# CostaLab/PILOT

Measured on AMD Instinct MI355X. Metric: W2 patient-pairs/sec (full NxN EMD matrix), higher is better.
Workload: dtype f32 (products as 2-way fp16 splits, 22 significant bits, on the f16 MFMA, f32 accumulate)

## Files before the change

pilot_amd/csrc/grid_plan.hpp:

```cpp
#pragma once
#include <hip/hip_runtime.h>

#include "abi_common.hpp"
#include "sinkhorn_layout.hpp"

constexpr int TIMING_RING = 64;

struct pilot_ot_plan {
    int N, K, device;
    double max_cost;
    void *img;
    void *p_slot;
    int *track_list;
    int *ctrl;
    int *order_list;
    unsigned char *order_bucket;
    int *order_hist;
    int *flags_ws;
    int *emd_counter;
    double *f_slab;
    size_t f_slab_bytes;
    double *emdg_slab;
    int emdg_wgs;
    double *kws;
    int generic_wgs;
    float *wide_rec;
    size_t wide_rec_n;
    int *nan_list;
    int n_cu;
    int timing;
    long n_timed;
    long n_calls;
    hipEvent_t ev[TIMING_RING][4];
    int graph_mode;
    int gkey_seen;
    struct GraphKey {
        const void *P, *M, *emd, *iters, *err, *flags;
        double reg, stop_thr, tau, floor_ulps, max_cost;
        int num_iter_max, check_period, cfg, mixed, sym, row_begin, n_rows, row_step;
        pilot::SinkhornSwitches sw;
        bool operator==(const GraphKey &o) const {
            return P == o.P && M == o.M && emd == o.emd && iters == o.iters && err == o.err && flags == o.flags && reg == o.reg &&
                   stop_thr == o.stop_thr && tau == o.tau && floor_ulps == o.floor_ulps && max_cost == o.max_cost && num_iter_max == o.num_iter_max &&
                   check_period == o.check_period && cfg == o.cfg && mixed == o.mixed && sym == o.sym && row_begin == o.row_begin &&
                   n_rows == o.n_rows && row_step == o.row_step && sw == o.sw;
        }
    } gkey;
    hipStream_t gstream;
    hipGraphExec_t gexec;
};

namespace pilot {

struct HostCtx {
    pilot_ot_plan *plan = nullptr;
    int N = 0, K = 0, device = -1;
    size_t n_out = 0;
    double *dP = nullptr, *dM = nullptr, *dE = nullptr, *dErr = nullptr;
    int *dIt = nullptr, *dFl = nullptr;
    unsigned char *pin = nullptr;
    size_t pin_bytes = 0;
    static constexpr int FETCH_EVENTS = 32;
    hipEvent_t fev[FETCH_EVENTS];
    int n_fev = 0;
    void release() {
        for (int i = 0; i < n_fev; ++i) (void)hipEventDestroy(fev[i]);
        n_fev = 0;
        if (pin) (void)hipHostFree(pin);
        pin = nullptr; pin_bytes = 0;
        if (dP) (void)hipFree(dP);
        if (dM) (void)hipFree(dM);
        if (dE) (void)hipFree(dE);
        if (dErr) (void)hipFree(dErr);
        if (dIt) (void)hipFree(dIt);
        if (dFl) (void)hipFree(dFl);
        dP = dM = dE = dErr = nullptr; dIt = dFl = nullptr;
        if (plan) pilot_ot_plan_destroy(plan);
        plan = nullptr; N = K = 0; n_out = 0; device = -1;
    }
    ~HostCtx() {}
};
HostCtx &thread_host();
int host_ctx_prepare(int N, int K, size_t n_out);
struct Fetch { void *dst; const void *src; size_t bytes; };
int host_fetch(const Fetch *f, int n);

size_t emd_counter_bytes();

}
```

pilot_amd/csrc/pilot_ot_sinkhorn.hip:

```cpp
#include <hip/hip_runtime.h>

#include <chrono>
#include <cmath>
#include <cstdio>
#include <cstdlib>
#include <new>

#include "abi_common.hpp"
#include "grid_plan.hpp"
#include "sinkhorn_launch.hpp"
#include "generic_kernels.hpp"

namespace {
using pilot::LDS_BYTES, pilot::MAX_K, pilot::GENERIC_MAX_K, pilot::WIDE_MAX_K;

bool split_fits_lds(int K, bool sym, int bands = 1) {
    const pilot::CfgShape c = pilot::shape_of(pilot::CFG_S32);
    return pilot::stream_layout(c, (K + 15) / 16, sym, true, 0, bands, 4).bytes + (size_t)pilot::handover_elems(c) * 4 <= LDS_BYTES;
}
}

static double h_max_cost_over_reg() {
    const char *e = pilot::test_switch("PILOT_OT_H_MAX_COST_OVER_REG");
    return e && *e ? atof(e) : pilot::H_MAX_COST_OVER_REG;
}

PILOT_API int pilot_ot_auto_precision(double max_cost_over_reg) {
    if (max_cost_over_reg <= h_max_cost_over_reg()) return PILOT_OT_PREC_F16X2;
    return max_cost_over_reg <= 60.0 ? PILOT_OT_PREC_BF16X3 : PILOT_OT_PREC_F64;
}

PILOT_API int pilot_ot_auto_precision_for(double max_cost_over_reg, int K, int cost_is_symmetric) {
    int prec = pilot_ot_auto_precision(max_cost_over_reg);
    if ((prec == PILOT_OT_PREC_BF16X3 || prec == PILOT_OT_PREC_F16X2) && !split_fits_lds(K, cost_is_symmetric != 0, 1)) prec = PILOT_OT_PREC_F32;
    return prec;
}

PILOT_API int pilot_ot_resolve_precision(int precision, double max_cost_over_reg, int K, int cost_is_symmetric, double tau) {
    if (precision == PILOT_OT_PREC_GENERIC || max_cost_over_reg > PILOT_OT_MAX_COST_OVER_REG) return PILOT_OT_PREC_GENERIC;
    const bool f32_class = precision == PILOT_OT_PREC_F32 || precision == PILOT_OT_PREC_BF16X3 || precision == PILOT_OT_PREC_F16X2;
    const char *raw = pilot::test_switch("PILOT_OT_RAW_PRECISION");
    const bool promote = f32_class && max_cost_over_reg > 60.0 && !(raw && *raw && *raw != '0');
    if (precision == PILOT_OT_PREC_AUTO || promote) {
        precision = pilot_ot_auto_precision_for(max_cost_over_reg, K, cost_is_symmetric);
        if (precision == PILOT_OT_PREC_F64) precision = PILOT_OT_PREC_AUTO_MIXED;
    }
    if (precision == PILOT_OT_PREC_F16X2 &&
        (max_cost_over_reg > h_max_cost_over_reg() || tau > pilot::H_MAX_TAU || !split_fits_lds(K, cost_is_symmetric != 0, 1)))
        precision = split_fits_lds(K, cost_is_symmetric != 0, 1) ? PILOT_OT_PREC_BF16X3 : PILOT_OT_PREC_F32;
    return precision;
}

PILOT_API int pilot_ot_plan_create(int N, int K, pilot_ot_plan **plan) {
    if (!plan) return fail(PILOT_OT_EINVAL, "plan is NULL");
    if (N <= 0 || K <= 0) return fail(PILOT_OT_EINVAL, "N=%d K=%d must be positive", N, K);
    if (K > GENERIC_MAX_K) return fail(PILOT_OT_ENOTSUP, "K=%d > %d cell types", K, GENERIC_MAX_K);
    if ((long long)N * N > 0x7fffffffLL) return fail(PILOT_OT_ENOTSUP, "N=%d: N*N overflows the pair index", N);
    pilot_ot_plan *pl = new (std::nothrow) pilot_ot_plan();
    if (!pl) return fail(PILOT_OT_EINVAL, "out of host memory");
    pl->N = N; pl->K = K; pl->max_cost = 1.0;
    pl->img = nullptr; pl->p_slot = nullptr; pl->track_list = nullptr; pl->ctrl = nullptr;
    pl->emd_counter = nullptr; pl->f_slab = nullptr; pl->f_slab_bytes = 0; pl->emdg_slab = nullptr; pl->emdg_wgs = 0; pl->n_cu = 256; pl->kws = nullptr; pl->generic_wgs = 0; pl->nan_list = nullptr;
    pl->wide_rec = nullptr; pl->wide_rec_n = 0;
    pl->order_list = nullptr; pl->order_bucket = nullptr; pl->order_hist = nullptr;
    pl->flags_ws = nullptr;
    pl->timing = 0; pl->n_timed = 0; pl->n_calls = 0;
    pl->graph_mode = 0; pl->gkey_seen = 0; pl->gstream = nullptr; pl->gexec = nullptr;
    for (int i = 0; i < TIMING_RING; ++i) for (int j = 0; j < 4; ++j) pl->ev[i][j] = nullptr;
    hipError_t e = hipGetDevice(&pl->device);
    if (e == hipSuccess) pl->n_cu = pilot::cu_count();
    const int kp = ((K + 31) / 32) * 32;
    if (K <= MAX_K) {
        const int rt = (K + 15) / 16;
        size_t img_bytes = pilot::img_elems(pilot::CFG_F64, rt) * sizeof(double);
        const size_t b32 = pilot::img_elems(pilot::CFG_F32, rt) * sizeof(float), bs = pilot::img_elems(pilot::CFG_S32, rt) * sizeof(float);
        const size_t bh = pilot::img_elems(pilot::CFG_H32, rt) * sizeof(float);
        if (b32 > img_bytes) img_bytes = b32;
        if (bs > img_bytes) img_bytes = bs;
        if (bh > img_bytes) img_bytes = bh;
        if (e == hipSuccess) e = hipMalloc(&pl->img, img_bytes);
    } else if (K <= WIDE_MAX_K) {
        if (e == hipSuccess) e = hipMalloc(&pl->img, pilot::img_elems(pilot::CFG_H32, 16) * sizeof(float));
    }
    {
        size_t p_bytes = sizeof(double) * ((size_t)N * kp + N);
        if (K > MAX_K && K <= WIDE_MAX_K) { const size_t two = 2 * sizeof(float) * ((size_t)N * 256 + N); p_bytes = two > p_bytes ? two : p_bytes; }
        if (e == hipSuccess) e = hipMalloc(&pl->p_slot, p_bytes);
    }
    if (e == hipSuccess) e = hipMalloc(reinterpret_cast<void **>(&pl->track_list), sizeof(int) * (size_t)N * N);
    if (e == hipSuccess) e = hipMalloc(reinterpret_cast<void **>(&pl->ctrl), pilot::CTRL_BLOCK_INTS * sizeof(int));
    if (e == hipSuccess) e = hipMalloc(reinterpret_cast<void **>(&pl->order_list), sizeof(int) * (size_t)N * N);
    if (e == hipSuccess) e = hipMalloc(reinterpret_cast<void **>(&pl->order_bucket), (size_t)N * N);
    if (e == hipSuccess) e = hipMalloc(reinterpret_cast<void **>(&pl->emd_counter), pilot::emd_counter_bytes());
    if (e == hipSuccess) e = hipMalloc(reinterpret_cast<void **>(&pl->nan_list), 2 * sizeof(int) * (size_t)N * N);
    if (e == hipSuccess) e = hipMalloc(reinterpret_cast<void **>(&pl->flags_ws), sizeof(int) * (size_t)N * N);
    if (e != hipSuccess) {
        pilot_ot_plan_destroy(pl);
        return fail(PILOT_OT_EHIP, "plan allocation failed: %s", hipGetErrorString(e));
    }
    pl->order_hist = pl->ctrl + pilot::CTRL_ORDER_HIST;
    *plan = pl;
    return PILOT_OT_OK;
}

PILOT_API int pilot_ot_plan_set_max_cost(pilot_ot_plan *pl, double max_cost) {
    if (!pl) return fail(PILOT_OT_EINVAL, "plan is NULL");
    if (!(max_cost > 0.0) || !std::isfinite(max_cost)) return fail(PILOT_OT_EINVAL, "max_cost=%g must be positive and finite", max_cost);
    pl->max_cost = max_cost;
    return PILOT_OT_OK;
}

PILOT_API int pilot_ot_plan_destroy(pilot_ot_plan *pl) {
    if (!pl) return PILOT_OT_OK;
    if (pl->img) (void)hipFree(pl->img);
    if (pl->p_slot) (void)hipFree(pl->p_slot);
    if (pl->track_list) (void)hipFree(pl->track_list);
    if (pl->ctrl) (void)hipFree(pl->ctrl);
    if (pl->order_list) (void)hipFree(pl->order_list);
    if (pl->order_bucket) (void)hipFree(pl->order_bucket);
    if (pl->flags_ws) (void)hipFree(pl->flags_ws);
    if (pl->emd_counter) (void)hipFree(pl->emd_counter);
    if (pl->f_slab) (void)hipFree(pl->f_slab);
    if (pl->emdg_slab) (void)hipFree(pl->emdg_slab);
    if (pl->kws) (void)hipFree(pl->kws);
    if (pl->nan_list) (void)hipFree(pl->nan_list);
    if (pl->wide_rec) (void)hipFree(pl->wide_rec);
    if (pl->gexec) (void)hipGraphExecDestroy(pl->gexec);
    if (pl->gstream) (void)hipStreamDestroy(pl->gstream);
    for (int i = 0; i < TIMING_RING; ++i) for (int j = 0; j < 4; ++j) if (pl->ev[i][j]) (void)hipEventDestroy(pl->ev[i][j]);
    delete pl;
    return PILOT_OT_OK;
}

namespace {

int check_grid_args(int N, int K, double reg, int num_iter_max, double stop_thr, double tau, int check_period,
                    int precision, int row_begin, int row_end, int row_step) {
    if (N <= 0 || K <= 0) return fail(PILOT_OT_EINVAL, "N=%d K=%d must be positive", N, K);
    if (!(reg > 0.0) || !std::isfinite(reg)) return fail(PILOT_OT_EINVAL, "reg=%g must be positive and finite", reg);
    if (num_iter_max < 1) return fail(PILOT_OT_EINVAL, "num_iter_max=%d must be >= 1", num_iter_max);
    if (check_period < 1) return fail(PILOT_OT_EINVAL, "check_period=%d must be >= 1", check_period);
    if (!(stop_thr >= 0.0) || !(stop_thr < 1.0)) return fail(PILOT_OT_EINVAL, "stop_thr=%g must be in [0, 1)", stop_thr);
    if (!(tau > 1.0)) return fail(PILOT_OT_EINVAL, "tau=%g must be > 1", tau);
    if (precision < PILOT_OT_PREC_AUTO || precision > PILOT_OT_PREC_F16X2)
        return fail(PILOT_OT_EINVAL, "unknown precision id %d", precision);
    if (row_step < 1 || row_begin < 0 || row_end > N || row_begin > row_end)
        return fail(PILOT_OT_EINVAL, "bad row range [%d, %d) step %d for N=%d", row_begin, row_end, row_step, N);
    if (K > GENERIC_MAX_K) return fail(PILOT_OT_ENOTSUP, "K=%d > %d cell types", K, GENERIC_MAX_K);
    return PILOT_OT_OK;
}

constexpr double MAX_COST_OVER_REG = PILOT_OT_MAX_COST_OVER_REG;

int run_generic(pilot_ot_plan *pl, const pilot::SinkhornSwitches &sw, const double *d_P, const double *d_M, double reg, int num_iter_max, double stop_thr, double tau,
                int check_period, int row_begin, int n_rows, int row_step, double *d_emd, int *d_iters, double *d_err, int *d_flags,
                hipStream_t s, const int *list = nullptr, const int *list_len = nullptr, int *queue = nullptr) {
    const int N = pl->N, K = pl->K;
    const int n_pairs = n_rows * N;
    if (n_pairs == 0) return PILOT_OT_OK;
    int nsplit = pilot::GENERIC_WAVES;
    auto lds_for = [&](int ns) { return sizeof(double) * ((8 + (size_t)ns) * (size_t)K + pilot::GENERIC_WAVES) + 16; };
    while (nsplit > 1 && lds_for(nsplit) > LDS_BYTES) nsplit /= 2;
    const size_t lds = lds_for(nsplit);
    if (lds > LDS_BYTES) return fail(PILOT_OT_ENOTSUP, "K=%d does not fit the generic kernel's LDS vectors", K);
    if (!pl->kws) {
        int wgs = 3 * pl->n_cu;
        const size_t per = sizeof(double) * 2 * (size_t)K * K;
        while (wgs > 1 && per * wgs > ((size_t)8 << 30)) wgs /= 2;
        HIP_TRY(hipMalloc(reinterpret_cast<void **>(&pl->kws), per * wgs));
        pl->generic_wgs = wgs;
    }
    if (!queue) { queue = pl->ctrl + pilot::CTRL_GENERIC_HEAD; HIP_TRY(hipMemsetAsync(queue, 0, sizeof(int), s)); }
    pilot::GenericParams g;
    g.P = d_P; g.M = d_M; g.N = N; g.K = K; g.n_pairs = n_pairs; g.row_begin = row_begin; g.row_step = row_step;
    g.reg = reg; g.tau = tau; g.stop_thr = stop_thr; g.max_iter = num_iter_max; g.period = check_period;
    g.emd = d_emd; g.iters = d_iters; g.err = d_err; g.flags = d_flags; g.kws = pl->kws; g.queue = queue; g.nsplit = nsplit;
    g.list = list; g.list_len = list_len;
    int wgs = pl->generic_wgs < n_pairs ? pl->generic_wgs : n_pairs;
    if (list && wgs > 64) wgs = 64;
    if (sw.generic_wgs > 0 && sw.generic_wgs < wgs) wgs = sw.generic_wgs;
    HIP_TRY(hipFuncSetAttribute(reinterpret_cast<const void *>(pilot::sinkhorn_generic_kernel), hipFuncAttributeMaxDynamicSharedMemorySize, (int)lds));
    hipLaunchKernelGGL(pilot::sinkhorn_generic_kernel, dim3(wgs), dim3(pilot::GENERIC_WG), lds, s, g);
    HIP_TRY(hipGetLastError());
    return PILOT_OT_OK;
}

pilot::GridParams call_params(const pilot_ot_plan *pl, int n_pairs, int row_begin, int row_step, int num_iter_max, int check_period,
                              double stop_thr, double tau, double floor_ulps, double *d_emd, int *d_iters, double *d_err, int *d_flags) {
    pilot::GridParams p;
    p.P = pl->p_slot; p.img = pl->img; p.N = pl->N; p.K = pl->K;
    p.n_pairs = n_pairs;
    p.list = pl->order_list; p.list_len = nullptr;
    p.solo_len = nullptr; p.solo_head = nullptr; p.solo_blocks = 0;
    p.row_begin = row_begin; p.row_step = row_step;
    p.max_iter = num_iter_max; p.period = check_period;
    p.stop_thr = stop_thr; p.tau = tau; p.floor_ulps = floor_ulps;
    p.emd = d_emd; p.iters = d_iters; p.err = d_err; p.flags = d_flags;
    p.track_list = pl->track_list; p.track_count = pl->ctrl + pilot::CTRL_TRACK_LEN;
    p.queue_head = pl->ctrl + pilot::CTRL_HEAD_FAST; p.queue_shards = nullptr;
    p.ring = 0; p.bands = 1;
    p.fb_list = nullptr; p.fb_count = nullptr;
    p.nan_list = pl->nan_list; p.nan_count = pl->ctrl + pilot::CTRL_NAN_LEN;
    p.unequal = pl->ctrl + pilot::CTRL_UNEQUAL;
    p.debug = 0;
    return p;
}

int run_grid(int cfg, pilot_ot_plan *pl, const pilot::SinkhornSwitches &sw, const double *d_P, const double *d_M, double reg, int num_iter_max,
             double stop_thr, double tau, int check_period, double floor_ulps, bool sym, int row_begin, int n_rows, int row_step,
             double *d_emd, int *d_iters, double *d_err, int *d_flags, hipStream_t s, bool mixed = false) {
    const int N = pl->N, K = pl->K, RT = (K + 15) / 16;
    const pilot::GridPasses g = pilot::plan_grid(cfg, N, K, n_rows, sym, mixed, pl->max_cost / reg, pl->n_cu, sw);
    if (g.rc != PILOT_OT_OK) return fail(g.rc, "%s", g.msg);
    HIP_TRY(hipMemsetAsync(pl->ctrl, 0, pilot::CTRL_BLOCK_INTS * sizeof(int), s));
    if (n_rows == 0) return PILOT_OT_OK;
    pilot::GridParams p = call_params(pl, n_rows * N, row_begin, row_step, num_iter_max, check_period, stop_thr, tau, floor_ulps, d_emd, d_iters,
                                      d_err, d_flags);
    p.debug = sw.debug;
    int *const lists[] = {pl->order_list, pl->track_list, pl->nan_list + (size_t)N * N};
    auto slot = [&](int at) { return at == pilot::CTRL_NONE ? nullptr : pl->ctrl + at; };
    if (g.f64.run) { p.fb_list = lists[g.f64.list]; p.fb_count = slot(pilot::CTRL_FB_LEN); }
    if (g.fast.solo_blocks) { p.solo_len = slot(pilot::CTRL_SOLO_LEN); p.solo_head = slot(pilot::CTRL_HEAD_SOLO); }
    auto launch = [&](const pilot::PassPlan &v) -> hipError_t {
        p.list = lists[v.list]; p.list_len = slot(v.len_slot); p.queue_head = slot(v.head_slot); p.queue_shards = slot(v.shards_at);
        p.solo_blocks = v.solo_blocks; p.ring = v.lds.ring; p.bands = v.bands;
        const dim3 wgs(v.wgs);
        if (v.solo_f64) return pilot::launch_solo_track_f64(wgs, s, p);
        if (v.tv) return pilot::launch_stream_tv(v.cfg, v.tv, RT, sym, v.track, wgs, v.lds.bytes, s, p);
        if (v.quad) return pilot::launch_quad(wgs, s, p);
        if (v.cfg == pilot::CFG_H32) return pilot::launch_stream_h32(RT, sym, v.live1, wgs, v.lds.bytes, s, p);
        if (v.cfg == pilot::CFG_S32) return pilot::launch_stream_s32(RT, sym, v.track, v.live1, wgs, v.lds.bytes, s, p);
        return v.cfg == pilot::CFG_F64 ? pilot::launch_stream_f64(RT, sym, v.track, wgs, v.lds.bytes, s, p)
                                       : pilot::launch_stream_f32(RT, sym, v.track, wgs, v.lds.bytes, s, p);
    };
    HIP_TRY(pilot::launch_prep(cfg, d_M, K, RT, reg, pl->img, d_P, pl->p_slot, N, g.write_tail, stop_thr, floor_ulps, n_rows, row_begin, row_step,
                               pl->order_bucket, pl->order_hist, pl->order_list, slot(pilot::CTRL_SPLIT), slot(pilot::CTRL_HEAD_FAST), g.mode, g.ob, s));
    hipEvent_t *ev = (pl->timing > 0 && (pl->n_calls++ % pl->timing) == 0) ? pl->ev[pl->n_timed % TIMING_RING] : nullptr;
    if (ev) HIP_TRY(hipEventRecord(ev[0], s));
    if (g.fast.run) HIP_TRY(launch(g.fast));
    if (ev) { HIP_TRY(hipEventRecord(ev[1], s)); HIP_TRY(hipEventRecord(ev[2], s)); }
    p.img = static_cast<float *>(pl->img) + pilot::track_img_elems(cfg, RT);
    HIP_TRY(launch(g.track));
    if (g.f64.run) {
        HIP_TRY(pilot::launch_prep(pilot::CFG_F64, d_M, K, RT, reg, pl->img, d_P, pl->p_slot, N, 2, stop_thr, floor_ulps, 0, row_begin, row_step,
                                   pl->order_bucket, pl->order_hist, pl->order_list, slot(pilot::CTRL_SPLIT), slot(pilot::CTRL_HEAD_FAST), 0, 1, s));
        p.img = pl->img; p.fb_list = nullptr; p.fb_count = nullptr;
        HIP_TRY(launch(g.f64));
    }
    if (ev) { HIP_TRY(hipEventRecord(ev[3], s)); ++pl->n_timed; }
    if (sw.debug & pilot::DBG_NO_NAN_PASS) return PILOT_OT_OK;
    return run_generic(pl, sw, d_P, d_M, reg, num_iter_max, stop_thr, tau, check_period, row_begin, n_rows, row_step, d_emd, d_iters, d_err, d_flags,
                       s, pl->nan_list, slot(pilot::CTRL_NAN_LEN), slot(pilot::CTRL_NAN_HEAD));
}

int run_wide(pilot_ot_plan *pl, const pilot::SinkhornSwitches &sw, const double *d_P, const double *d_M, double reg, int num_iter_max, double stop_thr, double tau,
             int check_period, double floor_ulps, int row_begin, int n_rows, int row_step, double *d_emd, int *d_iters, double *d_err,
             int *d_flags, hipStream_t s) {
    const int N = pl->N, K = pl->K, RT = 16;
    long WIDE_CHUNK_PAIRS = 512L * 1024;
    if (const char *e = pilot::test_switch("PILOT_OT_WIDE_CHUNK")) { const long v = atol(e); if (v > 0) WIDE_CHUNK_PAIRS = v; }
    if ((long)n_rows * N > WIDE_CHUNK_PAIRS && n_rows > 1) {
        const int rows_per = (int)(WIDE_CHUNK_PAIRS / N) > 0 ? (int)(WIDE_CHUNK_PAIRS / N) : 1;
        for (int r0 = 0; r0 < n_rows; r0 += rows_per) {
            const int nr = n_rows - r0 < rows_per ? n_rows - r0 : rows_per;
            const size_t off = (size_t)r0 * N;
            const int rc = run_wide(pl, sw, d_P, d_M, reg, num_iter_max, stop_thr, tau, check_period, floor_ulps, row_begin + r0 * row_step, nr, row_step,
                                    d_emd + off, d_iters ? d_iters + off : nullptr, d_err ? d_err + off : nullptr, d_flags + off, s);
            if (rc != PILOT_OT_OK) return rc;
        }
        return PILOT_OT_OK;
    }
    HIP_TRY(hipMemsetAsync(pl->ctrl, 0, (pilot::CTRL_ORDER_HIST + 2 * pilot::ORDER_NB) * sizeof(int), s));
    if (n_rows == 0) return PILOT_OT_OK;
    const int n_pairs = n_rows * N;
    if ((size_t)n_pairs > pl->wide_rec_n) {
        if (pl->wide_rec) HIP_TRY(hipFree(pl->wide_rec));
        pl->wide_rec = nullptr; pl->wide_rec_n = 0;
        HIP_TRY(hipMalloc(reinterpret_cast<void **>(&pl->wide_rec), sizeof(float) * pilot::wide_rec_elems() * (size_t)n_pairs));
        pl->wide_rec_n = (size_t)n_pairs;
    }
    int ob = (n_pairs + 1023) / 1024;
    if (ob > pl->n_cu) ob = pl->n_cu;
    HIP_TRY(pilot::launch_prep(pilot::CFG_H32, d_M, K, RT, reg, pl->img, d_P, pl->p_slot, N, 0, stop_thr, floor_ulps, n_rows, row_begin, row_step,
                               pl->order_bucket, pl->order_hist, pl->order_list, pl->ctrl + pilot::CTRL_SPLIT, pl->ctrl + pilot::CTRL_HEAD_FAST, 0, ob, s));
    const pilot::GridParams p = call_params(pl, n_pairs, row_begin, row_step, num_iter_max, check_period, stop_thr, tau, floor_ulps, d_emd,
                                            d_iters, d_err, d_flags);
    hipEvent_t *ev = (pl->timing > 0 && (pl->n_calls++ % pl->timing) == 0) ? pl->ev[pl->n_timed % TIMING_RING] : nullptr;
    if (ev) HIP_TRY(hipEventRecord(ev[0], s));
    const int tiles = (n_pairs + 15) / 16;
    int wgs = pl->n_cu < tiles ? pl->n_cu : tiles;
    HIP_TRY(pilot::launch_wide(dim3(wgs), s, p, pl->wide_rec));
    if (ev) { HIP_TRY(hipEventRecord(ev[1], s)); HIP_TRY(hipEventRecord(ev[2], s)); }
    HIP_TRY(pilot::launch_wide_value(dim3(pilot::clamp_wgs(pl->n_cu, 2, tiles)), s, p, pl->wide_rec));
    if (ev) { HIP_TRY(hipEventRecord(ev[3], s)); ++pl->n_timed; }
    return run_generic(pl, sw, d_P, d_M, reg, num_iter_max, stop_thr, tau, check_period, row_begin, n_rows, row_step, d_emd, d_iters, d_err,
                       d_flags, s, pl->nan_list, pl->ctrl + pilot::CTRL_NAN_LEN, pl->ctrl + pilot::CTRL_NAN_HEAD);
}

pilot::SinkhornSwitches read_switches() {
    const char *dbg = pilot::test_switch("PILOT_OT_DEBUG");
    const int debug = dbg ? atoi(dbg) : 0;
    const int no_quad = pilot::test_switch("PILOT_OT_NO_QUAD") ? 1 : 0;
    const char *gw = pilot::test_switch("PILOT_OT_GENERIC_WGS");
    return {debug, no_quad, gw ? atoi(gw) : 0};
}

}

PILOT_API int pilot_ot_sinkhorn_grid_dev(pilot_ot_plan *pl, const double *d_P, const double *d_M, double reg,
                                         int num_iter_max, double stop_thr, double tau, int check_period,
                                         int precision, double f32_floor_ulps, int cost_is_symmetric,
                                         int row_begin, int row_end, int row_step, double *d_emd, int *d_iters,
                                         double *d_err, int *d_flags, void *stream) {
    if (!pl || !d_P || !d_M || !d_emd) return fail(PILOT_OT_EINVAL, "NULL pointer");
    int rc = check_grid_args(pl->N, pl->K, reg, num_iter_max, stop_thr, tau, check_period, precision, row_begin,
                             row_end, row_step);
    if (rc != PILOT_OT_OK) return rc;
    const pilot::SinkhornSwitches sw = read_switches();
    if (!d_flags) d_flags = pl->flags_ws;
    {
        const int n_rows_g = (row_end - row_begin + row_step - 1) / row_step;
        if (pl->K > MAX_K && pl->K <= WIDE_MAX_K && cost_is_symmetric && precision != PILOT_OT_PREC_GENERIC && precision != PILOT_OT_PREC_F64 &&
            pl->max_cost / reg <= h_max_cost_over_reg() && tau <= pilot::H_MAX_TAU && !pilot::test_switch("PILOT_OT_NO_WIDE")) {
            if (!(f32_floor_ulps > 0.0)) f32_floor_ulps = 8.0;
            return run_wide(pl, sw, d_P, d_M, reg, num_iter_max, stop_thr, tau, check_period, f32_floor_ulps, row_begin, n_rows_g, row_step, d_emd,
                            d_iters, d_err, d_flags, static_cast<hipStream_t>(stream));
        }
        if (precision == PILOT_OT_PREC_GENERIC || pl->K > MAX_K || pl->max_cost / reg > MAX_COST_OVER_REG)
            return run_generic(pl, sw, d_P, d_M, reg, num_iter_max, stop_thr, tau, check_period, row_begin, n_rows_g, row_step, d_emd,
                               d_iters, d_err, d_flags, static_cast<hipStream_t>(stream));
    }
    precision = pilot_ot_resolve_precision(precision, pl->max_cost / reg, pl->K, cost_is_symmetric, tau);
    bool mixed = false;
    if (precision == PILOT_OT_PREC_AUTO_MIXED) {
        precision = PILOT_OT_PREC_F64;
        mixed = true;
    }
    mixed = mixed && split_fits_lds(pl->K, cost_is_symmetric != 0, 2) && pl->max_cost / reg <= 140.0 && !pilot::test_switch("PILOT_OT_NO_MIXED");
    if (!(f32_floor_ulps > 0.0)) f32_floor_ulps = 8.0;
    const int n_rows = (row_end - row_begin + row_step - 1) / row_step;
    hipStream_t s = static_cast<hipStream_t>(stream);
    const int cfg = mixed ? pilot::CFG_S32
                          : (precision == PILOT_OT_PREC_F32 ? pilot::CFG_F32
                             : (precision == PILOT_OT_PREC_BF16X3 ? pilot::CFG_S32 : (precision == PILOT_OT_PREC_F16X2 ? pilot::CFG_H32 : pilot::CFG_F64)));
    auto run = [&](hipStream_t on) {
        int r = run_grid(cfg, pl, sw, d_P, d_M, reg, num_iter_max, stop_thr, tau, check_period, f32_floor_ulps, cost_is_symmetric != 0,
                         row_begin, n_rows, row_step, d_emd, d_iters, d_err, d_flags, on, mixed);
        if (r == PILOT_OT_ENOTSUP)
            r = run_generic(pl, sw, d_P, d_M, reg, num_iter_max, stop_thr, tau, check_period, row_begin, n_rows, row_step, d_emd, d_iters,
                            d_err, d_flags, on);
        return r;
    };
    if (!pl->graph_mode || pl->timing || n_rows == 0) return run(s);
    const pilot_ot_plan::GraphKey key = {d_P, d_M, d_emd, d_iters, d_err, d_flags, reg, stop_thr, tau, f32_floor_ulps, pl->max_cost, num_iter_max,
                                         check_period, cfg, mixed ? 1 : 0, cost_is_symmetric != 0 ? 1 : 0, row_begin, n_rows, row_step, sw};
    if (pl->gexec && key == pl->gkey) {
        HIP_TRY(hipGraphLaunch(pl->gexec, s));
        return PILOT_OT_OK;
    }
    if (pl->gexec) { (void)hipGraphExecDestroy(pl->gexec); pl->gexec = nullptr; }
    if (!(pl->gkey_seen && key == pl->gkey)) {
        pl->gkey = key; pl->gkey_seen = 1;
        return run(s);
    }
    if (!pl->gstream) HIP_TRY(hipStreamCreateWithFlags(&pl->gstream, hipStreamNonBlocking));
    HIP_TRY(hipStreamBeginCapture(pl->gstream, hipStreamCaptureModeThreadLocal));
    rc = run(pl->gstream);
    hipGraph_t graph = nullptr;
    const hipError_t ce = hipStreamEndCapture(pl->gstream, &graph);
    if (rc != PILOT_OT_OK) { if (graph) (void)hipGraphDestroy(graph); return rc; }
    if (ce != hipSuccess) { (void)hipGetLastError(); return fail(PILOT_OT_EHIP, "graph capture failed: %s", hipGetErrorString(ce)); }
    const hipError_t ie = hipGraphInstantiate(&pl->gexec, graph, nullptr, nullptr, 0);
    (void)hipGraphDestroy(graph);
    if (ie != hipSuccess) { (void)hipGetLastError(); pl->gexec = nullptr; return fail(PILOT_OT_EHIP, "graph instantiation failed: %s", hipGetErrorString(ie)); }
    HIP_TRY(hipGraphLaunch(pl->gexec, s));
    return PILOT_OT_OK;
}

PILOT_API int pilot_ot_plan_enable_graph(pilot_ot_plan *pl, int enable) {
    if (!pl) return fail(PILOT_OT_EINVAL, "plan is NULL");
    pl->graph_mode = enable ? 1 : 0;
    if (!enable) {
        if (pl->gexec) { (void)hipGraphExecDestroy(pl->gexec); pl->gexec = nullptr; }
        pl->gkey_seen = 0;
    }
    return PILOT_OT_OK;
}

PILOT_API int pilot_ot_sinkhorn_grid(const double *P, int N, int K, const double *M, double reg, int num_iter_max,
                                     double stop_thr, double tau, int check_period, int precision,
                                     double f32_floor_ulps, int cost_is_symmetric, int row_begin, int row_end,
                                     int row_step, double *emd, int *iters, double *err, int *flags) {
    if (!P || !M || !emd) return fail(PILOT_OT_EINVAL, "NULL pointer");
    int rc = check_grid_args(N, K, reg, num_iter_max, stop_thr, tau, check_period, precision, row_begin, row_end,
                             row_step);
    if (rc != PILOT_OT_OK) return rc;
    double mx = 0.0;
    for (size_t t = 0; t < (size_t)K * K; ++t) mx = M[t] > mx ? M[t] : mx;
    precision = pilot_ot_resolve_precision(precision, mx / reg, K, cost_is_symmetric, tau);
    const int n_rows = (row_end - row_begin + row_step - 1) / row_step;
    const size_t n_out = (size_t)n_rows * N;
    if (n_out == 0) return PILOT_OT_OK;

    const bool trace = pilot::test_switch("PILOT_OT_HOST_TRACE") != nullptr;
    auto now = [] { return std::chrono::steady_clock::now(); };
    auto us = [](std::chrono::steady_clock::time_point a, std::chrono::steady_clock::time_point b) { return std::chrono::duration<double, std::micro>(b - a).count(); };
    const auto t0 = now();
    rc = pilot::host_ctx_prepare(N, K, n_out);
    if (rc != PILOT_OT_OK) return rc;
    pilot::HostCtx &h = pilot::thread_host();
    hipError_t e = hipMemcpy(h.dP, P, sizeof(double) * (size_t)N * K, hipMemcpyHostToDevice);
    if (e == hipSuccess) e = hipMemcpy(h.dM, M, sizeof(double) * (size_t)K * K, hipMemcpyHostToDevice);
    if (e != hipSuccess) return fail(PILOT_OT_EHIP, "H2D copy failed: %s", hipGetErrorString(e));
    const auto t1 = now();
    h.plan->max_cost = mx > 0.0 ? mx : 1.0;
    rc = pilot_ot_sinkhorn_grid_dev(h.plan, h.dP, h.dM, reg, num_iter_max, stop_thr, tau, check_period, precision,
                                    f32_floor_ulps, cost_is_symmetric, row_begin, row_end, row_step, h.dE,
                                    iters ? h.dIt : nullptr, err ? h.dErr : nullptr, h.dFl, nullptr);
    if (rc != PILOT_OT_OK) return rc;
    const auto t2 = now();
    if (trace) (void)hipStreamSynchronize(nullptr);
    const auto t3 = now();
    const pilot::Fetch f[4] = {{emd, h.dE, sizeof(double) * n_out}, {iters, h.dIt, sizeof(int) * n_out},
                        {err, h.dErr, sizeof(double) * n_out}, {flags, h.dFl, sizeof(int) * n_out}};
    rc = pilot::host_fetch(f, 4);
    if (trace) fprintf(stderr, "pilot_ot_sinkhorn_grid: prepare + H2D %.0f us, enqueue %.0f us, device %.0f us, fetch %.0f us\n", us(t0, t1), us(t1, t2), us(t2, t3), us(t3, now()));
    return rc;
}

PILOT_API int pilot_ot_plan_enable_timing(pilot_ot_plan *pl, int enable) {
    if (!pl) return fail(PILOT_OT_EINVAL, "plan is NULL");
    if (enable)
        for (int i = 0; i < TIMING_RING; ++i)
            for (int j = 0; j < 4; ++j)
                if (!pl->ev[i][j]) HIP_TRY(hipEventCreate(&pl->ev[i][j]));
    pl->timing = enable > 0 ? enable : 0;
    pl->n_timed = 0; pl->n_calls = 0;
    return PILOT_OT_OK;
}

PILOT_API int pilot_ot_plan_kernel_times(pilot_ot_plan *pl, int max_n, float *main_ms, float *track_ms, int *n_out) {
    if (!pl || !main_ms || !track_ms || !n_out) return fail(PILOT_OT_EINVAL, "NULL pointer");
    long n = pl->n_timed < TIMING_RING ? pl->n_timed : TIMING_RING;
    if (n > max_n) n = max_n;
    for (long t = 0; t < n; ++t) {
        const long call = pl->n_timed - n + t;
        hipEvent_t *ev = pl->ev[call % TIMING_RING];
        HIP_TRY(hipEventElapsedTime(&main_ms[t], ev[0], ev[1]));
        HIP_TRY(hipEventElapsedTime(&track_ms[t], ev[2], ev[3]));
    }
    *n_out = (int)n;
    return PILOT_OT_OK;
}
```

pilot_amd/csrc/quad_kernels.hpp:

```cpp
#pragma once
#include "sinkhorn_kernels.hpp"

namespace pilot {

constexpr int QUAD_WAVES = 4, QUAD_KB = 4, QUAD_RING = 32;

__device__ inline void lds_barrier() { asm volatile("s_waitcnt lgkmcnt(0)\n\ts_barrier" ::: "memory"); }

template <int RT>
__global__ void __launch_bounds__(WAVE * QUAD_WAVES, 2) sinkhorn_quad_kernel(GridParams p) {
    static_assert(RT == 7 || RT == 8, "four waves own two row-tiles each");
    using C = CfgH32x16;
    using acc_t = C::acc_t;
    constexpr int TILE = C::TILE, NREG = C::NREG, NGRP = C::NGRP, KB = QUAD_KB;
    __shared__ u32x4_t PB[2][KB][2][WAVE];
    __shared__ u32x4_t ring_pu[QUAD_RING][KB][2][NGRP];
    __shared__ u32x4_t ring_pv[QUAD_RING][KB][2][NGRP];
    __shared__ int ring_meta[QUAD_RING][2];
    __shared__ int ovc[2][TILE];
    __shared__ float red_e2[2][QUAD_WAVES][TILE];
    __shared__ float red_val[QUAD_WAVES][TILE];
    __shared__ int sh_base[2];
    const int wave = threadIdx.x / WAVE, lane = threadIdx.x % WAVE, col = lane % TILE, grp = lane / TILE;
    const int K = p.K, N = p.N;
    constexpr int KP = RT * TILE;
    constexpr int KBL = (RT + 1) / 2;
    constexpr bool tail16 = PILOT_TAIL16 && (RT & 1);
    const int n_items = p.list_len ? *p.list_len : p.n_pairs;
    const float *img = static_cast<const float *>(p.img);
    constexpr int FORM = form_elems<C>(RT);
    const float *Pt = static_cast<const float *>(p.P) + (size_t)N * KP + N;
    const float *acc0 = img + 3 * FORM;
    const float tau = float(p.tau) * H_PANEL_SCALE;
    const unsigned long long colmask = (1ull << TILE) - 1ull;
    bool tile_live[2];
#pragma unroll
    for (int tl = 0; tl < 2; ++tl) tile_live[tl] = 2 * wave + tl < RT;

    u32x4_t AR[2][KB][2];
    unsigned int padmask = 0u;
#pragma unroll
    for (int tl = 0; tl < 2; ++tl)
#pragma unroll
        for (int r = 0; r < NREG; ++r) padmask |= (C::lidx(2 * wave + tl, r, grp) >= K ? 1u : 0u) << (tl * NREG + r);

    auto product_of = [&](const u32x4_t (&IMG)[2][KB][2], auto bget, acc_t (&OUT)[2]) {
#pragma unroll
        for (int kb = 0; kb < KBL; ++kb) {
            const u32x4_t b0 = bget(kb, 0), b1 = bget(kb, 1);
            if constexpr (tail16) {
                if (kb == KBL - 1) {
                    tail16_gap();
#pragma unroll
                    for (int tl = 0; tl < 2; ++tl) {
                        OUT[tl] = mfma_pieces<C, true>(IMG[1][kb][tl], b0, OUT[tl]);
                        OUT[tl] = mfma_pieces<C, true>(IMG[0][kb][tl], b1, OUT[tl]);
                        OUT[tl] = mfma_pieces<C, true>(IMG[0][kb][tl], b0, OUT[tl]);
                    }
                    continue;
                }
            }
#pragma unroll
            for (int tl = 0; tl < 2; ++tl) {
                OUT[tl] = mfma_pieces<C>(IMG[1][kb][tl], b0, OUT[tl]);
                OUT[tl] = mfma_pieces<C>(IMG[0][kb][tl], b1, OUT[tl]);
                OUT[tl] = mfma_pieces<C>(IMG[0][kb][tl], b0, OUT[tl]);
            }
        }
    };
    auto product = [&](int panel, acc_t (&OUT)[2]) {
#pragma unroll
        for (int tl = 0; tl < 2; ++tl)
#pragma unroll
            for (int r = 0; r < NREG; ++r) OUT[tl][r] = (padmask >> (tl * NREG + r)) & 1u ? 1.f : 0.f;
        product_of(AR, [&](int kb, int part) { return PB[panel][kb][part][lane]; }, OUT);
    };
    auto pieces_of = [&](const acc_t (&X)[2], u32x4_t &hi, u32x4_t &lo) {
#pragma unroll
        for (int h = 0; h < 4; ++h) {
            unsigned int a, b;
            quot_pieces(X[h / 2][2 * (h & 1)], X[h / 2][2 * (h & 1) + 1], a, b);
            hi[h] = a; lo[h] = b;
        }
    };

    u32x4_t AGM[2][KB][2];
    auto load_image = [&](int form, u32x4_t (&IMG)[2][KB][2]) {
        const u32x4_t *src = reinterpret_cast<const u32x4_t *>(img + form * FORM) + lane;
#pragma unroll
        for (int part = 0; part < 2; ++part)
#pragma unroll
            for (int kb = 0; kb < KBL; ++kb)
#pragma unroll
                for (int tl = 0; tl < 2; ++tl) {
                    const int t = 2 * wave + tl < RT ? 2 * wave + tl : RT - 1;
                    u32x4_t x = src[((part * KBL + kb) * RT + t) * WAVE];
                    if constexpr (RT & 1) {
                        const unsigned int m = tile_live[tl] ? 0xffffffffu : 0u;
#pragma unroll
                        for (int e = 0; e < 4; ++e) x[e] &= m;
                    }
                    IMG[part][kb][tl] = x;
                }
    };
    auto flush = [&](int cnt) {
        lds_barrier();
        for (int base = 0; base < cnt; base += TILE) {
            const int n = cnt - base < TILE ? cnt - base : TILE;
            const int s = base + (col < n ? col : n - 1);
            acc_t W[2];
#pragma unroll
            for (int tl = 0; tl < 2; ++tl)
#pragma unroll
                for (int r = 0; r < NREG; ++r) W[tl][r] = 0.f;
            product_of(AGM, [&](int kb, int part) { return ring_pv[s][kb][part][grp]; }, W);
            const u32x4_t uh = ring_pu[s][wave][0][grp], ul = ring_pu[s][wave][1][grp];
            float val = 0.f;
#pragma unroll
            for (int h = 0; h < 4; ++h) {
                val += pieces_sum_lo(uh[h], ul[h]) * W[h / 2][2 * (h & 1)];
                val += pieces_sum_hi(uh[h], ul[h]) * W[h / 2][2 * (h & 1) + 1];
            }
            val = group_sum<C>(val);
            if (grp == 0) red_val[wave][col] = val;
            lds_barrier();
            if (wave == 0 && grp == 0 && col < n) {
                float tot = 0.f;
#pragma unroll
                for (int w = 0; w < QUAD_WAVES; ++w) tot += red_val[w][col];
                tot *= 1.f / H_IN_SCALE;
                const int qq = ring_meta[s][0];
                int fl = ring_meta[s][1];
                if (p.nan_list && (!(tot - tot == 0.f) || (fl & FLAG_NAN))) {
                    p.nan_list[__hip_atomic_fetch_add(p.nan_count, 1, __ATOMIC_RELAXED, __HIP_MEMORY_SCOPE_AGENT)] = qq;
                } else {
                    if (tot != tot) fl |= FLAG_NAN;
                    p.emd[qq] = double(tot);
                    p.flags[qq] = fl;
                }
            }
            lds_barrier();
        }
    };

    load_image(0, AR);
    load_image(2, AGM);
    bool active = false, want = true, exhausted = false;
    int q = 0, ii = 0, chk = 1, flags = 0, ring_cnt = 0;
    float errv = 1.f, thr = 0.f;
    acc_t A[2], B[2], V[2], ACC[2];
#pragma unroll
    for (int tl = 0; tl < 2; ++tl)
#pragma unroll
        for (int r = 0; r < NREG; ++r) { A[tl][r] = B[tl][r] = V[tl][r] = 0.f; ACC[tl][r] = 1.f; }
    int res_next = 0, res_end = 0, res_base = 0, qbatch = 0, ibatch = 0, jbatch = 0, draws = 0;
    const bool all_over = p.unequal && *p.unequal != 0;
    if (threadIdx.x < 2 * TILE) (&ovc[0][0])[threadIdx.x] = 0;
    lds_barrier();
    if ((int)blockIdx.x * TILE >= n_items) return;

    for (int it = 0;; ++it) {
        const int par = it & 1;
        const unsigned long long wmask = __ballot(want) & colmask;
        if (wmask) {
            if (res_next >= res_end && !exhausted) {
                int base;
                if (draws == 0) {
                    base = (int)blockIdx.x * TILE;
                } else {
                    if (threadIdx.x == 0)
                        sh_base[draws & 1] = (int)gridDim.x * TILE + __hip_atomic_fetch_add(p.queue_head, TILE, __ATOMIC_RELAXED, __HIP_MEMORY_SCOPE_AGENT);
                    lds_barrier();
                    base = __builtin_amdgcn_readfirstlane(sh_base[draws & 1]);
                }
                ++draws;
                exhausted = base >= n_items;
                res_next = exhausted ? n_items : base;
                res_end = (base + TILE < n_items) ? base + TILE : n_items;
                if (exhausted) res_end = n_items;
                res_base = base;
                const int bi = base + col;
                qbatch = (p.list && bi < n_items) ? p.list[bi] : bi;
                const int qv = bi < n_items ? qbatch : 0;
                ibatch = p.row_begin + (qv / N) * p.row_step;
                jbatch = qv % N;
            }
            const int avail = res_end - res_next;
            const int n_want = (int)__popcll(wmask);
            const int rank = (int)__popcll(wmask & ((1ull << col) - 1ull));
            const int item = res_next + rank;
            const bool take = want && rank < avail;
            const int bsel = 4 * ((item - res_base) & (TILE - 1));
            const int qsel = __builtin_amdgcn_ds_bpermute(bsel, qbatch);
            const int isel = __builtin_amdgcn_ds_bpermute(bsel, ibatch), jsel = __builtin_amdgcn_ds_bpermute(bsel, jbatch);
            res_next = __builtin_amdgcn_readfirstlane(res_next + (n_want < avail ? n_want : avail));
            if (want && !take && exhausted) {
                want = false;
#pragma unroll
                for (int tl = 0; tl < 2; ++tl)
#pragma unroll
                    for (int r = 0; r < NREG; ++r) { A[tl][r] = B[tl][r] = 0.f; ACC[tl][r] = 1.f; }
            }
            if (take) {
                want = false; active = true;
                q = qsel;
#pragma unroll
                for (int tl = 0; tl < 2; ++tl) {
                    const int t = 2 * wave + tl;
#pragma unroll
                    for (int r = 0; r < NREG; ++r) { A[tl][r] = B[tl][r] = 0.f; ACC[tl][r] = 1.f; }
                    if (tile_live[tl]) {
                        load_regs<C>(Pt + (size_t)isel * KP + (t * NGRP + grp) * NREG, A[tl]);
                        load_regs<C>(Pt + (size_t)jsel * KP + (t * NGRP + grp) * NREG, B[tl]);
                        load_regs<C>(acc0 + (t * NGRP + grp) * NREG, ACC[tl]);
                    }
                }
                thr = Pt[(size_t)N * KP + jsel];
                chk = 1; ii = 0; flags = 0; errv = 1.f;
                if (all_over) {
                    if (wave == 0 && grp == 0) p.track_list[__hip_atomic_fetch_add(p.track_count, 1, __ATOMIC_RELAXED, __HIP_MEMORY_SCOPE_AGENT)] = q;
                    active = false; want = true;
                }
            }
        }
        if (__ballot(active || want) == 0ull) break;

        float mx = 0.f;
#pragma unroll
        for (int tl = 0; tl < 2; ++tl)
#pragma unroll
            for (int r = 0; r < NREG; ++r) { V[tl][r] = B[tl][r] * C::rcp(ACC[tl][r]); mx = fmaxf(mx, V[tl][r]); }
        {
            u32x4_t hi, lo;
            pieces_of(V, hi, lo);
            PB[0][wave][0][lane] = hi; PB[0][wave][1][lane] = lo;
        }
        if (active && !(mx <= tau)) ovc[par][col] = 1;
        lds_barrier();
        product(0, ACC);
        mx = 0.f;
        {
            acc_t U[2];
#pragma unroll
            for (int tl = 0; tl < 2; ++tl)
#pragma unroll
                for (int r = 0; r < NREG; ++r) { U[tl][r] = A[tl][r] * C::rcp(ACC[tl][r]); mx = fmaxf(mx, U[tl][r]); }
            u32x4_t hi, lo;
            pieces_of(U, hi, lo);
            PB[1][wave][0][lane] = hi; PB[1][wave][1][lane] = lo;
        }
        if (active && !(mx <= tau)) ovc[par][col] = 1;
        if (threadIdx.x < TILE) ovc[par ^ 1][threadIdx.x] = 0;
        lds_barrier();
        const bool over = active && ovc[par][col] != 0;
        if (over) {
            if (wave == 0 && grp == 0) p.track_list[__hip_atomic_fetch_add(p.track_count, 1, __ATOMIC_RELAXED, __HIP_MEMORY_SCOPE_AGENT)] = q;
            active = false; want = true;
        }
        ++ii;
        product(1, ACC);
        const bool pending = active && ii == chk;
        if (pending) chk += p.period;
        const bool capped = active && ii >= p.max_iter;
        if (__ballot(pending || capped)) {
            float e2 = 0.f;
#pragma unroll
            for (int tl = 0; tl < 2; ++tl) {
                float et = 0.f;
#pragma unroll
                for (int r = 0; r < NREG; ++r) { const float d = V[tl][r] * ACC[tl][r] - B[tl][r]; et += d * d; }
                e2 += et;
            }
            e2 = group_sum<C>(e2);
            if (grp == 0) red_e2[par][wave][col] = e2;
            lds_barrier();
            float tot = 0.f;
#pragma unroll
            for (int w = 0; w < QUAD_WAVES; ++w) tot += red_e2[par][w][col];
            const float e = sqrtf(tot);
            bool fin = capped;
            if (pending) {
                errv = e;
                if (e <= thr) { fin = true; flags |= FLAG_CONVERGED; }
                else if (e != e) { fin = true; flags |= FLAG_NAN; }
            }
            unsigned long long fmask = __ballot(fin) & colmask;
            if (fmask) {
                if (fin && wave == 0 && grp == 0) {
                    if (p.iters) p.iters[q] = ii;
                    if (p.err) p.err[q] = double(errv) * double(1.f / H_IN_SCALE);
                }
                while (fmask) {
                    if (ring_cnt >= QUAD_RING) { flush(ring_cnt); ring_cnt = 0; }
                    const int space = QUAD_RING - ring_cnt;
                    const int rank = (int)__popcll(fmask & ((1ull << col) - 1ull));
                    const bool put = fin && ((fmask >> col) & 1ull) && rank < space;
                    if (put) {
                        const int s = ring_cnt + rank;
                        ring_pu[s][wave][0][grp] = PB[1][wave][0][lane]; ring_pu[s][wave][1][grp] = PB[1][wave][1][lane];
                        ring_pv[s][wave][0][grp] = PB[0][wave][0][lane]; ring_pv[s][wave][1][grp] = PB[0][wave][1][lane];
                        if (wave == 0 && grp == 0) { ring_meta[s][0] = q; ring_meta[s][1] = flags; }
                    }
                    const unsigned long long taken = __ballot(put) & colmask;
                    fmask &= ~taken;
                    ring_cnt = __builtin_amdgcn_readfirstlane(ring_cnt + (int)__popcll(taken));
                }
                if (fin) { active = false; want = true; }
            }
        }
    }
    if (ring_cnt > 0) flush(ring_cnt);
}

}
```

pilot_amd/csrc/sinkhorn_kernels.hpp:

```cpp
#pragma once
#include <hip/hip_runtime.h>

#include "sinkhorn_layout.hpp"

namespace pilot {

constexpr int FLAG_CONVERGED = 1, FLAG_NAN = 2, FLAG_ABSORB_LAST = 4, FLAG_ABSORBED = 8, FLAG_F64 = 16;


struct CfgF32x16 {
    using T = float;
    static constexpr bool SPLIT = false, HALF = false;
    static constexpr int NP = 0;
    static constexpr int TILE = 16, NREG = 4, NGRP = 4, VEC = 4;
    using acc_t = float __attribute__((ext_vector_type(4)));
    using vec4_t = float __attribute__((ext_vector_type(4)));
    __host__ __device__ static constexpr int lidx(int t, int r, int g) { return 4 * (4 * t + r) + g; }
    __host__ __device__ static constexpr int lidx_of_row(int t, int p) { return lidx(t, p & 3, p >> 2); }
    __device__ static inline acc_t mfma(float a, float b, acc_t c) {
        return __builtin_amdgcn_mfma_f32_16x16x4f32(a, b, c, 0, 0, 0);
    }
    __device__ static inline float rcp(float x) { return __builtin_amdgcn_rcpf(x); }
    __device__ static inline float eps() { return 1.1920929e-07f; }
};
// ... 241 lines not shown
        V v;
#pragma unroll
        for (int e = 0; e < C::VEC; ++e) v[e] = x[c * C::VEC + e];
        *reinterpret_cast<V *>(dst + c * C::VEC) = v;
    }
}
template <class C> __device__ inline void load_regs(const typename C::T *src, typename C::acc_t &x) {
    using V = typename C::vec4_t;
#pragma unroll
    for (int c = 0; c < C::NREG / C::VEC; ++c) {
        const V v = *reinterpret_cast<const V *>(src + c * C::VEC);
#pragma unroll
        for (int e = 0; e < C::VEC; ++e) x[c * C::VEC + e] = v[e];
    }
}

constexpr float SPLIT_SAFE_MIN = 7.70371978e-34f;
constexpr float BAND1_DOWN = 2.93873588e-39f;
constexpr double BAND1_UP_LN = 88.722839111672999;
using bf16x8_t = __bf16 __attribute__((ext_vector_type(8)));
using bf16x2_t = __bf16 __attribute__((ext_vector_type(2)));
using f16x8_t = _Float16 __attribute__((ext_vector_type(8)));
using f16x2_t = _Float16 __attribute__((ext_vector_type(2)));
using u32x4_t = unsigned int __attribute__((ext_vector_type(4)));
using f32x2_t = float __attribute__((ext_vector_type(2)));

__device__ inline unsigned int cvt_pk_bf16(float lo, float hi) {
    const f32x2_t v = {lo, hi};
    return __builtin_bit_cast(unsigned int, __builtin_convertvector(v, bf16x2_t));
}
__device__ inline unsigned int cvt_pk_f16(float lo, float hi) {
    const f32x2_t v = {lo, hi};
    return __builtin_bit_cast(unsigned int, __builtin_convertvector(v, f16x2_t));
}
__device__ inline float resid_f16_lo(float x, unsigned int h) {
    float r;
    asm("v_fma_mix_f32 %0, %1, -1.0, %2 op_sel:[0,0,0] op_sel_hi:[1,0,0]" : "=v"(r) : "v"(h), "v"(x));
    return r;
}
__device__ inline float resid_f16_hi(float x, unsigned int h) {
    float r;
    asm("v_fma_mix_f32 %0, %1, -1.0, %2 op_sel:[1,0,0] op_sel_hi:[1,0,0]" : "=v"(r) : "v"(h), "v"(x));
    return r;
}
__device__ inline void quot_pieces(float x0, float x1, unsigned int &hi, unsigned int &lo) {
    hi = cvt_pk_f16(x0, x1);
    lo = cvt_pk_f16(resid_f16_lo(x0, hi), resid_f16_hi(x1, hi));
}
__device__ inline float pieces_sum_lo(unsigned int h, unsigned int l) {
    float r;
    asm("v_fma_mix_f32 %0, %1, 1.0, %2 op_sel:[0,0,0] op_sel_hi:[1,0,1]" : "=v"(r) : "v"(h), "v"(l));
    return r;
}
__device__ inline float pieces_sum_hi(unsigned int h, unsigned int l) {
    float r;
    asm("v_fma_mix_f32 %0, %1, 1.0, %2 op_sel:[1,0,1] op_sel_hi:[1,0,1]" : "=v"(r) : "v"(h), "v"(l));
    return r;
}
__device__ inline unsigned int pk_max3_f16(unsigned int a, unsigned int b, unsigned int c) {
    unsigned int r;
    asm("v_pk_maximum3_f16 %0, %1, %2, %3" : "=v"(r) : "v"(a), "v"(b), "v"(c));
    return r;
}
template <int NP> struct Pieces { unsigned int p[NP]; };
template <class C> __device__ inline Pieces<C::NP> split_pair(float x0, float x1) {
    Pieces<C::NP> o;
    if constexpr (C::HALF) {
        o.p[0] = cvt_pk_f16(x0, x1);
        o.p[1] = cvt_pk_f16(resid_f16_lo(x0, o.p[0]), resid_f16_hi(x1, o.p[0]));
    } else {
        o.p[0] = cvt_pk_bf16(x0, x1);
        float r0 = x0 - __uint_as_float(o.p[0] << 16), r1 = x1 - __uint_as_float(o.p[0] & 0xffff0000u);
        o.p[1] = cvt_pk_bf16(r0, r1);
        r0 -= __uint_as_float(o.p[1] << 16);
        r1 -= __uint_as_float(o.p[1] & 0xffff0000u);
        o.p[2] = cvt_pk_bf16(r0, r1);
    }
    return o;
}
__host__ __device__ constexpr int split_kblocks(int RT) { return (RT + 1) / 2; }
template <int NP> __host__ __device__ constexpr int n_terms() { return NP == 3 ? 6 : 3; }
template <int NP> __host__ __device__ constexpr int term_a(int i) {
    if (NP == 3) return i == 0 ? 2 : (i == 2 || i == 3 ? 1 : 0);
    return i == 0 ? 1 : 0;
}
template <int NP> __host__ __device__ constexpr int term_b(int i) {
    if (NP == 3) return i == 1 ? 2 : (i == 2 || i == 4 ? 1 : 0);
    return i == 1 ? 1 : 0;
}
#ifndef PILOT_TAIL16
#define PILOT_TAIL16 7
#endif
template <int RT, int BIT = 7> __host__ __device__ constexpr bool tail16_kb(int kb) { return (PILOT_TAIL16 & BIT) && (RT & 1) && kb == (RT + 1) / 2 - 1; }
using u32x2_t = unsigned int __attribute__((ext_vector_type(2)));
using f16x4_t = _Float16 __attribute__((ext_vector_type(4)));
using s16x4_t = short __attribute__((ext_vector_type(4)));
#ifndef PILOT_TAIL16_GAP
#define PILOT_TAIL16_GAP 12
#endif
#ifndef PILOT_TAIL16_ORDER
#define PILOT_TAIL16_ORDER 1
#endif
__device__ inline void tail16_gap() {
    __builtin_amdgcn_sched_barrier(0);
    asm volatile("s_nop %0" ::"n"(PILOT_TAIL16_GAP - 1) : "memory");
    __builtin_amdgcn_sched_barrier(0);
}
template <class C, bool TAIL16 = false> __device__ inline typename C::acc_t mfma_pieces(u32x4_t a, u32x4_t b, typename C::acc_t c) {
    if constexpr (TAIL16) {
        const u32x2_t a2 = {a[0], a[1]}, b2 = {b[0], b[1]};
        if constexpr (C::HALF) return __builtin_amdgcn_mfma_f32_16x16x16f16(__builtin_bit_cast(f16x4_t, a2), __builtin_bit_cast(f16x4_t, b2), c, 0, 0, 0);
        else return __builtin_amdgcn_mfma_f32_16x16x16bf16_1k(__builtin_bit_cast(s16x4_t, a2), __builtin_bit_cast(s16x4_t, b2), c, 0, 0, 0);
    } else {
    if constexpr (C::HALF) return __builtin_amdgcn_mfma_f32_16x16x32_f16(__builtin_bit_cast(f16x8_t, a), __builtin_bit_cast(f16x8_t, b), c, 0, 0, 0);
    else return __builtin_amdgcn_mfma_f32_16x16x32_bf16(__builtin_bit_cast(bf16x8_t, a), __builtin_bit_cast(bf16x8_t, b), c, 0, 0, 0);
    }
}

template <int RT, int NP> struct SplitPanel { u32x4_t p[NP][split_kblocks(RT)]; };
template <class C, int RT, bool LIVE1 = false>
__device__ inline void split_panel(const typename C::acc_t (&IN)[RT], SplitPanel<RT, C::NP> &B) {
    constexpr int KB = split_kblocks(RT);
#pragma unroll
    for (int kb = 0; kb < KB; ++kb)
#pragma unroll
        for (int h = 0; h < 4; ++h) {
            const int t = 2 * kb + h / 2;
            Pieces<C::NP> sp;
#pragma unroll
            for (int part = 0; part < C::NP; ++part) sp.p[part] = 0u;
            if (t < RT && !(LIVE1 && t == RT - 1 && (h & 1)))
                sp = split_pair<C>(IN[t < RT ? t : 0][2 * (h & 1)], (LIVE1 && t == RT - 1) ? 0.f : IN[t < RT ? t : 0][2 * (h & 1) + 1]);
#pragma unroll
            for (int part = 0; part < C::NP; ++part) B.p[part][kb][h] = sp.p[part];
        }
}
template <class C, int RT, int TP = C::NP>
__device__ inline typename C::acc_t split_tile_product(const typename C::T *form, int lane, int t, const SplitPanel<RT, C::NP> &B,
                                                       typename C::acc_t acc) {
    constexpr int KB = split_kblocks(RT);
    const u32x4_t *img = reinterpret_cast<const u32x4_t *>(form);
#pragma unroll
    for (int kb = 0; kb < KB; ++kb) {
        u32x4_t a[TP];
#pragma unroll
        for (int part = 0; part < TP; ++part) a[part] = img[((part * KB + kb) * RT + t) * WAVE + lane];
        if (tail16_kb<RT, 4>(kb)) {
            if (kb > 0) tail16_gap();
#pragma unroll
            for (int i = 0; i < n_terms<TP>(); ++i) acc = mfma_pieces<C, true>(a[term_a<TP>(i)], B.p[term_b<TP>(i)][kb], acc);
        } else {
#pragma unroll
        for (int i = 0; i < n_terms<TP>(); ++i) acc = mfma_pieces<C>(a[term_a<TP>(i)], B.p[term_b<TP>(i)][kb], acc);
        }
    }
    return acc;
}
template <class C, int RT> __host__ __device__ constexpr int lds_ahead() {
#ifdef PILOT_LDS_AHEAD
    return PILOT_LDS_AHEAD;
#else
    return !C::HALF ? 1 : (RT <= 5 ? 2 : 3);
#endif
}
template <class C, int RT>
__device__ inline void panel_product_pieces(const typename C::T *form, const typename C::T *form1, int lane,
                                            const SplitPanel<RT, C::NP> &B, typename C::acc_t (&OUT)[RT],
                                            const typename C::acc_t &last_init) {
    constexpr int KB = split_kblocks(RT), NP = C::NP;
    const u32x4_t *img = reinterpret_cast<const u32x4_t *>(form) + lane;
    constexpr bool TAILS_LAST = PILOT_TAIL16_ORDER == 1 && tail16_kb<RT, 2>(KB - 1) && KB > 1;
    constexpr int STEPS = RT * KB, FULL = RT * (KB - 1);
    auto step_t = [](int s) { return TAILS_LAST ? (s < FULL ? s / (KB - 1) : s - FULL) : s / KB; };
    auto step_kb = [](int s) { return TAILS_LAST ? (s < FULL ? s % (KB - 1) : KB - 1) : s % KB; };
    constexpr int AHEAD = lds_ahead<C, RT>();
    u32x4_t a[AHEAD + 1][NP];
#pragma unroll
    for (int d = 0; d < AHEAD; ++d)
        if (d < STEPS) {
#pragma unroll
            for (int part = 0; part < NP; ++part) a[d][part] = img[((part * KB + step_kb(d)) * RT + step_t(d)) * WAVE];
        }
#pragma unroll
    for (int t = 0; t < RT; ++t)
#pragma unroll
        for (int r = 0; r < 4; ++r) OUT[t][r] = (t == RT - 1) ? last_init[r] : 0.f;
#pragma unroll
    for (int s = 0; s < STEPS; ++s) {
        const int t = step_t(s), kb = step_kb(s);
        if (s + AHEAD < STEPS) {
            const int nt = step_t(s + AHEAD), nkb = step_kb(s + AHEAD);
#pragma unroll
            for (int part = 0; part < NP; ++part) a[(s + AHEAD) % (AHEAD + 1)][part] = img[((part * KB + nkb) * RT + nt) * WAVE];
        }
        __builtin_amdgcn_sched_barrier(0x6);
        const u32x4_t (&ac)[NP] = a[s % (AHEAD + 1)];
        if (tail16_kb<RT, 2>(kb)) {
            if (kb > 0 && !TAILS_LAST) tail16_gap();
#pragma unroll
            for (int i = 0; i < n_terms<NP>(); ++i) OUT[t] = mfma_pieces<C, true>(ac[term_a<NP>(i)], B.p[term_b<NP>(i)][kb], OUT[t]);
        } else {
#pragma unroll
            for (int i = 0; i < n_terms<NP>(); ++i) OUT[t] = mfma_pieces<C>(ac[term_a<NP>(i)], B.p[term_b<NP>(i)][kb], OUT[t]);
        }
        __builtin_amdgcn_sched_barrier(0x6);
    }
    if (form1) {
#pragma unroll
        for (int t = 0; t < RT; ++t) {
            typename C::acc_t zero;
#pragma unroll
            for (int r = 0; r < 4; ++r) zero[r] = 0.f;
            const typename C::acc_t lo = split_tile_product<C, RT, 2>(form1, lane, t, B, zero);
#pragma unroll
            for (int r = 0; r < 4; ++r) OUT[t][r] = fmaf(lo[r], BAND1_DOWN, OUT[t][r]);
        }
    }
}
template <int RT, int NP> struct SplitImage { u32x4_t a[NP][split_kblocks(RT)][RT]; };
#ifndef PILOT_AREG_ORDER
#define PILOT_AREG_ORDER 2
#endif
#ifndef PILOT_E2_EARLY
#define PILOT_E2_EARLY 0
#endif
#ifndef PILOT_DEFER_HANDOVER
#define PILOT_DEFER_HANDOVER 1
#endif
#ifndef PILOT_E2_PACKED
#define PILOT_E2_PACKED 1
#endif
template <class C, int RT>
__device__ inline void panel_product_pieces_regs(const SplitImage<RT, C::NP> &A, const SplitPanel<RT, C::NP> &B,
                                                 typename C::acc_t (&OUT)[RT], const typename C::acc_t &last_init) {
    constexpr int KB = split_kblocks(RT), NP = C::NP;
#pragma unroll
    for (int t = 0; t < RT; ++t)
#pragma unroll
        for (int r = 0; r < 4; ++r) OUT[t][r] = (t == RT - 1) ? last_init[r] : 0.f;
#if PILOT_AREG_ORDER == 0
#pragma unroll
    for (int t = 0; t < RT; ++t)
#pragma unroll
        for (int kb = 0; kb < KB; ++kb)
#pragma unroll
            for (int i = 0; i < n_terms<NP>(); ++i) OUT[t] = mfma_pieces<C>(A.a[term_a<NP>(i)][kb][t], B.p[term_b<NP>(i)][kb], OUT[t]);
#elif PILOT_AREG_ORDER == 2
#pragma unroll
    for (int kb = 0; kb < KB - 1; ++kb)
#pragma unroll
        for (int i = 0; i < n_terms<NP>(); ++i)
#pragma unroll
            for (int t = 0; t < RT; ++t) OUT[t] = mfma_pieces<C>(A.a[term_a<NP>(i)][kb][t], B.p[term_b<NP>(i)][kb], OUT[t]);
#pragma unroll
    for (int t = 0; t < RT; ++t)
#pragma unroll
        for (int i = 0; i < n_terms<NP>(); ++i) OUT[t] = mfma_pieces<C, tail16_kb<RT, 1>(KB - 1)>(A.a[term_a<NP>(i)][KB - 1][t], B.p[term_b<NP>(i)][KB - 1], OUT[t]);
#elif PILOT_AREG_ORDER == 3
#pragma unroll
    for (int kb = 0; kb < KB; ++kb)
#pragma unroll
        for (int t = 0; t < RT; ++t)
#pragma unroll
            for (int i = 0; i < n_terms<NP>(); ++i) OUT[t] = mfma_pieces<C>(A.a[term_a<NP>(i)][kb][t], B.p[term_b<NP>(i)][kb], OUT[t]);
#elif PILOT_AREG_ORDER == 4
#pragma unroll
    for (int kb = 0; kb < KB - 1; ++kb)
#pragma unroll
        for (int i = 0; i < n_terms<NP>(); ++i)
#pragma unroll
            for (int t = 0; t < RT; ++t) OUT[t] = mfma_pieces<C>(A.a[term_a<NP>(i)][kb][t], B.p[term_b<NP>(i)][kb], OUT[t]);
#pragma unroll
    for (int t0 = 0; t0 < RT; t0 += 2)
#pragma unroll
        for (int i = 0; i < n_terms<NP>(); ++i)
#pragma unroll
            for (int t = t0; t < (t0 + 2 < RT ? t0 + 2 : RT); ++t) OUT[t] = mfma_pieces<C>(A.a[term_a<NP>(i)][KB - 1][t], B.p[term_b<NP>(i)][KB - 1], OUT[t]);
#else
#pragma unroll
    for (int kb = 0; kb < KB; ++kb)
#pragma unroll
        for (int i = 0; i < n_terms<NP>(); ++i)
#pragma unroll
            for (int t = 0; t < RT; ++t) OUT[t] = mfma_pieces<C>(A.a[term_a<NP>(i)][kb][t], B.p[term_b<NP>(i)][kb], OUT[t]);
#endif
}
template <class C, int RT, bool LIVE1 = false>
__device__ inline void panel_product_split(const typename C::T *form, const typename C::T *form1, int lane,
                                           const typename C::acc_t (&IN)[RT], typename C::acc_t (&OUT)[RT],
                                           const typename C::acc_t &last_init) {
    SplitPanel<RT, C::NP> B;
    split_panel<C, RT, LIVE1>(IN, B);
    panel_product_pieces<C, RT>(form, form1, lane, B, OUT, last_init);
}

constexpr int QUEUE_SHARD_MAX_RT = 2;
struct GridParams {
    const void *P;
    const void *img;
    int N, K;
    int n_pairs;
    const int *list;
    const int *list_len;
    int row_begin, row_step;
    int max_iter, period;
    double stop_thr, tau, floor_ulps;
    double *emd;
    int *iters;
    double *err;
    int *flags;
    int *track_list;
    int *track_count;
    int *queue_head;
    int *queue_shards;
    const int *solo_len;
    int *solo_head;
    int solo_blocks;
    int ring;
    int bands;
    int *fb_list;
    int *fb_count;
    int *nan_list;
    int *nan_count;
    int debug;
    const int *unequal;
};

template <class C> constexpr int form_elems(int RT) { return form_elems(shape_of<C>(), RT); }
template <class C> __host__ __device__ constexpr int acc0_offset(int RT) { return 3 * form_elems<C>(RT); }
template <class C> __host__ __device__ constexpr int tail_offset(int RT) { return acc0_offset<C>(RT) + RT * C::TILE; }
template <class C> __host__ __device__ constexpr int plain_offset(int RT) { return tail_offset<C>(RT) + 2 * 2 * ((RT - 1) * 4 + 1) * WAVE * 2; }
template <class C> __host__ __device__ constexpr int band1_offset(int RT) { return plain_offset<C>(RT) + 3 * 64 * WAVE; }
template <class C> __host__ __device__ constexpr int img_total_plain(int RT) { return band1_offset<C>(RT) + ((C::SPLIT && !C::HALF) ? 3 * form_elems<C>(RT) : 0); }
template <class C> __host__ __device__ constexpr int track_img_offset(int RT) { return C::HALF ? band1_offset<C>(RT) : 0; }
template <class C> __host__ __device__ constexpr int img_total(int RT) { return img_total_plain<C>(RT) + (C::HALF ? img_total_plain<CfgS32x16>(RT) : 0); }


template <typename T> __device__ inline T readlane_t(T x, int k);
template <> __device__ inline float readlane_t<float>(float x, int k) {
    return __int_as_float(__builtin_amdgcn_readlane(__float_as_int(x), k));
}
template <> __device__ inline double readlane_t<double>(double x, int k) {
    union { double d; int u[2]; } v;
    v.d = x;
    v.u[0] = __builtin_amdgcn_readlane(v.u[0], k);
    v.u[1] = __builtin_amdgcn_readlane(v.u[1], k);
    return v.d;
}
template <typename T> __device__ inline T wave_sum(T x) {
#pragma unroll
    for (int off = 1; off < 16; off <<= 1) x += __shfl_xor(x, off);
    return sum_xor32(sum_xor16(x));
}

template <class C, bool SYM, int NCH, bool TRACK = false>
__device__ inline void solo_pairs(const GridParams &p, unsigned char *solo_smem, const int *n_items_ptr, int *head_ptr) {
    constexpr int RT = NCH, KP = NCH * C::TILE;
    using T = typename C::T;
    const int lane = threadIdx.x % WAVE;
    const int K = p.K, N = p.N;
    const T *img = static_cast<const T *>(p.img);
    const T *plain = img + plain_offset<C>(RT);
    const T *Pt = static_cast<const T *>(p.P);
    constexpr int KC = NCH * 16;
    using P2 = pair_of<T>;
    P2 g1[KC / 2], g2[SYM ? 1 : KC / 2];
#pragma unroll
    for (int k = 0; k < KC / 2; ++k) {
        g1[k] = P2{plain[(2 * k) * WAVE + lane], plain[(2 * k + 1) * WAVE + lane]};
        if constexpr (!SYM) g2[k] = P2{plain[64 * WAVE + (2 * k) * WAVE + lane], plain[64 * WAVE + (2 * k + 1) * WAVE + lane]};
    }
    T *xline = reinterpret_cast<T *>(solo_smem) + (threadIdx.x / WAVE) * WAVE;
    using V4 = T __attribute__((ext_vector_type(16 / sizeof(T))));
    constexpr int VE = 16 / sizeof(T);
    auto matvec = [&](const P2 (&g)[KC / 2], T x) {
        xline[lane] = x;
        constexpr int NV = NCH * 16 / VE;
        V4 xv[NV];
#pragma unroll
        for (int c = 0; c < NV; ++c) xv[c] = *reinterpret_cast<const V4 *>(xline + c * VE);
        P2 acc[4];
#pragma unroll
        for (int j = 0; j < 4; ++j) acc[j] = P2{T(0), T(0)};
#pragma unroll
        for (int c = 0; c < NV; ++c)
#pragma unroll
            for (int h = 0; h < VE / 2; ++h) {
                const int k2 = c * (VE / 2) + h;
                const P2 xx = {xv[c][2 * h], xv[c][2 * h + 1]};
                acc[k2 & 3] = __builtin_elementwise_fma(g[k2], xx, acc[k2 & 3]);
            }
        const P2 s2 = (acc[0] + acc[1]) + (acc[2] + acc[3]);
        return s2[0] + s2[1];
    };
    const bool live = lane < K;
    const int pos = ((lane / 16) * 4 + (lane % 4)) * 4 + (lane % 16) / 4;
    const bool inrec = lane < KP;
    const T acc0 = inrec ? img[acc0_offset<C>(RT) + pos] * (C::HALF ? T(1) / (T(H_GIBBS_SCALE) * T(H_PANEL_SCALE)) : T(1)) : T(1);
    const T tau = T(p.tau);
    const int n_items = *n_items_ptr;
    const T kk = T(K) * T(K);
    for (;;) {
        int item = 0;
        if (lane == 0) item = __hip_atomic_fetch_add(head_ptr, 1, __ATOMIC_RELAXED, __HIP_MEMORY_SCOPE_AGENT);
        item = __builtin_amdgcn_readfirstlane(item);
        if (item >= n_items) break;
        const int q = p.list[item];
        const int i = p.row_begin + (q / N) * p.row_step, j = q % N;
        const T a = inrec ? Pt[(size_t)i * KP + pos] : T(0), b = inrec ? Pt[(size_t)j * KP + pos] : T(0);
        const T thr = Pt[(size_t)N * KP + j];
        T u = live ? T(1) / T(K) : T(0), v = u, ACC = acc0, errv = T(1);
        T ru = live ? T(1) : T(0), rv = ru;
        int ii = 0, chk = 1, flags = sizeof(T) == 8 ? FLAG_F64 : 0, abs_at = -1;
        for (;;) {
            v = b * C::rcp(ACC);
            T r1 = SYM ? matvec(g1, v) : matvec(g1, v);
            r1 = live ? r1 : T(1);
            u = a * C::rcp(r1);
            if constexpr (TRACK) {
                if (ballot_b(live && (u * ru > tau || v * rv > tau))) {
                    ru = live ? C::rcp(u * T(K)) : T(0);
                    rv = live ? T(K) * C::rcp(v) : T(0);
                    abs_at = ii;
                    flags |= FLAG_ABSORBED;
                    {
                        constexpr T BIG = sizeof(T) == 4 ? T(1.2676506e30) : T(8.452712498170644e270);
                        constexpr T SMALL = T(1) / BIG;
                        if (ballot_b(live && !(u >= SMALL && u < BIG && v >= SMALL && v < BIG))) u = T(__builtin_nanf(""));
                    }
                }
            } else {
                if (ballot_b(live && (u > tau || v > tau))) {
                    if (lane == 0) p.track_list[__hip_atomic_fetch_add(p.track_count, 1, __ATOMIC_RELAXED, __HIP_MEMORY_SCOPE_AGENT)] = q;
                    break;
                }
            }
            ++ii;
            if constexpr (SYM) ACC = matvec(g1, u); else ACC = matvec(g2, u);
            ACC = live ? ACC : T(1);
            const bool pending = ii == chk, capped = ii >= p.max_iter;
            if (pending) chk += p.period;
            if (pending || capped) {
                const T sc = (TRACK && abs_at == ii - 1) ? T(1) / kk : T(1);
                const T d = v * ACC * sc - b;
                const T e = sqrt(wave_sum(d * d));
                bool fin = capped;
                if (pending) {
                    errv = e;
                    if (e <= thr) { fin = true; flags |= FLAG_CONVERGED; }
                    else if (e != e) { fin = true; flags |= FLAG_NAN; }
                }
                if (fin) {
                    xline[lane] = v;
                    T val = T(0);
                    {
                        const T *gm = plain + 2 * 64 * WAVE + lane;
                        for (int k0 = 0; k0 < K; k0 += 8) {
                            T gk[8];
#pragma unroll
                            for (int e = 0; e < 8; ++e) gk[e] = gm[(k0 + e) * WAVE];
#pragma unroll
                            for (int e = 0; e < 8; ++e) val = fma(gk[e], xline[k0 + e], val);
                        }
                    }
                    val = wave_sum(live ? u * val : T(0));
                    if (TRACK && abs_at >= 0 && abs_at == ii - 1) { val *= T(1) / kk; flags |= FLAG_ABSORB_LAST; }
                    if (lane == 0) {
                        if (!(val - val == T(0))) flags |= FLAG_NAN;
                        if (p.fb_list && (flags & FLAG_NAN) && sizeof(T) == 4) {
                            p.fb_list[__hip_atomic_fetch_add(p.fb_count, 1, __ATOMIC_RELAXED, __HIP_MEMORY_SCOPE_AGENT)] = q;
                        } else if (p.nan_list && (flags & FLAG_NAN)) {
                            p.nan_list[__hip_atomic_fetch_add(p.nan_count, 1, __ATOMIC_RELAXED, __HIP_MEMORY_SCOPE_AGENT)] = q;
                        } else {
                            p.emd[q] = double(val);
                            if (p.iters) p.iters[q] = ii;
                            if (p.err) p.err[q] = double(errv);
                            p.flags[q] = flags;
                        }
                    }
                    break;
                }
            }
        }
    }
}

template <class C>
__global__ void __launch_bounds__(WAVE * WAVES_PER_WG) sinkhorn_solo_track_kernel(GridParams p) {
    extern __shared__ __attribute__((aligned(16))) unsigned char solo_track_smem[];
    switch ((p.K + C::TILE - 1) / C::TILE) {
    case 1: solo_pairs<C, true, 1, true>(p, solo_track_smem, p.list_len, p.queue_head); break;
    case 2: solo_pairs<C, true, 2, true>(p, solo_track_smem, p.list_len, p.queue_head); break;
    case 3: solo_pairs<C, true, 3, true>(p, solo_track_smem, p.list_len, p.queue_head); break;
    default: solo_pairs<C, true, 4, true>(p, solo_track_smem, p.list_len, p.queue_head); break;
    }
}

template <class C, int RT, bool V_PIECES = false>
__device__ inline __attribute__((always_inline)) void ring_flush_body(const typename C::T *ring, const GridParams &p, int cnt) {
    using M = C;
    using T = typename C::T;
    using acc_t = typename C::acc_t;
    constexpr int TILE = C::TILE, NREG = C::NREG, NGRP = C::NGRP;
    constexpr StreamLayout L = stream_layout(shape_of<C>(), RT, true, false, 0, 1, 0);
    constexpr int RSTRIDE = L.slot, PE = L.panel;
    const int lane = threadIdx.x % WAVE;
    const int col = lane % TILE, grp = lane / TILE;
    const T *img_gm = static_cast<const T *>(p.img) + 2 * form_elems<C>(RT);
    __builtin_amdgcn_fence(__ATOMIC_RELEASE, "workgroup");
    __builtin_amdgcn_wave_barrier();
    __builtin_amdgcn_fence(__ATOMIC_ACQUIRE, "workgroup");
    const int s = col < cnt ? col : cnt - 1;
    const T *rec = ring + s * RSTRIDE;
    const T scale = rec[2 * PE];
    T val = T(0), val1 = T(0);
    if constexpr (C::HALF) {
        constexpr int KB = split_kblocks(RT);
        SplitPanel<RT, 2> Bv;
        if constexpr (V_PIECES) {
#pragma unroll
            for (int part = 0; part < 2; ++part)
#pragma unroll
                for (int kb = 0; kb < KB; ++kb)
                    Bv.p[part][kb] = *reinterpret_cast<const u32x4_t *>(rec + PE + ((part * KB + kb) * NGRP + grp) * 4);
        } else {
            acc_t Vr[RT];
#pragma unroll
            for (int t = 0; t < RT; ++t) load_regs<C>(rec + PE + (t * NGRP + grp) * NREG, Vr[t]);
#pragma unroll
            for (int kb = 0; kb < KB; ++kb)
#pragma unroll
                for (int h = 0; h < 4; ++h) {
                    const int t = 2 * kb + h / 2, e = 2 * (h & 1);
                    unsigned int hi = 0u, lo = 0u;
                    if (t < RT) quot_pieces(float(Vr[t][e]), float(Vr[t][e + 1]), hi, lo);
                    Bv.p[0][kb][h] = hi; Bv.p[1][kb][h] = lo;
                }
        }
#pragma unroll
        for (int t = 0; t < RT; ++t) {
            acc_t zero;
#pragma unroll
            for (int r = 0; r < NREG; ++r) zero[r] = T(0);
            const acc_t w = split_tile_product<C, RT>(img_gm, lane, t, Bv, zero);
            using u32x2_t = unsigned int __attribute__((ext_vector_type(2)));
            const u32x2_t uh = *reinterpret_cast<const u32x2_t *>(rec + ((0 * KB + t / 2) * NGRP + grp) * 4 + 2 * (t & 1));
            const u32x2_t ul = *reinterpret_cast<const u32x2_t *>(rec + ((1 * KB + t / 2) * NGRP + grp) * 4 + 2 * (t & 1));
            val += pieces_sum_lo(uh[0], ul[0]) * w[0];
            val += pieces_sum_hi(uh[0], ul[0]) * w[1];
            val += pieces_sum_lo(uh[1], ul[1]) * w[2];
            val += pieces_sum_hi(uh[1], ul[1]) * w[3];
        }
    } else if constexpr (C::SPLIT) {
        SplitPanel<RT, C::NP> Bv;
        {
            acc_t Vr[RT];
#pragma unroll
            for (int t = 0; t < RT; ++t) load_regs<C>(rec + PE + (t * NGRP + grp) * NREG, Vr[t]);
            split_panel<C, RT>(Vr, Bv);
        }
        const T *img_gm1 = static_cast<const T *>(p.img) + band1_offset<C>(RT) + 2 * form_elems<C>(RT);
#pragma unroll
        for (int t = 0; t < RT; ++t) {
            acc_t zero;
#pragma unroll
            for (int r = 0; r < NREG; ++r) zero[r] = T(0);
            acc_t w = split_tile_product<C, RT>(img_gm, lane, t, Bv, zero);
            acc_t ur;
            load_regs<C>(rec + (t * NGRP + grp) * NREG, ur);
            if (p.bands == 2) {
                const acc_t w1 = split_tile_product<C, RT>(img_gm1, lane, t, Bv, zero);
#pragma unroll
                for (int r = 0; r < NREG; ++r) {
                    w[r] = fmaf(w1[r], BAND1_DOWN, w[r]);
                    val1 += ur[r] * (w1[r] * BAND1_DOWN);
                }
            }
#pragma unroll
            for (int r = 0; r < NREG; ++r) val += ur[r] * w[r];
        }
    } else {
        acc_t Vr[RT];
#pragma unroll
        for (int t = 0; t < RT; ++t) load_regs<C>(rec + PE + (t * NGRP + grp) * NREG, Vr[t]);
        const int n_last = (p.K - M::lidx(RT - 1, 0, 0) + NGRP - 1) / NGRP;
#pragma unroll
        for (int t = 0; t < RT; ++t) {
            acc_t w;
#pragma unroll
            for (int r = 0; r < NREG; ++r) w[r] = T(0);
#pragma unroll
            for (int tp = 0; tp < RT; ++tp)
#pragma unroll
                for (int r = 0; r < NREG; ++r)
                    if (tp < RT - 1 || r < n_last)
                        w = M::mfma(img_gm[((tp * NREG + r) * RT + t) * WAVE + lane], Vr[tp][r], w);
            acc_t ur;
            load_regs<C>(rec + (t * NGRP + grp) * NREG, ur);
#pragma unroll
            for (int r = 0; r < NREG; ++r) val += ur[r] * w[r];
        }
    }
    val = group_sum<C>(val) * scale;
    if constexpr (C::HALF) val *= T(1) / T(H_IN_SCALE);
    bool redo = p.fb_list && !(val - val == T(0));
    if constexpr (C::SPLIT && !C::HALF) {
        if (p.bands == 2 && p.fb_list) redo = redo || group_sum<C>(val1) * scale > T(0.25) * val;
    }
    if (grp == 0 && col < cnt) {
        const int *meta = reinterpret_cast<const int *>(rec + 2 * PE + 1);
        const int qq = meta[0];
        int fl = meta[1];
        if (redo || (p.fb_list && (fl & FLAG_NAN))) {
            p.fb_list[__hip_atomic_fetch_add(p.fb_count, 1, __ATOMIC_RELAXED, __HIP_MEMORY_SCOPE_AGENT)] = qq;
        } else if (p.nan_list && (!(val - val == T(0)) || (fl & FLAG_NAN))) {
            p.nan_list[__hip_atomic_fetch_add(p.nan_count, 1, __ATOMIC_RELAXED, __HIP_MEMORY_SCOPE_AGENT)] = qq;
        } else {
            if (val != val) fl |= FLAG_NAN;
            p.emd[qq] = double(val);
            p.flags[qq] = fl;
        }
    }
    __builtin_amdgcn_fence(__ATOMIC_RELEASE, "workgroup");
    __builtin_amdgcn_wave_barrier();
}
template <class C, int RT>
__device__ __attribute__((noinline)) void ring_flush(const typename C::T *ring, const GridParams &p, int cnt) {
    ring_flush_body<C, RT>(ring, p, cnt);
}
template <class C, int RT, bool TRACK> constexpr bool parked_flush() { return parked_flush(shape_of<C>(), RT, TRACK); }

#ifndef PILOT_AREG_MAX_RT
#define PILOT_AREG_MAX_RT 4
#endif
template <class C, int RT, bool SYM> constexpr bool operands_in_regs() { return operands_in_regs(shape_of<C>(), RT, SYM); }
template <class C, int RT, bool SYM, bool TRACK, int TV = 0> constexpr int min_waves_per_simd() { return min_waves_per_simd(shape_of<C>(), RT, SYM, TRACK, TV); }
template <class C, int RT, bool SYM, bool TRACK, int TV> constexpr bool solo_in_stream() { return solo_in_stream(shape_of<C>(), RT, SYM, TRACK, TV); }

template <class C, int RT, bool SYM, bool TRACK, int TV = 0>
__global__ void __launch_bounds__(WAVE * WAVES_PER_WG, (min_waves_per_simd<C, RT, SYM, TRACK, TV>()))
sinkhorn_stream_kernel(GridParams p) {
    using M = C;
    using T = typename C::T;
    using acc_t = typename M::acc_t;
    static_assert(!(C::HALF && TRACK), "the fp16-split configuration has no tracking variant (scalings beyond tau leave its scaled domain)");
    constexpr int TILE = M::TILE, NREG = M::NREG, NGRP = M::NGRP;
    constexpr int KP = RT * TILE, FORM = form_elems<C>(RT);
    constexpr StreamLayout L0 = stream_layout(shape_of<C>(), RT, SYM, TRACK, TV, 1, 0);
    constexpr int RSTRIDE = L0.slot;
    constexpr T PANEL_SCALE = C::HALF ? T(H_PANEL_SCALE) : T(1), IN_SCALE = C::HALF ? T(H_IN_SCALE) : T(1);
    extern __shared__ __attribute__((aligned(16))) unsigned char smem_raw[];
    T *lds = reinterpret_cast<T *>(smem_raw);

    int block = blockIdx.x;
    if constexpr (solo_in_stream<C, RT, SYM, TRACK, TV>()) {
        if (block < p.solo_blocks) { solo_pairs<C, SYM, RT>(p, smem_raw, p.solo_len, p.solo_head); return; }
        block -= p.solo_blocks;
    }
    const int n_items = p.list_len ? *p.list_len : p.n_pairs;
    const int lane = threadIdx.x % WAVE;
    if (block * WAVES_PER_WG * TILE >= n_items) return;

    const bool two_bands = C::SPLIT && TRACK && p.bands == 2;
    const int n_img = two_bands ? stream_layout(shape_of<C>(), RT, SYM, TRACK, TV, 2, 0).table : L0.table;
    {
        const T *g = static_cast<const T *>(p.img);
        constexpr int n_b0 = L0.table;
        for (int i = threadIdx.x; i < n_b0; i += WAVE * WAVES_PER_WG) lds[i] = g[i];
        if (two_bands)
            for (int i = threadIdx.x; i < n_b0; i += WAVE * WAVES_PER_WG) lds[n_b0 + i] = g[band1_offset<C>(RT) + i];
        for (int i = threadIdx.x; i < KP; i += WAVE * WAVES_PER_WG) lds[n_img + i] = g[acc0_offset<C>(RT) + i];
        if constexpr (TV > 0 && !C::SPLIT) {
            constexpr int n_form = TV * tail_steps<RT>() * WAVE * 2;
            const T *tg = g + tail_offset<C>(RT);
            for (int i = threadIdx.x; i < n_form; i += WAVE * WAVES_PER_WG) {
                lds[n_img + (L0.tail - L0.table) + i] = tg[i];
                if constexpr (!SYM) lds[n_img + (L0.tail - L0.table) + n_form + i] = tg[2 * tail_form_stride<RT>() + i];
            }
        }
    }
    __syncthreads();
    const T *img_gt = lds;
    const T *img_g = SYM ? lds : lds + FORM;
    T *ring = lds + n_img + (L0.rings - L0.table) + (threadIdx.x / WAVE) * p.ring * RSTRIDE;
    constexpr bool PARK = parked_flush<C, RT, TRACK>();
    constexpr int PARK_LANE = park_lane_elems<C>(RT);
    T *park = lds + n_img + (L0.park - L0.table) + WAVES_PER_WG * p.ring * RSTRIDE + (threadIdx.x / WAVE) * (PARK_LANE * WAVE) + (threadIdx.x % WAVE) * 4;
    static_assert(HANDOVER_FLUSH - 1 + C::TILE <= HANDOVER_BUF, "a wave's hand-over buffer must hold one flush level plus one tile of pairs");
    int *hb = reinterpret_cast<int *>(lds + n_img + (L0.hb - L0.table) + WAVES_PER_WG * p.ring * RSTRIDE) + (threadIdx.x / WAVE) * HANDOVER_BUF;
    int hb_cnt = 0;
    auto hb_flush = [&]() {
        int base = 0;
        if (lane == 0) base = __hip_atomic_fetch_add(p.track_count, hb_cnt, __ATOMIC_RELAXED, __HIP_MEMORY_SCOPE_AGENT);
        base = __builtin_amdgcn_readfirstlane(base);
        if (lane < hb_cnt) p.track_list[base + lane] = hb[lane];
        hb_cnt = 0;
    };
    constexpr int NA = RT * NREG * RT;
    constexpr bool GREG = operands_in_regs<C, RT, SYM>();
    AFromRegs<C, GREG ? NA : 1> areg;
    if constexpr (GREG) {
#pragma unroll
        for (int i = 0; i < NA; ++i) areg.a[i] = lds[i * WAVE + lane];
    }
    const AFromImage<C> a_gt{img_gt, lane}, a_g{img_g, lane};
    const T *acc0 = lds + n_img;
    const int col = lane % TILE, grp = lane / TILE;
    constexpr int NTF = (TV > 0 ? TV : 1) * tail_steps<RT>() * WAVE;
    const pair_of<T> *tl_base = reinterpret_cast<const pair_of<T> *>(acc0 + (L0.tail - L0.table));
    const TailFromImage<T, RT> w_gt{tl_base, lane}, w_g{SYM ? tl_base : tl_base + NTF, lane};
    TailFromRegs<T, RT, (GREG && TV > 0) ? TV : 0> wreg;
    if constexpr (GREG && TV > 0 && !C::SPLIT) {
#pragma unroll
        for (int i = 0; i < TV * tail_steps<RT>(); ++i) wreg.a[i] = tl_base[i * WAVE + lane];
    }
    auto dead = [](int t, int r) { return TV > 0 && t == RT - 1 && r > 0; };
    auto product = [&](const AFromImage<C> &a_img, const TailFromImage<T, RT> &w_img, const acc_t (&IN)[RT], acc_t (&OUT)[RT],
                       const acc_t &init) {
        if constexpr (C::SPLIT) {
            if constexpr (TRACK) panel_product_split<C, RT, (TV > 0)>(a_img.img, two_bands ? a_img.img + L0.table : nullptr, lane, IN, OUT, init);
            else panel_product_split<C, RT, (TV > 0)>(a_img.img, nullptr, lane, IN, OUT, init);
        } else if constexpr (TV > 0) {
            if constexpr (GREG) panel_product_tail<C, RT, TV>(areg, wreg, IN, OUT, init, grp);
            else panel_product_tail<C, RT, TV>(a_img, w_img, IN, OUT, init, grp);
        } else {
            if constexpr (GREG) panel_product<C, RT>(areg, IN, OUT, p.K, init);
            else panel_product<C, RT>(a_img, IN, OUT, p.K, init);
        }
    };

    const int K = p.K, N = p.N;
    const T *Pt = static_cast<const T *>(p.P) + (C::HALF ? (size_t)p.N * (RT * M::TILE) + p.N : 0);
    const T uinit = PANEL_SCALE / T(K);
    const T tau = T(p.tau) * PANEL_SCALE * (C::HALF ? T(1) - T(0.0009765625) : T(1));
    const T kk = T(K) * T(K);
    const unsigned long long colmask = (1ull << TILE) - 1ull;

    acc_t A[RT], B[RT], U[RT], V[RT], ACC[RT];
    acc_t RU[TRACK ? RT : 1], RV[TRACK ? RT : 1];
    constexpr int KB = split_kblocks(RT);
    constexpr bool LIVE1 = TV > 0;
    SplitPanel<RT, 2> PU, PV;
    constexpr bool AREG = C::HALF && SYM && RT <= PILOT_AREG_MAX_RT;
    SplitImage<AREG ? RT : 1, 2> AR;
    if constexpr (AREG) {
#pragma unroll
        for (int part = 0; part < 2; ++part)
#pragma unroll
            for (int kb = 0; kb < KB; ++kb)
#pragma unroll
                for (int t = 0; t < RT; ++t) AR.a[part][kb][t] = reinterpret_cast<const u32x4_t *>(lds)[((part * KB + kb) * RT + t) * WAVE + lane];
    }
    unsigned int pu0_hi = 0u, pu0_lo = 0u;
    if constexpr (C::HALF) { const Pieces<2> s0 = split_pair<C>(PANEL_SCALE / T(p.K), PANEL_SCALE / T(p.K)); pu0_hi = s0.p[0]; pu0_lo = s0.p[1]; }
    auto pieces_live = [](int kb, int h) { const int t = 2 * kb + h / 2; return t < RT && !(LIVE1 && t == RT - 1 && (h & 1)); };
    auto pad_mask = [&](int kb, int h, const acc_t &padc) -> unsigned int {
        const int t = 2 * kb + h / 2;
        if (t != RT - 1) return 0xffffffffu;
        const int e = 2 * (h & 1);
        return (padc[e] != T(0) ? 0u : 0x0000ffffu) | ((padc[e + 1] != T(0) || LIVE1) ? 0u : 0xffff0000u);
    };
    auto quot_panel = [&](const acc_t (&X)[RT], SplitPanel<RT, 2> &P) {
#pragma unroll
        for (int kb = 0; kb < KB; ++kb)
#pragma unroll
            for (int h = 0; h < 4; ++h) {
                const int t = 2 * kb + h / 2, e = 2 * (h & 1);
                unsigned int hi = 0u, lo = 0u;
                if (pieces_live(kb, h)) {
                    const int tt = t < RT ? t : 0;
                    quot_pieces(float(X[tt][e]), (LIVE1 && t == RT - 1) ? 0.f : float(X[tt][e + 1]), hi, lo);
                }
                P.p[0][kb][h] = hi; P.p[1][kb][h] = lo;
            }
    };
    acc_t PADC;
#pragma unroll
    for (int r = 0; r < NREG; ++r) PADC[r] = M::lidx(RT - 1, r, grp) >= K ? T(1) : T(0);
    auto product_h = [&](const T *form, const SplitPanel<RT, 2> &P, acc_t (&OUT)[RT]) {
        if constexpr (AREG) panel_product_pieces_regs<C, RT>(AR, P, OUT, PADC);
        else if constexpr (C::HALF) panel_product_pieces<C, RT>(form, nullptr, lane, P, OUT, PADC);
    };
    bool active = false;
    int q = 0, ii = 0, chk = 1, flags = 0, abs_at = -1;
    T errv = T(1), thr = T(0);
#pragma unroll
    for (int t = 0; t < RT; ++t)
#pragma unroll
        for (int r = 0; r < NREG; ++r) {
            A[t][r] = B[t][r] = U[t][r] = V[t][r] = T(0);
            ACC[t][r] = T(1);
            if constexpr (TRACK) { RU[t][r] = RV[t][r] = T(0); }
        }
#pragma unroll
    for (int part = 0; part < 2; ++part)
#pragma unroll
        for (int kb = 0; kb < KB; ++kb)
#pragma unroll
            for (int h = 0; h < 4; ++h) { PU.p[part][kb][h] = 0u; PV.p[part][kb][h] = 0u; }

    int ring_cnt = 0;
    auto flush = [&](int cnt) { ring_flush<C, RT>(ring, p, cnt); };

    int res_next = 0, res_end = 0, res_base = 0, qbatch = 0, ibatch = 0, jbatch = 0;
    bool exhausted = false, first_draw = true;
    const int wave_id = block * WAVES_PER_WG + (int)(threadIdx.x / WAVE);
    const int n_tile_waves = ((int)gridDim.x - (solo_in_stream<C, RT, SYM, TRACK, TV>() ? p.solo_blocks : 0)) * WAVES_PER_WG;
    const int queue_start = (solo_in_stream<C, RT, SYM, TRACK, TV>() && p.solo_len && p.solo_blocks > 0) ? *p.solo_len : 0;
    bool want = true;
    constexpr bool SHARDED_QUEUE = RT <= QUEUE_SHARD_MAX_RT;
    int qc = wave_id % QUEUE_SHARDS, q_tries = 0;
    const int q_max_tries = n_tile_waves >= QUEUE_SHARDS ? 4 : QUEUE_SHARDS;
    const bool hand_all_over = C::HALF && p.unequal && *p.unequal != 0;
    for (;;) {
        const unsigned long long wmask = ballot_b(want) & colmask;
        if (wmask) {
            if (res_next >= res_end && !exhausted) {
                int base = 0;
                if (first_draw) {
                    base = queue_start + wave_id * TILE;
                    first_draw = false;
                } else if (SHARDED_QUEUE && p.queue_shards) {
                    base = n_items;
                    while (q_tries < q_max_tries) {
                        int t = 0;
                        if (lane == 0) t = __hip_atomic_fetch_add(p.queue_shards + qc * QUEUE_SHARD_STRIDE, 1, __ATOMIC_RELAXED, __HIP_MEMORY_SCOPE_AGENT);
                        t = __builtin_amdgcn_readfirstlane(t);
                        const long b = (long)queue_start + ((long)n_tile_waves + qc + (long)QUEUE_SHARDS * t) * TILE;
                        if (b < n_items) { base = (int)b; q_tries = 0; break; }
                        ++q_tries;
                        qc = qc + 1 == QUEUE_SHARDS ? 0 : qc + 1;
                    }
                } else {
                    if (lane == 0) base = __hip_atomic_fetch_add(p.queue_head, TILE, __ATOMIC_RELAXED, __HIP_MEMORY_SCOPE_AGENT);
                    base = __builtin_amdgcn_readfirstlane(base) + n_tile_waves * TILE;
                }
                exhausted = base >= n_items;
                res_next = exhausted ? n_items : base;
                res_end = (base + TILE < n_items) ? base + TILE : n_items;
                if (exhausted) res_end = n_items;
                res_base = base;
                const int bi = base + col;
                qbatch = (p.list && bi < n_items) ? p.list[bi] : bi;
                const int qv = bi < n_items ? qbatch : 0;
                ibatch = p.row_begin + (qv / N) * p.row_step;
                jbatch = qv % N;
            }
            const int avail = res_end - res_next;
            const int n_want = (int)__popcll(wmask);
            const int rank = (int)__popcll(wmask & ((1ull << col) - 1ull));
            const int item = res_next + rank;
            const bool take = want && rank < avail;
            const int bsel = 4 * ((item - res_base) & (TILE - 1));
            const int qsel = __builtin_amdgcn_ds_bpermute(bsel, qbatch);
            const int isel = __builtin_amdgcn_ds_bpermute(bsel, ibatch), jsel = __builtin_amdgcn_ds_bpermute(bsel, jbatch);
            res_next = __builtin_amdgcn_readfirstlane(res_next + (n_want < avail ? n_want : avail));
            if (want && !take && exhausted) {
                want = false;
#pragma unroll
                for (int t = 0; t < RT; ++t)
#pragma unroll
                    for (int r = 0; r < NREG; ++r) { A[t][r] = B[t][r] = U[t][r] = V[t][r] = T(0); ACC[t][r] = T(1); }
                if constexpr (C::HALF) {
#pragma unroll
                    for (int part = 0; part < 2; ++part)
#pragma unroll
                        for (int kb = 0; kb < KB; ++kb)
#pragma unroll
                            for (int h = 0; h < 4; ++h) { PU.p[part][kb][h] = 0u; PV.p[part][kb][h] = 0u; }
                }
            }
            if (take) {
                want = false;
                active = true;
                q = qsel;
                const int i = isel, j = jsel;
                const T *pa = Pt + (size_t)i * KP + grp * NREG, *pb = Pt + (size_t)j * KP + grp * NREG;
#pragma unroll
                for (int t = 0; t < RT; ++t) {
                    load_regs<C>(pa + t * NGRP * NREG, A[t]);
                    load_regs<C>(pb + t * NGRP * NREG, B[t]);
                }
                thr = Pt[(size_t)N * KP + j];
#pragma unroll
                for (int t = 0; t < RT; ++t) {
                    load_regs<C>(acc0 + (t * NGRP + grp) * NREG, ACC[t]);
#pragma unroll
                    for (int r = 0; r < NREG; ++r) {
                        U[t][r] = (t == RT - 1) ? uinit - uinit * PADC[r] : uinit;
                        if constexpr (TRACK) { RU[t][r] = T(1); RV[t][r] = T(1); }
                    }
                }
                if constexpr (C::HALF) {
#pragma unroll
                    for (int kb = 0; kb < KB; ++kb)
#pragma unroll
                        for (int h = 0; h < 4; ++h)
                            if (pieces_live(kb, h)) {
                                const unsigned int m = pad_mask(kb, h, PADC);
                                PU.p[0][kb][h] = pu0_hi & m; PU.p[1][kb][h] = pu0_lo & m;
                            }
                }
                chk = 1;
                ii = 0; flags = 0; abs_at = -1; errv = T(1);
            }
            if constexpr (C::HALF) {
                if (hand_all_over) {
                    const unsigned long long tm = ballot_b(take) & colmask;
                    if (tm) {
                        int base = 0;
                        if (lane == 0) base = __hip_atomic_fetch_add(p.track_count, (int)__popcll(tm), __ATOMIC_RELAXED, __HIP_MEMORY_SCOPE_AGENT);
                        base = __builtin_amdgcn_readfirstlane(base);
                        if (take && grp == 0) p.track_list[base + __popcll(tm & ((1ull << col) - 1ull))] = q;
                    }
                    if (take) { active = false; want = true; }
                }
            }
        }
        if (ballot_b(active || want) == 0ull) break;

        T mx = T(0);
        if constexpr (C::HALF) {
#pragma unroll
            for (int t = 0; t < RT; ++t)
#pragma unroll
                for (int r = 0; r < NREG; ++r) V[t][r] = dead(t, r) ? T(0) : B[t][r] * M::rcp(ACC[t][r]);
            quot_panel(V, PV);
            unsigned int m2 = 0u;
            {
                unsigned int pend = 0u;
                bool have = false;
#pragma unroll
                for (int kb = 0; kb < KB; ++kb)
#pragma unroll
                    for (int h = 0; h < 4; ++h)
                        if (pieces_live(kb, h)) {
                            if (have) { m2 = pk_max3_f16(m2, pend, PV.p[0][kb][h]); have = false; }
                            else { pend = PV.p[0][kb][h]; have = true; }
                        }
                if (have) m2 = pk_max3_f16(m2, pend, pend);
            }
            product_h(a_g.img, PV, ACC);
            {
                acc_t X[RT];
#pragma unroll
                for (int t = 0; t < RT; ++t)
#pragma unroll
                    for (int r = 0; r < NREG; ++r) X[t][r] = dead(t, r) ? T(0) : A[t][r] * M::rcp(ACC[t][r]);
                quot_panel(X, PU);
            }
            {
                unsigned int pend = 0u;
                bool have = false;
#pragma unroll
                for (int kb = 0; kb < KB; ++kb)
#pragma unroll
                    for (int h = 0; h < 4; ++h)
                        if (pieces_live(kb, h)) {
                            if (have) { m2 = pk_max3_f16(m2, pend, PU.p[0][kb][h]); have = false; }
                            else { pend = PU.p[0][kb][h]; have = true; }
                        }
                if (have) m2 = pk_max3_f16(m2, pend, pend);
            }
            const f16x2_t mh = __builtin_bit_cast(f16x2_t, m2);
            const float m0 = float(mh[0]), m1 = float(mh[1]);
            mx = (m0 <= tau && m1 <= tau) ? fmax(m0, m1) : __builtin_inff();
        } else {
#pragma unroll
        for (int t = 0; t < RT; ++t)
#pragma unroll
            for (int r = 0; r < NREG; ++r) {
                if (dead(t, r)) continue;
                V[t][r] = B[t][r] * M::rcp(ACC[t][r]);
            }
        product(a_g, w_g, V, ACC, PADC);
#pragma unroll
        for (int t = 0; t < RT; ++t)
#pragma unroll
            for (int r = 0; r < NREG; ++r) {
                if (dead(t, r)) continue;
                const T un = A[t][r] * M::rcp(ACC[t][r]);
                U[t][r] = un;
                if constexpr (TRACK) mx = fmax(fmax(mx, un * RU[t][r]), V[t][r] * RV[t][r]);
                else mx = fmax(fmax(mx, un), V[t][r]);
            }
        }
        const unsigned long long omask = column_any_mask<C>(active && mx > tau);
        const bool over = (omask >> col) & 1ull;
        if constexpr (TRACK) {
            if (over) {
#pragma unroll
                for (int t = 0; t < RT; ++t)
#pragma unroll
                    for (int r = 0; r < NREG; ++r) {
                        const bool pad = M::lidx(t, r, grp) >= K;
                        RU[t][r] = pad ? T(0) : M::rcp(U[t][r] * T(K));
                        RV[t][r] = pad ? T(0) : T(K) * M::rcp(V[t][r]);
                    }
                abs_at = ii;
                flags |= FLAG_ABSORBED;
            }
            if (omask) {
                constexpr T BIG = sizeof(T) == 4 ? T(1.2676506e30) : T(8.452712498170644e270);
                constexpr T SMALL = T(1) / BIG;
                bool z = false;
#pragma unroll
                for (int t = 0; t < RT; ++t)
#pragma unroll
                    for (int r = 0; r < NREG; ++r)
                        z = z || (M::lidx(t, r, grp) < K && !(U[t][r] >= SMALL && U[t][r] < BIG && V[t][r] >= SMALL && V[t][r] < BIG));
                const unsigned long long zmask = column_any_mask<C>(over && z);
                if ((zmask >> col) & 1ull) U[0][0] = __builtin_nanf("");
            }
        }
        auto hand_over = [&]() {
            if (omask) {
                if (over) {
                    if (grp == 0) hb[hb_cnt + (int)__popcll(omask & ((1ull << col) - 1ull))] = q;
                    active = false;
                    want = true;
                }
                hb_cnt += (int)__popcll(omask);
                if (hb_cnt >= HANDOVER_FLUSH) hb_flush();
            }
        };
        if constexpr (!TRACK && !(C::HALF && PILOT_DEFER_HANDOVER)) hand_over();
        ++ii;

        if constexpr (C::HALF) product_h(a_gt.img, PU, ACC);
        else product(a_gt, w_gt, U, ACC, PADC);
        if constexpr (!TRACK && C::HALF && PILOT_DEFER_HANDOVER) hand_over();

        const bool pending = active && ii == chk;
        if (pending) chk += p.period;
        const bool capped = active && ii >= p.max_iter;
        auto lane_e2 = [&](T sc) {
            T e2 = T(0);
            if constexpr (PILOT_E2_PACKED && sizeof(T) == 4 && !TRACK && NREG == 4) {
                using P2 = pair_of<float>;
                P2 acc2 = {0.f, 0.f};
#pragma unroll
                for (int t = 0; t < RT; ++t)
#pragma unroll
                    for (int h = 0; h < 2; ++h) {
                        const int r0 = 2 * h, r1 = 2 * h + 1;
                        if (dead(t, r0) && dead(t, r1)) continue;
                        if (dead(t, r0) || dead(t, r1)) {
                            const int r = dead(t, r0) ? r1 : r0;
                            const float d = V[t][r] * ACC[t][r] - B[t][r];
                            acc2[0] = __builtin_fmaf(d, d, acc2[0]);
                            continue;
                        }
                        const P2 v2 = {V[t][r0], V[t][r1]}, a2 = {ACC[t][r0], ACC[t][r1]}, b2 = {B[t][r0], B[t][r1]};
                        const P2 d2 = __builtin_elementwise_fma(v2, a2, -b2);
                        acc2 = __builtin_elementwise_fma(d2, d2, acc2);
                    }
                return acc2[0] + acc2[1];
            }
#pragma unroll
            for (int t = 0; t < RT; ++t) {
                T et = T(0);
#pragma unroll
                for (int r = 0; r < NREG; ++r) {
                    if (dead(t, r)) continue;
                    T d;
                    if constexpr (TRACK) d = V[t][r] * ACC[t][r] * sc - B[t][r];
                    else d = V[t][r] * ACC[t][r] - B[t][r];
                    et += d * d;
                }
                e2 += et;
            }
            return e2;
        };
        constexpr bool E2_EARLY = C::SPLIT && !TRACK && PILOT_E2_EARLY;
        T e2_early = T(0);
        if constexpr (E2_EARLY) e2_early = lane_e2(T(1));
        if (ballot_b(pending || capped)) {
            T sc = T(1);
            if constexpr (TRACK) sc = (abs_at == ii - 1) ? T(1) / kk : T(1);
            T e2 = E2_EARLY ? e2_early : lane_e2(sc);
            e2 = group_sum<C>(e2);
            const T e = sqrt(e2);
            bool fin = capped;
            if (pending) {
                errv = e;
                if (e <= thr) { fin = true; flags |= FLAG_CONVERGED; }
                else if (e != e) { fin = true; flags |= FLAG_NAN; }
            }
            unsigned long long fmask = ballot_b(fin) & colmask;
            if (fmask) {
                T scale = T(1);
                if constexpr (TRACK) {
                    if (fin && abs_at >= 0 && abs_at == ii - 1) { scale = T(1) / kk; flags |= FLAG_ABSORB_LAST; }
                }
                if constexpr (sizeof(T) == 8) flags |= FLAG_F64;
                if (fin && grp == 0) {
                    if (p.iters) p.iters[q] = ii;
                    if (p.err) p.err[q] = double(errv) * double(T(1) / IN_SCALE);
                }
                while (fmask) {
                    if constexpr (PARK) {
                        if (ring_cnt > 0 && ring_cnt + (int)__popcll(fmask) > p.ring) {
                            if constexpr (C::HALF) {
#pragma unroll
                                for (int part = 0; part < 2; ++part)
#pragma unroll
                                    for (int kb = 0; kb < KB; ++kb) *reinterpret_cast<u32x4_t *>(park + (part * KB + kb) * 4 * WAVE) = PU.p[part][kb];
                            } else {
#pragma unroll
                            for (int t = 0; t < RT; ++t) store_regs<C>(park + t * NREG * WAVE, U[t]);
                            }
                            ring_flush_body<C, RT>(ring, p, ring_cnt);
                            ring_cnt = 0;
                            __builtin_amdgcn_fence(__ATOMIC_ACQUIRE, "workgroup");
                            const int i = p.row_begin + (q / N) * p.row_step, j = q % N;
                            const T *pa = Pt + (size_t)i * KP + grp * NREG, *pb = Pt + (size_t)j * KP + grp * NREG;
                            if constexpr (C::HALF) {
#pragma unroll
                                for (int part = 0; part < 2; ++part)
#pragma unroll
                                    for (int kb = 0; kb < KB; ++kb) PU.p[part][kb] = *reinterpret_cast<const u32x4_t *>(park + (part * KB + kb) * 4 * WAVE);
                            }
#pragma unroll
                            for (int t = 0; t < RT; ++t) {
                                if constexpr (!C::HALF) load_regs<C>(park + t * NREG * WAVE, U[t]);
#pragma unroll
                                for (int r = 0; r < NREG; ++r) { A[t][r] = T(0); B[t][r] = T(0); }
                                if (active) {
                                    load_regs<C>(pa + t * NGRP * NREG, A[t]);
                                    load_regs<C>(pb + t * NGRP * NREG, B[t]);
                                }
                            }
                            if constexpr (C::HALF) product_h(a_gt.img, PU, ACC);
                            else product(a_gt, w_gt, U, ACC, PADC);
                        }
                    }
                    const int space = p.ring - ring_cnt;
                    const int rank = (int)__popcll(fmask & ((1ull << col) - 1ull));
                    const bool put = fin && ((fmask >> col) & 1ull) && rank < space;
                    if (put) {
                        T *rec = ring + (ring_cnt + rank) * RSTRIDE;
                        constexpr int PE = L0.panel;
                        if constexpr (C::HALF) {
#pragma unroll
                            for (int part = 0; part < 2; ++part)
#pragma unroll
                                for (int kb = 0; kb < KB; ++kb)
                                    *reinterpret_cast<u32x4_t *>(rec + ((part * KB + kb) * NGRP + grp) * 4) = PU.p[part][kb];
                            static_assert(!C::HALF || PE >= RT * C::TILE, "the v half of a ring slot holds f32 values");
#pragma unroll
                            for (int t = 0; t < RT; ++t) store_regs<C>(rec + PE + (t * NGRP + grp) * NREG, V[t]);
                        } else {
#pragma unroll
                        for (int t = 0; t < RT; ++t) {
                            store_regs<C>(rec + (t * NGRP + grp) * NREG, U[t]);
                            store_regs<C>(rec + PE + (t * NGRP + grp) * NREG, V[t]);
                        }
                        }
                        if (grp == 0) {
                            rec[2 * PE] = scale;
                            int *meta = reinterpret_cast<int *>(rec + 2 * PE + 1);
                            meta[0] = q;
                            meta[1] = flags;
                        }
                    }
                    const unsigned long long taken = ballot_b(put) & colmask;
                    fmask &= ~taken;
                    ring_cnt = __builtin_amdgcn_readfirstlane(ring_cnt + (int)__popcll(taken));
                    if constexpr (!PARK) {
                        if (ring_cnt >= p.ring) { flush(ring_cnt); ring_cnt = 0; }
                    }
                }
                if (fin) { active = false; want = true; }
            }
        }
    }
    if (ring_cnt > 0) {
        if constexpr (PARK) ring_flush_body<C, RT>(ring, p, ring_cnt);
        else flush(ring_cnt);
    }
    if constexpr (!TRACK) {
        if (hb_cnt > 0) hb_flush();
    }
}

__device__ inline unsigned short bf16_bits(float x) {
    return __builtin_bit_cast(unsigned short, static_cast<__bf16>(x));
}
__device__ inline unsigned short f16_bits(float x) {
    return __builtin_bit_cast(unsigned short, static_cast<_Float16>(x));
}
template <class C>
__device__ inline void write_split_forms(const double *__restrict__ Msrc, int K, int RT, double reg, float *__restrict__ img,
                                         bool two_bands, int tid, int nthr) {
    using M = C;
    const int nimg = form_elems<C>(RT);
    const int KB = split_kblocks(RT);
    unsigned short *im16 = reinterpret_cast<unsigned short *>(img);
    for (int idx = tid; idx < KB * RT * WAVE * 8; idx += nthr) {
        const int e = idx % 8;
        int rest = idx / 8;
        const int lane = rest % WAVE; rest /= WAVE;
        const int t = rest % RT;
        const int kb = rest / RT;
        const int orow = M::lidx_of_row(t, lane % M::TILE);
        const int kt = 2 * kb + e / 4;
        const int k = kt < RT ? M::lidx(kt, e % 4, lane / M::TILE) : K;
        float f[3] = {0.f, 0.f, 0.f}, f1[3] = {0.f, 0.f, 0.f};
        if (orow < K && k < K) {
            const double m_ko = Msrc[(size_t)k * K + orow], m_ok = Msrc[(size_t)orow * K + k];
            const double sc = C::HALF ? double(H_GIBBS_SCALE) : 1.0;
            f[0] = float(exp(-m_ko / reg) * sc);
            f[1] = float(exp(-m_ok / reg) * sc);
            f[2] = float(exp(-m_ok / reg) * m_ok * sc);
            if (two_bands) {
                if (f[0] < SPLIT_SAFE_MIN) { f1[0] = float(exp(-m_ko / reg + BAND1_UP_LN)); f[0] = 0.f; }
                if (f[1] < SPLIT_SAFE_MIN) {
                    f1[1] = float(exp(-m_ok / reg + BAND1_UP_LN));
                    f1[2] = float(exp(-m_ok / reg + BAND1_UP_LN) * m_ok);
                    f[1] = 0.f; f[2] = 0.f;
                }
            }
        }
        if (two_bands) {
            unsigned short *im1 = reinterpret_cast<unsigned short *>(img + band1_offset<C>(RT));
#pragma unroll
            for (int form = 0; form < 3; ++form) {
                float x = f1[form];
#pragma unroll
                for (int part = 0; part < C::NP; ++part) {
                    const unsigned short hb = bf16_bits(x);
                    im1[(size_t)form * nimg * 2 + ((((size_t)part * KB + kb) * RT + t) * WAVE + lane) * 8 + e] = hb;
                    x -= __uint_as_float((unsigned int)hb << 16);
                }
            }
        }
#pragma unroll
        for (int form = 0; form < 3; ++form) {
            float x = f[form];
#pragma unroll
            for (int part = 0; part < C::NP; ++part) {
                unsigned short hb;
                if constexpr (C::HALF) { hb = f16_bits(x); x -= float(__builtin_bit_cast(_Float16, hb)); }
                else { hb = bf16_bits(x); x -= __uint_as_float((unsigned int)hb << 16); }
                im16[(size_t)form * nimg * 2 + ((((size_t)part * KB + kb) * RT + t) * WAVE + lane) * 8 + e] = hb;
            }
        }
    }
}
template <class C>
__device__ inline void write_first_product(const double *__restrict__ Msrc, int K, int RT, double reg, typename C::T *__restrict__ tab,
                                           double scale, int tid, int nthr) {
    using M = C;
    using T = typename C::T;
    const int KP = RT * M::TILE;
    for (int idx = tid; idx < 4 * KP; idx += nthr) {
        const int part = idx & 3, slot = idx >> 2;
        const int r = slot % M::NREG;
        const int g = (slot / M::NREG) % M::NGRP;
        const int t = slot / (M::NGRP * M::NREG);
        const int j = M::lidx(t, r, g);
        double s = 0.0;
        if (j < K)
            for (int k = part; k < K; k += 4) s += exp(-Msrc[(size_t)k * K + j] / reg);
        s += __shfl_xor(s, 1);
        s += __shfl_xor(s, 2);
        if (part == 0) tab[slot] = T(j < K ? s / K * scale : 1.0);
    }
}

template <class C>
__device__ inline void setup_body(const double *__restrict__ Msrc, int K, int RT, double reg,
                                  typename C::T *__restrict__ img, const double *__restrict__ Psrc,
                                  typename C::T *__restrict__ Pdst, long n_p, int write_tail, double stop_thr,
                                  double floor_ulps, int tid, int nthr, int *unequal = nullptr) {
    using M = C;
    using T = typename C::T;
    const int KP = RT * M::TILE;
    const int nimg = form_elems<C>(RT);
    if constexpr (C::SPLIT) {
        write_split_forms<C>(Msrc, K, RT, reg, img, (write_tail & 4) != 0, tid, nthr);
        if constexpr (C::HALF) {
            write_split_forms<CfgS32x16>(Msrc, K, RT, reg, img + track_img_offset<C>(RT), false, tid, nthr);
            write_first_product<CfgS32x16>(Msrc, K, RT, reg, img + track_img_offset<C>(RT) + acc0_offset<CfgS32x16>(RT), 1.0, tid, nthr);
        }
    } else {
    for (int idx = tid; idx < nimg; idx += nthr) {
        const int lane = idx % WAVE;
        int rest = idx / WAVE;
        const int t = rest % RT; rest /= RT;
        const int r = rest % M::NREG;
        const int tp = rest / M::NREG;
        const int orow = M::lidx_of_row(t, lane % M::TILE);
        const int k = M::lidx(tp, r, lane / M::TILE);
        double gt = 0.0, g = 0.0, gm = 0.0;
        if (orow < K && k < K) {
            const double m_ko = Msrc[(size_t)k * K + orow], m_ok = Msrc[(size_t)orow * K + k];
            gt = exp(-m_ko / reg);
            g = exp(-m_ok / reg);
            gm = g * m_ok;
        }
        img[idx] = T(gt);
        img[nimg + idx] = T(g);
        img[2 * nimg + idx] = T(gm);
    }
    }
    write_first_product<C>(Msrc, K, RT, reg, img + acc0_offset<C>(RT), C::HALF ? double(H_GIBBS_SCALE) * double(H_PANEL_SCALE) : 1.0, tid, nthr);
    if (write_tail & 2) {
        T *plain = img + plain_offset<C>(RT);
        for (int idx = tid; idx < 3 * 64 * WAVE; idx += nthr) {
            const int lane = idx % WAVE, k = (idx / WAVE) % 64, tbl = idx / (64 * WAVE);
            double v = 0.0;
            if (k < K && lane < K) {
                if (tbl == 1) v = exp(-Msrc[(size_t)k * K + lane] / reg);
                else v = exp(-Msrc[(size_t)lane * K + k] / reg);
                if (tbl == 2) v *= Msrc[(size_t)lane * K + k];
            }
            plain[idx] = T(v);
        }
    }
    if (write_tail & 1) {
        const int nst = (RT - 1) * 4 + 1;
        T *tail = img + tail_offset<C>(RT);
        for (int idx = tid; idx < 2 * 2 * nst * WAVE * 2; idx += nthr) {
            const int h = idx & 1;
            int rest = idx >> 1;
            const int lane = rest % WAVE; rest /= WAVE;
            const int st = rest % nst; rest /= nst;
            const int c = rest & 1, form = rest >> 1;
            const int row = M::lidx(RT - 1, 0, 2 * c + h);
            const int k = M::lidx(st / M::NREG, st % M::NREG, lane / M::TILE);
            double v = 0.0;
            if (row < K && k < K) v = form == 0 ? exp(-Msrc[(size_t)k * K + row] / reg) : exp(-Msrc[(size_t)row * K + k] / reg);
            tail[idx] = T(v);
        }
    }
    double mass0 = 0.0;
    for (int k = 0; k < K; ++k) mass0 += Psrc[k];
    for (long row = tid; row < n_p / KP; row += nthr) {
        double n2 = 0.0, mass = 0.0;
        for (int k = 0; k < K; ++k) { n2 += Psrc[row * K + k] * Psrc[row * K + k]; mass += Psrc[row * K + k]; }
        if (unequal && !(fabs(mass - mass0) <= 1e-6 * fabs(mass0))) atomicOr(unequal, 1);
        double thr = stop_thr;
        if (sizeof(T) == 4) { const double fl = floor_ulps * 1.1920928955078125e-07 * sqrt(n2); thr = thr > fl ? thr : fl; }
        Pdst[n_p + row] = T(thr);
        if constexpr (C::HALF) Pdst[(n_p + n_p / KP) + n_p + row] = T(thr) * T(H_IN_SCALE);
    }
    for (long idx = tid; idx < n_p; idx += nthr) {
        const long row = idx / KP;
        const int sidx = (int)(idx % KP);
        const int r = sidx % M::NREG, g = (sidx / M::NREG) % M::NGRP, t = sidx / (M::NGRP * M::NREG);
        const int l = M::lidx(t, r, g);
        Pdst[idx] = l < K ? T(Psrc[row * K + l]) : T(0);
        if constexpr (C::HALF) Pdst[(n_p + n_p / KP) + idx] = l < K ? T(Psrc[row * K + l]) * T(H_IN_SCALE) : T(0);
    }
}


__device__ inline int lds_count_aggregated(int *counters, int b, bool valid) {
    int slot = 0;
    unsigned long long todo = ballot_b(valid);
    while (todo) {
        const int leader = __builtin_ctzll(todo);
        const int b0 = __builtin_amdgcn_readlane(b, leader);
        const unsigned long long same = ballot_b(valid && b == b0);
        const int lane = threadIdx.x % WAVE;
        int base = 0;
        if (lane == leader) base = atomicAdd(&counters[b0], (int)__popcll(same));
        base = __builtin_amdgcn_readlane(base, leader);
        if (valid && b == b0) slot = base + (int)__popcll(same & ((1ull << lane) - 1ull));
        todo &= ~same;
    }
    return slot;
}

constexpr int ORDER_JW = 128, ORDER_RI = 8;

__device__ inline void bucket_body(int tile, const double *__restrict__ Psrc, int N, int K, int n_rows, int row_begin,
                                   int row_step, unsigned char *__restrict__ bucket, int *__restrict__ hist, int collapse,
                                   unsigned char *order_smem) {
    const int K4 = (K + 3) & ~3;
    float *Bt = reinterpret_cast<float *>(order_smem);
    float *Ar = Bt + (size_t)K4 * (ORDER_JW + 1);
    int *lh = reinterpret_cast<int *>(Ar + ORDER_RI * K4);
    const int n_jb = (N + ORDER_JW - 1) / ORDER_JW;
    const int jb = (tile % n_jb) * ORDER_JW, rb = (tile / n_jb) * ORDER_RI;
    const int nj = N - jb < ORDER_JW ? N - jb : ORDER_JW;
    const int nr = n_rows - rb < ORDER_RI ? n_rows - rb : ORDER_RI;
    for (int e = threadIdx.x; e < ORDER_NB; e += blockDim.x) lh[e] = 0;
    for (int e = threadIdx.x; e < nj * K; e += blockDim.x) {
        const int row = e / K, k = e % K;
        Bt[k * (ORDER_JW + 1) + row] = float(Psrc[(size_t)jb * K + e]);
    }
    for (int e = threadIdx.x; e < (K4 - K) * ORDER_JW; e += blockDim.x) Bt[(K + e / ORDER_JW) * (ORDER_JW + 1) + e % ORDER_JW] = 0.f;
    for (int e = threadIdx.x; e < ORDER_RI * K4; e += blockDim.x) {
        const int r = e / K4, k = e % K4;
        Ar[e] = (r < nr && k < K) ? float(Psrc[(size_t)(row_begin + (rb + r) * row_step) * K + k]) : 0.f;
    }
    __syncthreads();
    constexpr int R = ORDER_RI / 2;
    const int jl = threadIdx.x % ORDER_JW, half = threadIdx.x / ORDER_JW;
    float l1[R];
#pragma unroll
    for (int r = 0; r < R; ++r) l1[r] = 0.f;
    using f4 = float __attribute__((ext_vector_type(4)));
    for (int k = 0; k < K4; k += 4) {
        float bv[4];
#pragma unroll
        for (int e = 0; e < 4; ++e) bv[e] = Bt[(k + e) * (ORDER_JW + 1) + jl];
#pragma unroll
        for (int r = 0; r < R; ++r) {
            const f4 av = *reinterpret_cast<const f4 *>(Ar + (half * R + r) * K4 + k);
#pragma unroll
            for (int e = 0; e < 4; ++e) l1[r] += fabsf(av[e] - bv[e]);
        }
    }
#pragma unroll
    for (int r = 0; r < R; ++r) {
        const int rr = rb + half * R + r;
        const bool valid = jl < nj && half * R + r < nr;
        int b = ORDER_NB - 1;
        if (l1[r] > 0.f) {
            const float v = 4.f * (1.f - log2f(l1[r]));
            b = v < 0.f ? 0 : (v > float(ORDER_NB - 2) ? ORDER_NB - 2 : int(v));
            if (collapse) b = 0;
        } else if (row_begin + rr * row_step != jb + jl) {
            b = ORDER_NB - 2;
        }
        if (valid) bucket[(size_t)rr * N + jb + jl] = (unsigned char)b;
        (void)lds_count_aggregated(lh, b, valid);
    }
    __syncthreads();
    for (int i = threadIdx.x; i < ORDER_NB; i += blockDim.x) if (lh[i]) atomicAdd(&hist[i], lh[i]);
}

constexpr int PREP_SETUP_BLOCKS = 64;
template <class C>
__global__ void __launch_bounds__(256) sinkhorn_prep_kernel(const double *__restrict__ Msrc, int K, int RT, double reg,
                                                            typename C::T *__restrict__ img, const double *__restrict__ Psrc,
                                                            typename C::T *__restrict__ Pdst, int N, int write_tail, double stop_thr,
                                                            double floor_ulps, int n_tiles,
                                                            int n_rows, int row_begin, int row_step,
                                                            unsigned char *__restrict__ bucket, int *__restrict__ hist, int collapse) {
    extern __shared__ __attribute__((aligned(16))) unsigned char order_smem[];
    if ((int)blockIdx.x < n_tiles) {
        bucket_body(blockIdx.x, Psrc, N, K, n_rows, row_begin, row_step, bucket, hist, collapse, order_smem);
    } else {
        setup_body<C>(Msrc, K, RT, reg, img, Psrc, Pdst, (long)N * RT * C::TILE, write_tail, stop_thr, floor_ulps,
                      ((int)blockIdx.x - n_tiles) * (int)blockDim.x + (int)threadIdx.x, PREP_SETUP_BLOCKS * (int)blockDim.x,
                      hist - (CTRL_ORDER_HIST - CTRL_UNEQUAL));
    }
}

static __global__ void order_scatter_kernel(const unsigned char *__restrict__ bucket, int n_items, const int *__restrict__ hist,
                                     int *__restrict__ cursor, int *__restrict__ list, int *__restrict__ split,
                                     int *__restrict__ main_queue_head, int solo_mode) {
    __shared__ int offs[ORDER_NB], lh[ORDER_NB], lbase[ORDER_NB], gh[ORDER_NB];
    if (threadIdx.x < ORDER_NB) { lh[threadIdx.x] = 0; gh[threadIdx.x] = hist[threadIdx.x]; }
    __syncthreads();
    if (threadIdx.x < ORDER_NB) {
        int run = 0;
        for (int b = ORDER_NB - 1; b > (int)threadIdx.x; --b) run += gh[b];
        offs[threadIdx.x] = run;
    }
    if (blockIdx.x == 0 && threadIdx.x == 64) {
        const int n_dup = (solo_mode & 2) ? gh[ORDER_NB - 1] : 0;
        for (int i = 0; i < CTRL_SPLIT_INTS; ++i) split[i] = n_dup;
        *main_queue_head = n_dup;
    }
    __syncthreads();
    const int chunk = (n_items + gridDim.x - 1) / gridDim.x;
    const int q0 = blockIdx.x * chunk, q1 = (q0 + chunk < n_items) ? q0 + chunk : n_items;
    const int n_it = (q1 - q0 + (int)blockDim.x - 1) / (int)blockDim.x;
    for (int it = 0; it < n_it; ++it) {
        const int q = q0 + it * blockDim.x + threadIdx.x;
        const bool valid = q < q1;
        (void)lds_count_aggregated(lh, valid ? bucket[q] : 0, valid);
    }
    __syncthreads();
    if (threadIdx.x < ORDER_NB) {
        const int c = lh[threadIdx.x];
        lbase[threadIdx.x] = offs[threadIdx.x] + (c ? atomicAdd(&cursor[threadIdx.x], c) : 0);
        lh[threadIdx.x] = 0;
    }
    __syncthreads();
    for (int it = 0; it < n_it; ++it) {
        const int q = q0 + it * blockDim.x + threadIdx.x;
        const bool valid = q < q1;
        const int b = valid ? bucket[q] : 0;
        const int slot = lds_count_aggregated(lh, b, valid);
        if (valid) list[lbase[b] + slot] = q;
    }
}

}
```

pilot_amd/csrc/sinkhorn_launch.hpp:

```cpp
#pragma once
#include <hip/hip_runtime.h>
#include "sinkhorn_kernels.hpp"

namespace pilot {

constexpr bool same_shape(CfgShape a, CfgShape b) {
    return a.w == b.w && a.nreg == b.nreg && a.split == b.split && a.half == b.half && a.np == b.np && a.tile == b.tile && a.ngrp == b.ngrp;
}
static_assert(same_shape(shape_of(CFG_F32), shape_of<CfgF32x16>()) && same_shape(shape_of(CFG_F64), shape_of<CfgF64x16>()) &&
              same_shape(shape_of(CFG_S32), shape_of<CfgS32x16>()) && same_shape(shape_of(CFG_H32), shape_of<CfgH32x16>()),
              "shape_of(cfg) in sinkhorn_layout.hpp must state the traits of the kernels' configuration structs");

hipError_t launch_stream_f32(int RT, bool sym, bool track, dim3 grid, size_t lds, hipStream_t s, const GridParams &p);
hipError_t launch_stream_f64(int RT, bool sym, bool track, dim3 grid, size_t lds, hipStream_t s, const GridParams &p);
hipError_t launch_solo_track_f64(dim3 grid, hipStream_t s, const GridParams &p);
hipError_t launch_stream_s32(int RT, bool sym, bool track, int live1, dim3 grid, size_t lds, hipStream_t s, const GridParams &p);
hipError_t launch_stream_h32(int RT, bool sym, int live1, dim3 grid, size_t lds, hipStream_t s, const GridParams &p);
hipError_t launch_stream_tv(int cfg, int tv, int RT, bool sym, bool track, dim3 grid, size_t lds, hipStream_t s, const GridParams &p);
hipError_t launch_prep(int cfg, const double *M, int K, int RT, double reg, void *img, const double *P, void *Pslot, int N, int write_tail,
                       double stop_thr, double floor_ulps, int n_rows, int row_begin, int row_step, unsigned char *bucket, int *hist, int *list, int *split,
                       int *main_queue_head, int mode, int n_blocks, hipStream_t s);
hipError_t launch_wide(dim3 grid, hipStream_t s, const GridParams &p, float *rec);
hipError_t launch_wide_value(dim3 grid, hipStream_t s, const GridParams &p, const float *rec);
size_t wide_rec_elems();
hipError_t launch_quad(dim3 grid, hipStream_t s, const GridParams &p);
size_t img_elems(int cfg, int RT);
size_t track_img_elems(int cfg, int RT);

}
```

pilot_amd/csrc/sinkhorn_layout.hpp:

```cpp
#pragma once
#include <cstddef>
#include <cstdio>

#include "../../include/pilot_ot.h"

namespace pilot {

constexpr int WAVE = 64, WAVES_PER_WG = 4;
constexpr size_t LDS_BYTES = 160 * 1024;
constexpr int HANDOVER_BUF = 32, HANDOVER_FLUSH = 16;
constexpr int RING_MAX = 16, GREG_MAX = 64;
constexpr int min_of(int a, int b) { return a < b ? a : b; }
#ifndef PILOT_SPLIT_OCC2_MAX_RT
#define PILOT_SPLIT_OCC2_MAX_RT 4
#endif
#ifndef PILOT_SPLIT_OCC2_MAX_RT_TRACK
#define PILOT_SPLIT_OCC2_MAX_RT_TRACK 4
#endif
#ifndef PILOT_HALF_OCC2_MAX_RT
#define PILOT_HALF_OCC2_MAX_RT 7
#endif
#ifndef PILOT_HALF_SOLO_MIN_RT
#define PILOT_HALF_SOLO_MIN_RT 1
#endif
constexpr int HALF_SOLO_MIN_RT = PILOT_HALF_SOLO_MIN_RT, HALF_OCC4_MAX_RT = 2;
constexpr int SPLIT_OCC2_MAX_RT = PILOT_SPLIT_OCC2_MAX_RT, SPLIT_OCC2_MAX_RT_TRACK = PILOT_SPLIT_OCC2_MAX_RT_TRACK, HALF_OCC2_MAX_RT = PILOT_HALF_OCC2_MAX_RT;

enum { CFG_F32 = 0, CFG_F64 = 1, CFG_S32 = 2, CFG_H32 = 3 };
struct CfgShape { int w, nreg; bool split, half; int np, tile, ngrp; };
constexpr CfgShape shape_of(int cfg) {
    return cfg == CFG_H32 ? CfgShape{1, 4, true, true, 2, 16, 4}
                          : (cfg == CFG_S32 ? CfgShape{1, 4, true, false, 3, 16, 4} : CfgShape{cfg == CFG_F64 ? 2 : 1, 4, false, false, 0, 16, 4});
}

constexpr int tail_steps(int RT) { return (RT - 1) * 4 + 1; }
constexpr bool operands_in_regs(CfgShape c, int RT, bool sym) { return !c.split && sym && RT * c.nreg * RT * c.w <= GREG_MAX; }
constexpr int panel_regs(CfgShape c, int RT, bool sym, bool track, int tv) {
    return (track ? 7 : 5) * RT * c.nreg * c.w + c.nreg * c.w + 56 +
           (tv > 0 ? 24 * c.w : 0) +
           (c.split ? 3 * ((RT + 1) / 2) * 4 + 24 : 0) +
           (operands_in_regs(c, RT, sym) ? (RT * c.nreg * RT + 2 * tv * tail_steps(RT)) * c.w : 0);
}
constexpr int min_waves_per_simd(CfgShape c, int RT, bool sym, bool track, int tv) {
    if (c.half && !track && RT <= HALF_OCC4_MAX_RT) return 4;
    if (c.split) return RT <= (track ? SPLIT_OCC2_MAX_RT_TRACK : (c.half ? HALF_OCC2_MAX_RT : SPLIT_OCC2_MAX_RT)) ? 2 : 1;
    const int regs = panel_regs(c, RT, sym, track, tv);
    return regs <= 128 ? 4 : (regs <= 168 ? 3 : (regs <= 256 ? 2 : 1));
}
constexpr bool solo_in_stream(CfgShape c, int RT, bool sym, bool track, int tv) {
    const int mw = min_waves_per_simd(c, RT, sym, track, tv);
    const int budget = mw >= 4 ? 128 : (mw == 3 ? 168 : 256);
    return !track && sym && RT <= 4 && !(c.half && RT < HALF_SOLO_MIN_RT) && (64 + 45) * c.w <= budget;
}
constexpr int form_elems(CfgShape c, int RT) { return c.split ? c.np * ((RT + 1) / 2) * RT * WAVE * 4 : RT * c.tile * RT * c.tile; }
constexpr int ring_panel_elems(CfgShape c, int RT) { return c.half ? 2 * ((RT + 1) / 2) * c.ngrp * 4 : RT * c.tile; }
constexpr int ring_slot_stride(CfgShape c, int RT) { return 2 * ring_panel_elems(c, RT) + 4; }
constexpr bool parked_flush(CfgShape c, int RT, bool track) { return c.split && !track && RT <= 4; }
constexpr int park_lane_elems(CfgShape c, int RT) { return c.half ? 2 * ((RT + 1) / 2) * 4 : RT * c.nreg; }
constexpr int tail_weight_elems(CfgShape c, int RT, bool sym, int tv) { return (tv > 0 && !c.split) ? (sym ? 1 : 2) * tv * tail_steps(RT) * WAVE * 2 : 0; }
constexpr int handover_elems(CfgShape c) { return WAVES_PER_WG * HANDOVER_BUF / c.w; }
struct StreamLayout {
    int table, tail, rings, park, hb, end;
    int slot, panel;
    size_t bytes;
};
constexpr StreamLayout stream_layout(CfgShape c, int RT, bool sym, bool track, int tv, int bands, int ring) {
    StreamLayout l{};
    l.table = (sym ? 1 : 2) * form_elems(c, RT) * ((c.split && track && bands == 2) ? 2 : 1);
    l.tail = l.table + RT * c.tile;
    l.rings = l.tail + tail_weight_elems(c, RT, sym, tv);
    l.panel = ring_panel_elems(c, RT); l.slot = ring_slot_stride(c, RT);
    l.park = l.rings + WAVES_PER_WG * ring * l.slot;
    l.hb = l.park + (parked_flush(c, RT, track) ? WAVES_PER_WG * park_lane_elems(c, RT) * WAVE : 0);
    l.end = l.hb + (track ? 0 : handover_elems(c));
    l.bytes = (size_t)l.end * 4 * c.w;
    return l;
}
struct StreamLds { size_t bytes; int ring, wgs_per_cu; };
constexpr StreamLds stream_lds(CfgShape c, int RT, bool sym, bool track, int tv, int bands, size_t inherited, int want, int min_ring = 4) {
    const size_t fixed = stream_layout(c, RT, sym, track, tv, bands, 0).bytes + inherited;
    const size_t slots = stream_layout(c, RT, sym, track, tv, bands, 1).bytes + inherited - fixed;
    for (;; --want) {
        const size_t budget = LDS_BYTES / (size_t)want;
        const int ring = budget > fixed ? min_of((int)((budget - fixed) / slots), RING_MAX) : 0;
        if (ring >= min_ring || want == 1) return {fixed + slots * (size_t)(ring < 1 ? 1 : ring), ring, want};
    }
}
constexpr int ORDER_NB = 48;
constexpr int QUEUE_SHARDS = 32, QUEUE_SHARD_STRIDE = 32;
enum : int {
    CTRL_TRACK_LEN = 0,
    CTRL_GENERIC_HEAD = 0,
    CTRL_HEAD_FAST = 1,
    CTRL_HEAD_TRACK = 2,
    CTRL_HEAD_SOLO = 3,
    CTRL_SPLIT = 4,
    CTRL_SPLIT_INTS = 4,
    CTRL_SOLO_LEN = CTRL_SPLIT + 3,
    CTRL_FB_LEN = 8,
    CTRL_FB_HEAD = 9,
    CTRL_NAN_LEN = 10,
    CTRL_NAN_HEAD = 11,
    CTRL_UNEQUAL = 12,
    CTRL_INTS = 16,
    CTRL_ORDER_HIST = CTRL_INTS,
    CTRL_SHARDS_AT = (CTRL_ORDER_HIST + 2 * ORDER_NB + 31) / 32 * 32,
    CTRL_SHARDS_TRACK_AT = CTRL_SHARDS_AT + QUEUE_SHARDS * QUEUE_SHARD_STRIDE,
    CTRL_BLOCK_INTS = CTRL_SHARDS_TRACK_AT + QUEUE_SHARDS * QUEUE_SHARD_STRIDE,
    CTRL_NONE = -1,
};
enum : int {
    DBG_NATURAL_ORDER = 2,
    DBG_WGS_SHIFT = 4,
    DBG_NO_TAIL_ROWS = 256,
    DBG_NO_SOLO = 512,
    DBG_NO_NAN_PASS = 1024,
    DBG_NO_SOLO_F64 = 2048,
    DBG_NO_REDO64 = 4096,
    DBG_NO_TRACK_ALL = 8192,
};
struct SinkhornSwitches {
    int debug;
    int no_quad;
    int generic_wgs;
    bool operator==(const SinkhornSwitches &o) const { return debug == o.debug && no_quad == o.no_quad && generic_wgs == o.generic_wgs; }
};

constexpr int QUAD_MIN_K = 113, QUAD_MAX_K = 128;
constexpr bool quad_covers(int K, bool sym) { return sym && K >= QUAD_MIN_K && K <= QUAD_MAX_K; }
constexpr int clamp_wgs(int n_cu, int per_cu, int tiles) { return min_of(n_cu * per_cu, (tiles + WAVES_PER_WG - 1) / WAVES_PER_WG); }
enum PairList { LIST_ORDER, LIST_TRACK, LIST_FB };
struct PassPlan {
    bool run = false, track = false, quad = false, solo_f64 = false;
    int cfg = 0, tv = 0, live1 = 0;
    int bands = 1;
    size_t inherited = 0;
    StreamLds lds = {};
    int wgs = 0, solo_blocks = 0;
    PairList list = LIST_ORDER;
    int len_slot = CTRL_NONE, head_slot = CTRL_NONE, shards_at = CTRL_NONE;
};
struct GridPasses {
    int rc = PILOT_OT_OK;
    char msg[160] = "";
    int mode = 0, write_tail = 0, ob = 0;
    PassPlan fast, track, f64;
};
inline GridPasses plan_grid(int cfg, int N, int K, int n_rows, bool sym, bool mixed, double max_cost_over_reg, int n_cu, const SinkhornSwitches &sw) {
    GridPasses g;
    const CfgShape fast = shape_of(cfg);
    const bool half = fast.half, split = fast.split;
    const int TILE = 16, RT = (K + TILE - 1) / TILE, n_tail = K - (RT - 1) * TILE, debug = sw.debug;
    const int live1 = (split && RT >= 2 && RT <= 4 && n_tail <= 4) ? 1 : 0;
    int tv = (!split && RT >= 2 && RT <= 7 && n_tail <= 4 && !(debug & DBG_NO_TAIL_ROWS)) ? (n_tail <= 2 ? 1 : 2) : 0;
    if (tv && stream_layout(fast, RT, sym, false, tv, 1, 4).bytes > LDS_BYTES) tv = 0;
    const bool redo64 = !mixed && split && max_cost_over_reg > 12.0 && !(debug & DBG_NO_REDO64);
    const bool track_all = mixed || (split && !half && max_cost_over_reg > 24.0 && !(debug & DBG_NO_TRACK_ALL));
    const int tv_fast = split ? live1 : tv;
    const long full_tiles = ((long)N * N + TILE - 1) / TILE, wave_slots = (long)n_cu * min_waves_per_simd(fast, RT, sym, false, tv_fast) * WAVES_PER_WG;
    const bool solo = solo_in_stream(fast, RT, sym, false, tv_fast) && !(debug & DBG_NO_SOLO) && !track_all && full_tiles < 3 * wave_slots;
    const int n_pairs = n_rows * N, tiles = (n_pairs + TILE - 1) / TILE;
    PassPlan &f = g.fast, &t = g.track, &d = g.f64;
    f.run = !track_all; f.cfg = cfg; f.tv = tv; f.live1 = live1; f.quad = half && quad_covers(K, sym) && !sw.no_quad;  f.head_slot = CTRL_HEAD_FAST; f.shards_at = CTRL_SHARDS_AT;
    t.run = t.track = true; t.cfg = split ? (int)CFG_S32 : cfg; t.tv = RT <= 4 ? tv : 0; t.live1 = live1; t.bands = mixed ? 2 : 1;
    t.head_slot = CTRL_HEAD_TRACK; t.shards_at = CTRL_SHARDS_TRACK_AT; if (!track_all) { t.list = LIST_TRACK; t.len_slot = CTRL_TRACK_LEN; }
    const CfgShape tracking = shape_of(t.cfg);
    t.inherited = ((size_t)handover_elems(tracking) + tail_weight_elems(tracking, RT, sym, tv) - tail_weight_elems(tracking, RT, sym, t.tv)) * 4 * tracking.w;
    d.run = mixed || redo64; d.track = true; d.cfg = CFG_F64; d.solo_f64 = sym && K <= 64 && !(debug & DBG_NO_SOLO_F64);
    d.list = mixed ? LIST_TRACK : LIST_FB; d.len_slot = CTRL_FB_LEN; d.head_slot = CTRL_FB_HEAD;
    g.rc = PILOT_OT_ENOTSUP;
    t.lds = stream_lds(tracking, RT, sym, true, t.tv, t.bands, t.inherited, min_waves_per_simd(tracking, RT, sym, true, split ? live1 : t.tv));
    if (!t.lds.ring) { snprintf(g.msg, sizeof g.msg, "K=%d with a %ssymmetric cost needs %zu B of LDS (> %zu) in this precision", K, sym ? "" : "non-", t.lds.bytes, LDS_BYTES); return g; }
    if (f.run && !f.quad) {
        int want = min_waves_per_simd(fast, RT, sym, false, tv_fast);
        if (half && K <= 4 && want > 2) want = 2;
        if ((debug >> DBG_WGS_SHIFT) & 7) want = (debug >> DBG_WGS_SHIFT) & 7;
        f.lds = stream_lds(fast, RT, sym, false, tv, 1, 0, want);
        if (!f.lds.ring) { snprintf(g.msg, sizeof g.msg, "K=%d: operand images + ring + park area exceed LDS", K); return g; }
    }
    if (d.run && !d.solo_f64) {
        d.lds = stream_lds(shape_of(CFG_F64), RT, sym, true, 0, 1, 0, min_waves_per_simd(shape_of(CFG_F64), RT, sym, true, 0));
        if (!d.lds.ring) { snprintf(g.msg, sizeof g.msg, "K=%d: the f64 fallback needs %zu B of LDS", K, d.lds.bytes); return g; }
    }
    g.rc = PILOT_OT_OK;
    if (n_rows == 0) { f.run = t.run = d.run = false; return g; }
    g.ob = min_of((n_pairs + 1023) / 1024, n_cu);
    g.mode = (solo ? 2 : 0) | ((debug & DBG_NATURAL_ORDER) ? 4 : 0);
    g.write_tail = (tv ? 1 : 0) | 2 | (mixed ? 4 : 0);
    if (solo) f.solo_blocks = min_of((n_rows + WAVES_PER_WG - 1) / WAVES_PER_WG, n_cu);
    f.wgs = f.quad ? min_of(2 * n_cu, tiles) : clamp_wgs(n_cu, f.lds.wgs_per_cu, tiles) + f.solo_blocks;
    t.wgs = clamp_wgs(n_cu, t.lds.wgs_per_cu, tiles);
    d.wgs = d.solo_f64 ? 64 : clamp_wgs(n_cu, d.lds.wgs_per_cu, tiles);
    return g;
}

}
```

pilot_amd/csrc/sk_inst.hip:

```cpp
#include "sinkhorn_launch.hpp"

namespace pilot {
namespace {

template <class C, int RT, bool SYM, bool TRACK, int TV = 0>
hipError_t stream_one(dim3 grid, size_t lds, hipStream_t s, const GridParams &p) {
    auto kern = sinkhorn_stream_kernel<C, RT, SYM, TRACK, TV>;
    if (lds > 32 * 1024) {
        hipError_t e = hipFuncSetAttribute(reinterpret_cast<const void *>(kern), hipFuncAttributeMaxDynamicSharedMemorySize, (int)lds);
        if (e != hipSuccess) return e;
    }
    hipLaunchKernelGGL(kern, grid, dim3(WAVE * WAVES_PER_WG), lds, s, p);
    return hipGetLastError();
}
template <class C, int RT, int TV, int MAX_RT>
hipError_t stream_rt(bool sym, bool track, dim3 grid, size_t lds, hipStream_t s, const GridParams &p) {
    if constexpr (RT > MAX_RT || (TV > 0 && RT == 1)) return hipErrorInvalidValue;
    else {
        if constexpr (C::HALF) { if (track) return hipErrorInvalidValue; }
        else if (track) return sym ? stream_one<C, RT, true, true, TV>(grid, lds, s, p) : stream_one<C, RT, false, true, TV>(grid, lds, s, p);
        return sym ? stream_one<C, RT, true, false, TV>(grid, lds, s, p) : stream_one<C, RT, false, false, TV>(grid, lds, s, p);
    }
}
template <class C, int TV = 0, int MAX_RT = 8>
hipError_t stream_any(int RT, bool sym, bool track, dim3 grid, size_t lds, hipStream_t s, const GridParams &p) {
    switch (RT) {
    case 1: return stream_rt<C, 1, TV, MAX_RT>(sym, track, grid, lds, s, p);
    case 2: return stream_rt<C, 2, TV, MAX_RT>(sym, track, grid, lds, s, p);
    case 3: return stream_rt<C, 3, TV, MAX_RT>(sym, track, grid, lds, s, p);
    case 4: return stream_rt<C, 4, TV, MAX_RT>(sym, track, grid, lds, s, p);
    case 5: return stream_rt<C, 5, TV, MAX_RT>(sym, track, grid, lds, s, p);
    case 6: return stream_rt<C, 6, TV, MAX_RT>(sym, track, grid, lds, s, p);
    case 7: return stream_rt<C, 7, TV, MAX_RT>(sym, track, grid, lds, s, p);
    case 8: return stream_rt<C, 8, TV, MAX_RT>(sym, track, grid, lds, s, p);
    default: return hipErrorInvalidValue;
    }
}

template <class C>
hipError_t prep_any(const double *M, int K, int RT, double reg, void *img, const double *P, void *Pslot, int N, int write_tail,
                    double stop_thr, double floor_ulps, int n_rows, int row_begin, int row_step, unsigned char *bucket, int *hist, int *list, int *split,
                    int *main_queue_head, int mode, int n_blocks, hipStream_t s) {
    using T = typename C::T;
    const int collapse = (mode >> 2) & 1;
    const int tiles = n_rows > 0 ? ((N + ORDER_JW - 1) / ORDER_JW) * ((n_rows + ORDER_RI - 1) / ORDER_RI) : 0;
    const int K4 = (K + 3) & ~3;
    const size_t lds = sizeof(float) * ((size_t)K4 * (ORDER_JW + 1) + (size_t)ORDER_RI * K4) + sizeof(int) * ORDER_NB;
    static bool attr_set[64] = {};
    int dev = 0;
    if (hipGetDevice(&dev) != hipSuccess || dev < 0 || dev >= 64) dev = 0;
    if (!attr_set[dev]) {
        hipError_t e = hipFuncSetAttribute(reinterpret_cast<const void *>(sinkhorn_prep_kernel<C>),
                                           hipFuncAttributeMaxDynamicSharedMemorySize, 150 * 1024);
        if (e != hipSuccess) return e;
        attr_set[dev] = true;
    }
    hipLaunchKernelGGL(sinkhorn_prep_kernel<C>, dim3(tiles + PREP_SETUP_BLOCKS), dim3(256), lds, s, M, K, RT, reg, static_cast<T *>(img), P,
                       static_cast<T *>(Pslot), N, write_tail, stop_thr, floor_ulps, tiles, n_rows, row_begin, row_step, bucket, hist, collapse);
    if (n_rows > 0)
        hipLaunchKernelGGL(order_scatter_kernel, dim3(n_blocks), dim3(256), 0, s, bucket, n_rows * N, hist, hist + ORDER_NB, list, split,
                           main_queue_head, mode & 3);
    return hipGetLastError();
}
}

#if SK_PART == 0
hipError_t launch_stream_f32(int RT, bool sym, bool track, dim3 grid, size_t lds, hipStream_t s, const GridParams &p) {
    return stream_any<CfgF32x16>(RT, sym, track, grid, lds, s, p);
}
hipError_t launch_prep_f64(const double *M, int K, int RT, double reg, void *img, const double *P, void *Pslot, int N, int write_tail,
                           double stop_thr, double floor_ulps, int n_rows, int row_begin, int row_step, unsigned char *bucket, int *hist, int *list, int *split,
                           int *main_queue_head, int mode, int n_blocks, hipStream_t s);
hipError_t launch_prep_s32(const double *M, int K, int RT, double reg, void *img, const double *P, void *Pslot, int N, int write_tail,
                           double stop_thr, double floor_ulps, int n_rows, int row_begin, int row_step, unsigned char *bucket, int *hist, int *list, int *split,
                           int *main_queue_head, int mode, int n_blocks, hipStream_t s);
hipError_t launch_prep_h32(const double *M, int K, int RT, double reg, void *img, const double *P, void *Pslot, int N, int write_tail,
                           double stop_thr, double floor_ulps, int n_rows, int row_begin, int row_step, unsigned char *bucket, int *hist, int *list, int *split,
                           int *main_queue_head, int mode, int n_blocks, hipStream_t s);
hipError_t launch_prep(int cfg, const double *M, int K, int RT, double reg, void *img, const double *P, void *Pslot, int N, int write_tail,
                       double stop_thr, double floor_ulps, int n_rows, int row_begin, int row_step, unsigned char *bucket, int *hist, int *list, int *split,
                       int *main_queue_head, int mode, int n_blocks, hipStream_t s) {
    if (cfg == CFG_F64)
        return launch_prep_f64(M, K, RT, reg, img, P, Pslot, N, write_tail, stop_thr, floor_ulps, n_rows, row_begin, row_step, bucket, hist, list, split,
                               main_queue_head, mode, n_blocks, s);
    if (cfg == CFG_H32)
        return launch_prep_h32(M, K, RT, reg, img, P, Pslot, N, write_tail, stop_thr, floor_ulps, n_rows, row_begin, row_step, bucket, hist, list, split,
                               main_queue_head, mode, n_blocks, s);
    if (cfg == CFG_S32)
        return launch_prep_s32(M, K, RT, reg, img, P, Pslot, N, write_tail, stop_thr, floor_ulps, n_rows, row_begin, row_step, bucket, hist, list, split,
                               main_queue_head, mode, n_blocks, s);
    return prep_any<CfgF32x16>(M, K, RT, reg, img, P, Pslot, N, write_tail, stop_thr, floor_ulps, n_rows, row_begin, row_step, bucket, hist, list, split,
                               main_queue_head, mode, n_blocks, s);
}
size_t track_img_elems(int cfg, int RT) { return cfg == CFG_H32 ? (size_t)track_img_offset<CfgH32x16>(RT) : 0; }
size_t img_elems(int cfg, int RT) {
    if (cfg == CFG_H32) return (size_t)img_total<CfgH32x16>(RT);
    return cfg == CFG_S32 ? (size_t)img_total<CfgS32x16>(RT) : (cfg == CFG_F64 ? (size_t)img_total<CfgF64x16>(RT) : (size_t)img_total<CfgF32x16>(RT));
}
#define PILOT_TV_DECL(NAME) \
    hipError_t launch_stream_##NAME(int RT, bool sym, bool track, dim3 grid, size_t lds, hipStream_t s, const GridParams &p);
PILOT_TV_DECL(f32_tv1) PILOT_TV_DECL(f32_tv2) PILOT_TV_DECL(f64_tv1) PILOT_TV_DECL(f64_tv2)
#undef PILOT_TV_DECL
hipError_t launch_stream_tv(int cfg, int tv, int RT, bool sym, bool track, dim3 grid, size_t lds, hipStream_t s, const GridParams &p) {
    if (cfg == CFG_F32) return tv == 1 ? launch_stream_f32_tv1(RT, sym, track, grid, lds, s, p) : launch_stream_f32_tv2(RT, sym, track, grid, lds, s, p);
    return tv == 1 ? launch_stream_f64_tv1(RT, sym, track, grid, lds, s, p) : launch_stream_f64_tv2(RT, sym, track, grid, lds, s, p);
}
#elif SK_PART == 1
hipError_t launch_stream_f64(int RT, bool sym, bool track, dim3 grid, size_t lds, hipStream_t s, const GridParams &p) {
    return stream_any<CfgF64x16>(RT, sym, track, grid, lds, s, p);
}
hipError_t launch_solo_track_f64(dim3 grid, hipStream_t s, const GridParams &p) {
    hipLaunchKernelGGL(sinkhorn_solo_track_kernel<CfgF64x16>, grid, dim3(WAVE * WAVES_PER_WG), sizeof(double) * WAVE * WAVES_PER_WG, s, p);
    return hipGetLastError();
}
hipError_t launch_prep_f64(const double *M, int K, int RT, double reg, void *img, const double *P, void *Pslot, int N, int write_tail,
                           double stop_thr, double floor_ulps, int n_rows, int row_begin, int row_step, unsigned char *bucket, int *hist, int *list, int *split,
                           int *main_queue_head, int mode, int n_blocks, hipStream_t s) {
    return prep_any<CfgF64x16>(M, K, RT, reg, img, P, Pslot, N, write_tail, stop_thr, floor_ulps, n_rows, row_begin, row_step, bucket, hist, list, split,
                               main_queue_head, mode, n_blocks, s);
}
#elif SK_PART == 7
hipError_t launch_stream_s32_l1(int RT, bool sym, bool track, dim3 grid, size_t lds, hipStream_t s, const GridParams &p) {
    return stream_any<CfgS32x16, 1>(RT, sym, track, grid, lds, s, p);
}
#elif SK_PART == 9
hipError_t launch_stream_h32_l1(int RT, bool sym, dim3 grid, size_t lds, hipStream_t s, const GridParams &p) {
    return stream_any<CfgH32x16, 1, 4>(RT, sym, false, grid, lds, s, p);
}
#elif SK_PART == 8
hipError_t launch_stream_h32_l1(int RT, bool sym, dim3 grid, size_t lds, hipStream_t s, const GridParams &p);
hipError_t launch_stream_h32(int RT, bool sym, int live1, dim3 grid, size_t lds, hipStream_t s, const GridParams &p) {
    if (live1) return launch_stream_h32_l1(RT, sym, grid, lds, s, p);
    return stream_any<CfgH32x16>(RT, sym, false, grid, lds, s, p);
}
hipError_t launch_prep_h32(const double *M, int K, int RT, double reg, void *img, const double *P, void *Pslot, int N, int write_tail,
                           double stop_thr, double floor_ulps, int n_rows, int row_begin, int row_step, unsigned char *bucket, int *hist, int *list, int *split,
                           int *main_queue_head, int mode, int n_blocks, hipStream_t s) {
    return prep_any<CfgH32x16>(M, K, RT, reg, img, P, Pslot, N, write_tail, stop_thr, floor_ulps, n_rows, row_begin, row_step, bucket, hist, list, split,
                               main_queue_head, mode, n_blocks, s);
}
#elif SK_PART == 6
hipError_t launch_stream_s32_l1(int RT, bool sym, bool track, dim3 grid, size_t lds, hipStream_t s, const GridParams &p);
hipError_t launch_stream_s32(int RT, bool sym, bool track, int live1, dim3 grid, size_t lds, hipStream_t s, const GridParams &p) {
    if (live1) return launch_stream_s32_l1(RT, sym, track, grid, lds, s, p);
    return stream_any<CfgS32x16>(RT, sym, track, grid, lds, s, p);
}
hipError_t launch_prep_s32(const double *M, int K, int RT, double reg, void *img, const double *P, void *Pslot, int N, int write_tail,
                           double stop_thr, double floor_ulps, int n_rows, int row_begin, int row_step, unsigned char *bucket, int *hist, int *list, int *split,
                           int *main_queue_head, int mode, int n_blocks, hipStream_t s) {
    return prep_any<CfgS32x16>(M, K, RT, reg, img, P, Pslot, N, write_tail, stop_thr, floor_ulps, n_rows, row_begin, row_step, bucket, hist, list, split,
                               main_queue_head, mode, n_blocks, s);
}
#else
#if SK_PART == 2
#define PILOT_TV_CFG CfgF32x16
#define PILOT_TV_N 1
#define PILOT_TV_NAME(x) x##f32_tv1
#elif SK_PART == 3
#define PILOT_TV_CFG CfgF32x16
#define PILOT_TV_N 2
#define PILOT_TV_NAME(x) x##f32_tv2
#elif SK_PART == 4
#define PILOT_TV_CFG CfgF64x16
#define PILOT_TV_N 1
#define PILOT_TV_NAME(x) x##f64_tv1
#else
#define PILOT_TV_CFG CfgF64x16
#define PILOT_TV_N 2
#define PILOT_TV_NAME(x) x##f64_tv2
#endif
hipError_t PILOT_TV_NAME(launch_stream_)(int RT, bool sym, bool track, dim3 grid, size_t lds, hipStream_t s, const GridParams &p) {
    return stream_any<PILOT_TV_CFG, PILOT_TV_N>(RT, sym, track, grid, lds, s, p);
}
#endif

}
```

pilot_amd/csrc/wide_kernels.hpp:

```cpp
#pragma once
#include "sinkhorn_kernels.hpp"

namespace pilot {

constexpr int WIDE_WAVES = 8, WIDE_RT = 16, WIDE_KB = 8, WIDE_KP = 256, WIDE_MAX_K = 256;
constexpr int WIDE_PE = ring_panel_elems<CfgH32x16>(WIDE_RT);
constexpr int WIDE_REC = ring_slot_stride<CfgH32x16>(WIDE_RT);

__global__ void __launch_bounds__(WAVE * WIDE_WAVES, 2) sinkhorn_wide_kernel(GridParams p, float *__restrict__ rec_base) {
    using C = CfgH32x16;
    using acc_t = C::acc_t;
    constexpr int TILE = C::TILE, NREG = C::NREG, NGRP = C::NGRP, KB = WIDE_KB, RT = WIDE_RT, KP = WIDE_KP;
    __shared__ u32x4_t PB[2][KB][2][WAVE];
    __shared__ int ovc[2][TILE];
    __shared__ float red_e2[2][WIDE_WAVES][TILE];
    __shared__ int sh_base[2];
    const int wave = threadIdx.x / WAVE, lane = threadIdx.x % WAVE, col = lane % TILE, grp = lane / TILE;
    const int K = p.K, N = p.N, n_items = p.n_pairs;
    const int KBL = (K + 31) / 32;
    const bool live_wave = 2 * wave * TILE < K;
    const float *img = static_cast<const float *>(p.img);
    const float *Pt = static_cast<const float *>(p.P);
    const float *acc0 = img + acc0_offset<C>(RT);
    const float uinit = H_PANEL_SCALE / float(K), tau = float(p.tau) * H_PANEL_SCALE;
    const unsigned long long colmask = (1ull << TILE) - 1ull;

    u32x4_t AR[2][KB][2];
#pragma unroll
    for (int part = 0; part < 2; ++part)
#pragma unroll
        for (int kb = 0; kb < KB; ++kb)
#pragma unroll
            for (int tl = 0; tl < 2; ++tl)
                AR[part][kb][tl] = reinterpret_cast<const u32x4_t *>(img)[((part * KB + kb) * RT + (2 * wave + tl)) * WAVE + lane];
    acc_t PADC[2];
#pragma unroll
    for (int tl = 0; tl < 2; ++tl)
#pragma unroll
        for (int r = 0; r < NREG; ++r) PADC[tl][r] = C::lidx(2 * wave + tl, r, grp) >= K ? 1.f : 0.f;

    auto product = [&](int panel, acc_t (&OUT)[2]) {
#pragma unroll
        for (int tl = 0; tl < 2; ++tl) OUT[tl] = PADC[tl];
        if (live_wave) {
#pragma unroll
            for (int kb = 0; kb < KB; ++kb)
                if (kb < KBL) {
                    const u32x4_t b0 = PB[panel][kb][0][lane], b1 = PB[panel][kb][1][lane];
#pragma unroll
                    for (int tl = 0; tl < 2; ++tl) {
                        OUT[tl] = mfma_pieces<C>(AR[1][kb][tl], b0, OUT[tl]);
                        OUT[tl] = mfma_pieces<C>(AR[0][kb][tl], b1, OUT[tl]);
                        OUT[tl] = mfma_pieces<C>(AR[0][kb][tl], b0, OUT[tl]);
                    }
                }
        }
    };
    auto pieces_of = [&](const acc_t (&X)[2], u32x4_t &hi, u32x4_t &lo) {
#pragma unroll
        for (int h = 0; h < 4; ++h) {
            unsigned int a, b;
            quot_pieces(X[h / 2][2 * (h & 1)], X[h / 2][2 * (h & 1) + 1], a, b);
            hi[h] = a; lo[h] = b;
        }
    };

    bool active = false, want = true, exhausted = false;
    int q = 0, ii = 0, chk = 1, flags = 0;
    float errv = 1.f, thr = 0.f;
    acc_t A[2], B[2], V[2], U[2], ACC[2];
#pragma unroll
    for (int tl = 0; tl < 2; ++tl)
#pragma unroll
        for (int r = 0; r < NREG; ++r) { A[tl][r] = B[tl][r] = V[tl][r] = U[tl][r] = 0.f; ACC[tl][r] = 1.f; }
    u32x4_t pu_hi = {0u, 0u, 0u, 0u}, pu_lo = pu_hi, pv_hi = pu_hi, pv_lo = pu_hi;
    int res_next = 0, res_end = 0, res_base = 0, qbatch = 0, ibatch = 0, jbatch = 0, draws = 0;
    const bool all_over = p.unequal && *p.unequal != 0;
    if (threadIdx.x < 2 * TILE) (&ovc[0][0])[threadIdx.x] = 0;
    __syncthreads();

    for (int it = 0;; ++it) {
        const int par = it & 1;
        const unsigned long long wmask = __ballot(want) & colmask;
        if (wmask) {
            if (res_next >= res_end && !exhausted) {
                int base;
                if (draws == 0) {
                    base = (int)blockIdx.x * TILE;
                } else {
                    if (threadIdx.x == 0)
                        sh_base[draws & 1] = (int)gridDim.x * TILE + __hip_atomic_fetch_add(p.queue_head, TILE, __ATOMIC_RELAXED, __HIP_MEMORY_SCOPE_AGENT);
                    __syncthreads();
                    base = __builtin_amdgcn_readfirstlane(sh_base[draws & 1]);
                }
                ++draws;
                exhausted = base >= n_items;
                res_next = exhausted ? n_items : base;
                res_end = (base + TILE < n_items) ? base + TILE : n_items;
                if (exhausted) res_end = n_items;
                res_base = base;
                const int bi = base + col;
                qbatch = (p.list && bi < n_items) ? p.list[bi] : bi;
                const int qv = bi < n_items ? qbatch : 0;
                ibatch = p.row_begin + (qv / N) * p.row_step;
                jbatch = qv % N;
            }
            const int avail = res_end - res_next;
            const int n_want = (int)__popcll(wmask);
            const int rank = (int)__popcll(wmask & ((1ull << col) - 1ull));
            const int item = res_next + rank;
            const bool take = want && rank < avail;
            const int bsel = 4 * ((item - res_base) & (TILE - 1));
            const int qsel = __builtin_amdgcn_ds_bpermute(bsel, qbatch);
            const int isel = __builtin_amdgcn_ds_bpermute(bsel, ibatch), jsel = __builtin_amdgcn_ds_bpermute(bsel, jbatch);
            res_next = __builtin_amdgcn_readfirstlane(res_next + (n_want < avail ? n_want : avail));
            if (want && !take && exhausted) {
                want = false;
#pragma unroll
                for (int tl = 0; tl < 2; ++tl)
#pragma unroll
                    for (int r = 0; r < NREG; ++r) { A[tl][r] = B[tl][r] = 0.f; ACC[tl][r] = 1.f; }
                pu_hi = pu_lo = u32x4_t{0u, 0u, 0u, 0u};
            }
            if (take) {
                want = false; active = true;
                q = qsel;
#pragma unroll
                for (int tl = 0; tl < 2; ++tl) {
                    const int t = 2 * wave + tl;
                    load_regs<C>(Pt + (size_t)isel * KP + (t * NGRP + grp) * NREG, A[tl]);
                    load_regs<C>(Pt + (size_t)jsel * KP + (t * NGRP + grp) * NREG, B[tl]);
                    load_regs<C>(acc0 + (t * NGRP + grp) * NREG, ACC[tl]);
#pragma unroll
                    for (int r = 0; r < NREG; ++r) {
                        A[tl][r] *= H_IN_SCALE; B[tl][r] *= H_IN_SCALE;
                        U[tl][r] = uinit - uinit * PADC[tl][r];
                    }
                }
                pieces_of(U, pu_hi, pu_lo);
                thr = Pt[(size_t)N * KP + jsel] * H_IN_SCALE;
                chk = 1; ii = 0; flags = 0; errv = 1.f;
                if (all_over) {
                    if (wave == 0 && grp == 0) {
                        int *meta = reinterpret_cast<int *>(rec_base + (size_t)q * WIDE_REC + 2 * WIDE_PE + 1);
                        meta[0] = q; meta[1] = FLAG_NAN;
                    }
                    active = false; want = true;
                }
            }
        }
        if (__ballot(active || want) == 0ull) break;

        float mx = 0.f;
#pragma unroll
        for (int tl = 0; tl < 2; ++tl)
#pragma unroll
            for (int r = 0; r < NREG; ++r) { V[tl][r] = B[tl][r] * C::rcp(ACC[tl][r]); mx = fmaxf(mx, V[tl][r]); }
        pieces_of(V, pv_hi, pv_lo);
        PB[0][wave][0][lane] = pv_hi; PB[0][wave][1][lane] = pv_lo;
        if (active && !(mx <= tau)) ovc[par][col] = 1;
        __syncthreads();
        product(0, ACC);
        mx = 0.f;
#pragma unroll
        for (int tl = 0; tl < 2; ++tl)
#pragma unroll
            for (int r = 0; r < NREG; ++r) { U[tl][r] = A[tl][r] * C::rcp(ACC[tl][r]); mx = fmaxf(mx, U[tl][r]); }
        pieces_of(U, pu_hi, pu_lo);
        PB[1][wave][0][lane] = pu_hi; PB[1][wave][1][lane] = pu_lo;
        if (active && !(mx <= tau)) ovc[par][col] = 1;
        if (threadIdx.x < TILE) ovc[par ^ 1][threadIdx.x] = 0;
        __syncthreads();
        const bool over = active && ovc[par][col] != 0;
        if (over) {
            if (wave == 0 && grp == 0) {
                int *meta = reinterpret_cast<int *>(rec_base + (size_t)q * WIDE_REC + 2 * WIDE_PE + 1);
                meta[0] = q; meta[1] = FLAG_NAN;
            }
            active = false; want = true;
        }
        ++ii;
        product(1, ACC);
        const bool pending = active && ii == chk;
        if (pending) chk += p.period;
        const bool capped = active && ii >= p.max_iter;
        if (__ballot(pending || capped)) {
            float e2 = 0.f;
#pragma unroll
            for (int tl = 0; tl < 2; ++tl) {
                float et = 0.f;
#pragma unroll
                for (int r = 0; r < NREG; ++r) { const float d = V[tl][r] * ACC[tl][r] - B[tl][r]; et += d * d; }
                e2 += et;
            }
            e2 = group_sum<C>(e2);
            if (grp == 0) red_e2[par][wave][col] = e2;
            __syncthreads();
            float tot = 0.f;
#pragma unroll
            for (int w = 0; w < WIDE_WAVES; ++w) tot += red_e2[par][w][col];
            const float e = sqrtf(tot);
            bool fin = capped;
            if (pending) {
                errv = e;
                if (e <= thr) { fin = true; flags |= FLAG_CONVERGED; }
                else if (e != e) { fin = true; flags |= FLAG_NAN; }
            }
            if (fin) {
                float *rec = rec_base + (size_t)q * WIDE_REC;
                *reinterpret_cast<u32x4_t *>(rec + ((0 * KB + wave) * NGRP + grp) * 4) = pu_hi;
                *reinterpret_cast<u32x4_t *>(rec + ((1 * KB + wave) * NGRP + grp) * 4) = pu_lo;
                *reinterpret_cast<u32x4_t *>(rec + WIDE_PE + ((0 * KB + wave) * NGRP + grp) * 4) = pv_hi;
                *reinterpret_cast<u32x4_t *>(rec + WIDE_PE + ((1 * KB + wave) * NGRP + grp) * 4) = pv_lo;
                if (wave == 0 && grp == 0) {
                    rec[2 * WIDE_PE] = 1.f;
                    int *meta = reinterpret_cast<int *>(rec + 2 * WIDE_PE + 1);
                    meta[0] = q; meta[1] = flags;
                    if (p.iters) p.iters[q] = ii;
                    if (p.err) p.err[q] = double(errv) * double(1.f / H_IN_SCALE);
                }
                active = false; want = true;
            }
        }
    }
}

__global__ void __launch_bounds__(WAVE * WAVES_PER_WG) sinkhorn_wide_value_kernel(GridParams p, const float *__restrict__ rec_base) {
    const int n_tiles = (p.n_pairs + 15) / 16;
    const int n_waves = (int)gridDim.x * WAVES_PER_WG;
    for (int tile = (int)blockIdx.x * WAVES_PER_WG + (int)threadIdx.x / WAVE; tile < n_tiles; tile += n_waves) {
        const int cnt = p.n_pairs - tile * 16 < 16 ? p.n_pairs - tile * 16 : 16;
        ring_flush_body<CfgH32x16, WIDE_RT, true>(rec_base + (size_t)tile * 16 * WIDE_REC, p, cnt);
    }
}

}
```

Measured before the change: 568.3 million.

## Double-buffer control blocks and fuse pair ordering into a one-pass prep

Adds two ping-pong control blocks so each call zeroes the next call's block during prep instead of issuing a separate memset up front. It also adds a one-pass ordering mode that skips the order_scatter kernel, with consumers resolving pair indices through a class-end map (pair_at). The intent is fewer launches and memsets per call. The cost is more complex state, including graph-capture bookkeeping and cleanup on error paths.

```diff
diff --git a/pilot_amd/csrc/grid_plan.hpp b/pilot_amd/csrc/grid_plan.hpp
--- a/pilot_amd/csrc/grid_plan.hpp
+++ b/pilot_amd/csrc/grid_plan.hpp
@@ -12,10 +12,10 @@
     void *img;
     void *p_slot;
     int *track_list;
+    int *ctrl_blocks;
     int *ctrl;
     int *order_list;
     unsigned char *order_bucket;
-    int *order_hist;
     int *flags_ws;
     int *emd_counter;
     double *f_slab;
@@ -48,6 +48,8 @@
     } gkey;
     hipStream_t gstream;
     hipGraphExec_t gexec;
+    int capturing;
+    int *gctrl_next;
 };
 
 namespace pilot {
diff --git a/pilot_amd/csrc/pilot_ot_sinkhorn.hip b/pilot_amd/csrc/pilot_ot_sinkhorn.hip
--- a/pilot_amd/csrc/pilot_ot_sinkhorn.hip
+++ b/pilot_amd/csrc/pilot_ot_sinkhorn.hip
@@ -59,13 +59,13 @@
     pilot_ot_plan *pl = new (std::nothrow) pilot_ot_plan();
     if (!pl) return fail(PILOT_OT_EINVAL, "out of host memory");
     pl->N = N; pl->K = K; pl->max_cost = 1.0;
-    pl->img = nullptr; pl->p_slot = nullptr; pl->track_list = nullptr; pl->ctrl = nullptr;
+    pl->img = nullptr; pl->p_slot = nullptr; pl->track_list = nullptr; pl->ctrl_blocks = nullptr; pl->ctrl = nullptr;
     pl->emd_counter = nullptr; pl->f_slab = nullptr; pl->f_slab_bytes = 0; pl->emdg_slab = nullptr; pl->emdg_wgs = 0; pl->n_cu = 256; pl->kws = nullptr; pl->generic_wgs = 0; pl->nan_list = nullptr;
     pl->wide_rec = nullptr; pl->wide_rec_n = 0;
-    pl->order_list = nullptr; pl->order_bucket = nullptr; pl->order_hist = nullptr;
+    pl->order_list = nullptr; pl->order_bucket = nullptr;
     pl->flags_ws = nullptr;
     pl->timing = 0; pl->n_timed = 0; pl->n_calls = 0;
-    pl->graph_mode = 0; pl->gkey_seen = 0; pl->gstream = nullptr; pl->gexec = nullptr;
+    pl->graph_mode = 0; pl->gkey_seen = 0; pl->gstream = nullptr; pl->gexec = nullptr; pl->capturing = 0; pl->gctrl_next = nullptr;
     for (int i = 0; i < TIMING_RING; ++i) for (int j = 0; j < 4; ++j) pl->ev[i][j] = nullptr;
     hipError_t e = hipGetDevice(&pl->device);
     if (e == hipSuccess) pl->n_cu = pilot::cu_count();
@@ -88,8 +88,11 @@
         if (e == hipSuccess) e = hipMalloc(&pl->p_slot, p_bytes);
     }
     if (e == hipSuccess) e = hipMalloc(reinterpret_cast<void **>(&pl->track_list), sizeof(int) * (size_t)N * N);
-    if (e == hipSuccess) e = hipMalloc(reinterpret_cast<void **>(&pl->ctrl), pilot::CTRL_BLOCK_INTS * sizeof(int));
-    if (e == hipSuccess) e = hipMalloc(reinterpret_cast<void **>(&pl->order_list), sizeof(int) * (size_t)N * N);
+    const size_t ctrl_bytes = pilot::CTRL_BLOCKS * pilot::CTRL_BLOCK_INTS * sizeof(int);
+    if (e == hipSuccess) e = hipMalloc(reinterpret_cast<void **>(&pl->ctrl_blocks), ctrl_bytes);
+    if (e == hipSuccess) e = hipMemset(pl->ctrl_blocks, 0, ctrl_bytes);
+    if (e == hipSuccess) e = hipStreamSynchronize(nullptr);
+    if (e == hipSuccess) e = hipMalloc(reinterpret_cast<void **>(&pl->order_list), pilot::order_ws_bytes(N));
     if (e == hipSuccess) e = hipMalloc(reinterpret_cast<void **>(&pl->order_bucket), (size_t)N * N);
     if (e == hipSuccess) e = hipMalloc(reinterpret_cast<void **>(&pl->emd_counter), pilot::emd_counter_bytes());
     if (e == hipSuccess) e = hipMalloc(reinterpret_cast<void **>(&pl->nan_list), 2 * sizeof(int) * (size_t)N * N);
@@ -98,7 +101,7 @@
         pilot_ot_plan_destroy(pl);
         return fail(PILOT_OT_EHIP, "plan allocation failed: %s", hipGetErrorString(e));
     }
-    pl->order_hist = pl->ctrl + pilot::CTRL_ORDER_HIST;
+    pl->ctrl = pl->ctrl_blocks;
     *plan = pl;
     return PILOT_OT_OK;
 }
@@ -115,7 +118,7 @@
     if (pl->img) (void)hipFree(pl->img);
     if (pl->p_slot) (void)hipFree(pl->p_slot);
     if (pl->track_list) (void)hipFree(pl->track_list);
-    if (pl->ctrl) (void)hipFree(pl->ctrl);
+    if (pl->ctrl_blocks) (void)hipFree(pl->ctrl_blocks);
     if (pl->order_list) (void)hipFree(pl->order_list);
     if (pl->order_bucket) (void)hipFree(pl->order_bucket);
     if (pl->flags_ws) (void)hipFree(pl->flags_ws);
@@ -170,7 +173,8 @@
         HIP_TRY(hipMalloc(reinterpret_cast<void **>(&pl->kws), per * wgs));
         pl->generic_wgs = wgs;
     }
-    if (!queue) { queue = pl->ctrl + pilot::CTRL_GENERIC_HEAD; HIP_TRY(hipMemsetAsync(queue, 0, sizeof(int), s)); }
+    const bool own_queue = !queue;
+    if (own_queue) { queue = pl->ctrl + pilot::CTRL_GENERIC_HEAD; HIP_TRY(hipMemsetAsync(queue, 0, sizeof(int), s)); }
     pilot::GenericParams g;
     g.P = d_P; g.M = d_M; g.N = N; g.K = K; g.n_pairs = n_pairs; g.row_begin = row_begin; g.row_step = row_step;
     g.reg = reg; g.tau = tau; g.stop_thr = stop_thr; g.max_iter = num_iter_max; g.period = check_period;
@@ -182,26 +186,36 @@
     HIP_TRY(hipFuncSetAttribute(reinterpret_cast<const void *>(pilot::sinkhorn_generic_kernel), hipFuncAttributeMaxDynamicSharedMemorySize, (int)lds));
     hipLaunchKernelGGL(pilot::sinkhorn_generic_kernel, dim3(wgs), dim3(pilot::GENERIC_WG), lds, s, g);
     HIP_TRY(hipGetLastError());
-    return PILOT_OT_OK;
-}
-
-pilot::GridParams call_params(const pilot_ot_plan *pl, int n_pairs, int row_begin, int row_step, int num_iter_max, int check_period,
+    if (own_queue) HIP_TRY(hipMemsetAsync(queue, 0, sizeof(int), s));
+    return PILOT_OT_OK;
+}
+
+struct CtrlTake { int *ctrl, *other; };
+int ctrl_take(pilot_ot_plan *pl, bool zero_first, hipStream_t s, CtrlTake *t) {
+    t->ctrl = pl->ctrl;
+    t->other = pl->ctrl_blocks + (pl->ctrl == pl->ctrl_blocks ? pilot::CTRL_BLOCK_INTS : 0);
+    if (zero_first || pl->capturing) HIP_TRY(hipMemsetAsync(t->ctrl, 0, pilot::CTRL_BLOCK_INTS * sizeof(int), s));
+    return PILOT_OT_OK;
+}
+void ctrl_prepped(pilot_ot_plan *pl, const CtrlTake &t) { pl->ctrl = t.other; }
+
+pilot::GridParams call_params(const pilot_ot_plan *pl, int *ctrl, int n_pairs, int row_begin, int row_step, int num_iter_max, int check_period,
                               double stop_thr, double tau, double floor_ulps, double *d_emd, int *d_iters, double *d_err, int *d_flags) {
     pilot::GridParams p;
     p.P = pl->p_slot; p.img = pl->img; p.N = pl->N; p.K = pl->K;
     p.n_pairs = n_pairs;
-    p.list = pl->order_list; p.list_len = nullptr;
+    p.list = pl->order_list; p.list_len = nullptr; p.class_end = nullptr;
     p.solo_len = nullptr; p.solo_head = nullptr; p.solo_blocks = 0;
     p.row_begin = row_begin; p.row_step = row_step;
     p.max_iter = num_iter_max; p.period = check_period;
     p.stop_thr = stop_thr; p.tau = tau; p.floor_ulps = floor_ulps;
     p.emd = d_emd; p.iters = d_iters; p.err = d_err; p.flags = d_flags;
-    p.track_list = pl->track_list; p.track_count = pl->ctrl + pilot::CTRL_TRACK_LEN;
-    p.queue_head = pl->ctrl + pilot::CTRL_HEAD_FAST; p.queue_shards = nullptr;
+    p.track_list = pl->track_list; p.track_count = ctrl + pilot::CTRL_TRACK_LEN;
+    p.queue_head = ctrl + pilot::CTRL_HEAD_FAST; p.queue_shards = nullptr;
     p.ring = 0; p.bands = 1;
     p.fb_list = nullptr; p.fb_count = nullptr;
-    p.nan_list = pl->nan_list; p.nan_count = pl->ctrl + pilot::CTRL_NAN_LEN;
-    p.unequal = pl->ctrl + pilot::CTRL_UNEQUAL;
+    p.nan_list = pl->nan_list; p.nan_count = ctrl + pilot::CTRL_NAN_LEN;
+    p.unequal = ctrl + pilot::CTRL_UNEQUAL;
     p.debug = 0;
     return p;
 }
@@ -212,17 +226,21 @@
     const int N = pl->N, K = pl->K, RT = (K + 15) / 16;
     const pilot::GridPasses g = pilot::plan_grid(cfg, N, K, n_rows, sym, mixed, pl->max_cost / reg, pl->n_cu, sw);
     if (g.rc != PILOT_OT_OK) return fail(g.rc, "%s", g.msg);
-    HIP_TRY(hipMemsetAsync(pl->ctrl, 0, pilot::CTRL_BLOCK_INTS * sizeof(int), s));
+    CtrlTake ct;
+    if (const int rc = ctrl_take(pl, !g.one_pass || n_rows == 0, s, &ct)) return rc;
     if (n_rows == 0) return PILOT_OT_OK;
-    pilot::GridParams p = call_params(pl, n_rows * N, row_begin, row_step, num_iter_max, check_period, stop_thr, tau, floor_ulps, d_emd, d_iters,
+    int *const ctrl = ct.ctrl;
+    pilot::GridParams p = call_params(pl, ctrl, n_rows * N, row_begin, row_step, num_iter_max, check_period, stop_thr, tau, floor_ulps, d_emd, d_iters,
                                       d_err, d_flags);
     p.debug = sw.debug;
     int *const lists[] = {pl->order_list, pl->track_list, pl->nan_list + (size_t)N * N};
-    auto slot = [&](int at) { return at == pilot::CTRL_NONE ? nullptr : pl->ctrl + at; };
+    auto slot = [&](int at) { return at == pilot::CTRL_NONE ? nullptr : ctrl + at; };
     if (g.f64.run) { p.fb_list = lists[g.f64.list]; p.fb_count = slot(pilot::CTRL_FB_LEN); }
     if (g.fast.solo_blocks) { p.solo_len = slot(pilot::CTRL_SOLO_LEN); p.solo_head = slot(pilot::CTRL_HEAD_SOLO); }
     auto launch = [&](const pilot::PassPlan &v) -> hipError_t {
-        p.list = lists[v.list]; p.list_len = slot(v.len_slot); p.queue_head = slot(v.head_slot); p.queue_shards = slot(v.shards_at);
+        p.list = lists[v.list]; p.list_len = slot(v.len_slot);
+        p.class_end = (v.list == pilot::LIST_ORDER && g.one_pass) ? slot(pilot::CTRL_CLASS_END) : nullptr;
+        p.queue_head = slot(v.head_slot); p.queue_shards = slot(v.shards_at);
         p.solo_blocks = v.solo_blocks; p.ring = v.lds.ring; p.bands = v.bands;
         const dim3 wgs(v.wgs);
         if (v.solo_f64) return pilot::launch_solo_track_f64(wgs, s, p);
@@ -234,7 +252,8 @@
                                        : pilot::launch_stream_f32(RT, sym, v.track, wgs, v.lds.bytes, s, p);
     };
     HIP_TRY(pilot::launch_prep(cfg, d_M, K, RT, reg, pl->img, d_P, pl->p_slot, N, g.write_tail, stop_thr, floor_ulps, n_rows, row_begin, row_step,
-                               pl->order_bucket, pl->order_hist, pl->order_list, slot(pilot::CTRL_SPLIT), slot(pilot::CTRL_HEAD_FAST), g.mode, g.ob, s));
+                               pilot::PrepOrder{pl->order_bucket, ctrl, pl->order_list, ct.other, g.mode | (g.one_pass ? 8 : 0), g.ob}, s));
+    ctrl_prepped(pl, ct);
     hipEvent_t *ev = (pl->timing > 0 && (pl->n_calls++ % pl->timing) == 0) ? pl->ev[pl->n_timed % TIMING_RING] : nullptr;
     if (ev) HIP_TRY(hipEventRecord(ev[0], s));
     if (g.fast.run) HIP_TRY(launch(g.fast));
@@ -243,7 +262,7 @@
     HIP_TRY(launch(g.track));
     if (g.f64.run) {
         HIP_TRY(pilot::launch_prep(pilot::CFG_F64, d_M, K, RT, reg, pl->img, d_P, pl->p_slot, N, 2, stop_thr, floor_ulps, 0, row_begin, row_step,
-                                   pl->order_bucket, pl->order_hist, pl->order_list, slot(pilot::CTRL_SPLIT), slot(pilot::CTRL_HEAD_FAST), 0, 1, s));
+                                   pilot::PrepOrder{pl->order_bucket, ctrl, pl->order_list, nullptr, 0, 1}, s));
         p.img = pl->img; p.fb_list = nullptr; p.fb_count = nullptr;
         HIP_TRY(launch(g.f64));
     }
@@ -270,8 +289,11 @@
         }
         return PILOT_OT_OK;
     }
-    HIP_TRY(hipMemsetAsync(pl->ctrl, 0, (pilot::CTRL_ORDER_HIST + 2 * pilot::ORDER_NB) * sizeof(int), s));
+    const bool one_pass = pilot::one_pass_order(N, sw);
+    CtrlTake ct;
+    if (const int rc = ctrl_take(pl, !one_pass || n_rows == 0, s, &ct)) return rc;
     if (n_rows == 0) return PILOT_OT_OK;
+    int *const ctrl = ct.ctrl;
     const int n_pairs = n_rows * N;
     if ((size_t)n_pairs > pl->wide_rec_n) {
         if (pl->wide_rec) HIP_TRY(hipFree(pl->wide_rec));
@@ -282,9 +304,11 @@
     int ob = (n_pairs + 1023) / 1024;
     if (ob > pl->n_cu) ob = pl->n_cu;
     HIP_TRY(pilot::launch_prep(pilot::CFG_H32, d_M, K, RT, reg, pl->img, d_P, pl->p_slot, N, 0, stop_thr, floor_ulps, n_rows, row_begin, row_step,
-                               pl->order_bucket, pl->order_hist, pl->order_list, pl->ctrl + pilot::CTRL_SPLIT, pl->ctrl + pilot::CTRL_HEAD_FAST, 0, ob, s));
-    const pilot::GridParams p = call_params(pl, n_pairs, row_begin, row_step, num_iter_max, check_period, stop_thr, tau, floor_ulps, d_emd,
+                               pilot::PrepOrder{pl->order_bucket, ctrl, pl->order_list, ct.other, one_pass ? 8 : 0, ob}, s));
+    ctrl_prepped(pl, ct);
+    pilot::GridParams p = call_params(pl, ctrl, n_pairs, row_begin, row_step, num_iter_max, check_period, stop_thr, tau, floor_ulps, d_emd,
                                             d_iters, d_err, d_flags);
+    if (one_pass) p.class_end = ctrl + pilot::CTRL_CLASS_END;
     hipEvent_t *ev = (pl->timing > 0 && (pl->n_calls++ % pl->timing) == 0) ? pl->ev[pl->n_timed % TIMING_RING] : nullptr;
     if (ev) HIP_TRY(hipEventRecord(ev[0], s));
     const int tiles = (n_pairs + 15) / 16;
@@ -294,7 +318,7 @@
     HIP_TRY(pilot::launch_wide_value(dim3(pilot::clamp_wgs(pl->n_cu, 2, tiles)), s, p, pl->wide_rec));
     if (ev) { HIP_TRY(hipEventRecord(ev[3], s)); ++pl->n_timed; }
     return run_generic(pl, sw, d_P, d_M, reg, num_iter_max, stop_thr, tau, check_period, row_begin, n_rows, row_step, d_emd, d_iters, d_err,
-                       d_flags, s, pl->nan_list, pl->ctrl + pilot::CTRL_NAN_LEN, pl->ctrl + pilot::CTRL_NAN_HEAD);
+                       d_flags, s, pl->nan_list, ctrl + pilot::CTRL_NAN_LEN, ctrl + pilot::CTRL_NAN_HEAD);
 }
 
 pilot::SinkhornSwitches read_switches() {
@@ -302,7 +326,9 @@
     const int debug = dbg ? atoi(dbg) : 0;
     const int no_quad = pilot::test_switch("PILOT_OT_NO_QUAD") ? 1 : 0;
     const char *gw = pilot::test_switch("PILOT_OT_GENERIC_WGS");
-    return {debug, no_quad, gw ? atoi(gw) : 0};
+    const int generic_wgs = gw ? atoi(gw) : 0;
+    const char *tp = pilot::test_switch("PILOT_OT_TWO_PASS_ORDER");
+    return {debug, no_quad, generic_wgs, (tp && *tp && *tp != '0') ? 1 : 0};
 }
 
 }
@@ -318,17 +344,21 @@
     if (rc != PILOT_OT_OK) return rc;
     const pilot::SinkhornSwitches sw = read_switches();
     if (!d_flags) d_flags = pl->flags_ws;
+    auto cleaned = [&](int r, hipStream_t on) {
+        if (r != PILOT_OT_OK) (void)hipMemsetAsync(pl->ctrl, 0, pilot::CTRL_BLOCK_INTS * sizeof(int), on);
+        return r;
+    };
     {
         const int n_rows_g = (row_end - row_begin + row_step - 1) / row_step;
         if (pl->K > MAX_K && pl->K <= WIDE_MAX_K && cost_is_symmetric && precision != PILOT_OT_PREC_GENERIC && precision != PILOT_OT_PREC_F64 &&
             pl->max_cost / reg <= h_max_cost_over_reg() && tau <= pilot::H_MAX_TAU && !pilot::test_switch("PILOT_OT_NO_WIDE")) {
             if (!(f32_floor_ulps > 0.0)) f32_floor_ulps = 8.0;
-            return run_wide(pl, sw, d_P, d_M, reg, num_iter_max, stop_thr, tau, check_period, f32_floor_ulps, row_begin, n_rows_g, row_step, d_emd,
-                            d_iters, d_err, d_flags, static_cast<hipStream_t>(stream));
+            return cleaned(run_wide(pl, sw, d_P, d_M, reg, num_iter_max, stop_thr, tau, check_period, f32_floor_ulps, row_begin, n_rows_g, row_step, d_emd,
+                                    d_iters, d_err, d_flags, static_cast<hipStream_t>(stream)), static_cast<hipStream_t>(stream));
         }
         if (precision == PILOT_OT_PREC_GENERIC || pl->K > MAX_K || pl->max_cost / reg > MAX_COST_OVER_REG)
-            return run_generic(pl, sw, d_P, d_M, reg, num_iter_max, stop_thr, tau, check_period, row_begin, n_rows_g, row_step, d_emd,
-                               d_iters, d_err, d_flags, static_cast<hipStream_t>(stream));
+            return cleaned(run_generic(pl, sw, d_P, d_M, reg, num_iter_max, stop_thr, tau, check_period, row_begin, n_rows_g, row_step, d_emd,
+                                       d_iters, d_err, d_flags, static_cast<hipStream_t>(stream)), static_cast<hipStream_t>(stream));
     }
     precision = pilot_ot_resolve_precision(precision, pl->max_cost / reg, pl->K, cost_is_symmetric, tau);
     bool mixed = false;
@@ -344,18 +374,20 @@
                           : (precision == PILOT_OT_PREC_F32 ? pilot::CFG_F32
                              : (precision == PILOT_OT_PREC_BF16X3 ? pilot::CFG_S32 : (precision == PILOT_OT_PREC_F16X2 ? pilot::CFG_H32 : pilot::CFG_F64)));
     auto run = [&](hipStream_t on) {
+        const bool was_capturing = pl->capturing != 0;
         int r = run_grid(cfg, pl, sw, d_P, d_M, reg, num_iter_max, stop_thr, tau, check_period, f32_floor_ulps, cost_is_symmetric != 0,
                          row_begin, n_rows, row_step, d_emd, d_iters, d_err, d_flags, on, mixed);
         if (r == PILOT_OT_ENOTSUP)
             r = run_generic(pl, sw, d_P, d_M, reg, num_iter_max, stop_thr, tau, check_period, row_begin, n_rows, row_step, d_emd, d_iters,
                             d_err, d_flags, on);
-        return r;
+        return was_capturing ? r : cleaned(r, on);
     };
     if (!pl->graph_mode || pl->timing || n_rows == 0) return run(s);
     const pilot_ot_plan::GraphKey key = {d_P, d_M, d_emd, d_iters, d_err, d_flags, reg, stop_thr, tau, f32_floor_ulps, pl->max_cost, num_iter_max,
                                          check_period, cfg, mixed ? 1 : 0, cost_is_symmetric != 0 ? 1 : 0, row_begin, n_rows, row_step, sw};
     if (pl->gexec && key == pl->gkey) {
         HIP_TRY(hipGraphLaunch(pl->gexec, s));
+        pl->ctrl = pl->gctrl_next;
         return PILOT_OT_OK;
     }
     if (pl->gexec) { (void)hipGraphExecDestroy(pl->gexec); pl->gexec = nullptr; }
@@ -365,14 +397,19 @@
     }
     if (!pl->gstream) HIP_TRY(hipStreamCreateWithFlags(&pl->gstream, hipStreamNonBlocking));
     HIP_TRY(hipStreamBeginCapture(pl->gstream, hipStreamCaptureModeThreadLocal));
+    int *const ctrl_before = pl->ctrl;
+    pl->capturing = 1;
     rc = run(pl->gstream);
+    pl->capturing = 0;
+    pl->gctrl_next = pl->ctrl;
     hipGraph_t graph = nullptr;
     const hipError_t ce = hipStreamEndCapture(pl->gstream, &graph);
+    if (rc != PILOT_OT_OK || ce != hipSuccess) pl->ctrl = ctrl_before;
     if (rc != PILOT_OT_OK) { if (graph) (void)hipGraphDestroy(graph); return rc; }
     if (ce != hipSuccess) { (void)hipGetLastError(); return fail(PILOT_OT_EHIP, "graph capture failed: %s", hipGetErrorString(ce)); }
     const hipError_t ie = hipGraphInstantiate(&pl->gexec, graph, nullptr, nullptr, 0);
     (void)hipGraphDestroy(graph);
-    if (ie != hipSuccess) { (void)hipGetLastError(); pl->gexec = nullptr; return fail(PILOT_OT_EHIP, "graph instantiation failed: %s", hipGetErrorString(ie)); }
+    if (ie != hipSuccess) { (void)hipGetLastError(); pl->gexec = nullptr; pl->ctrl = ctrl_before; return fail(PILOT_OT_EHIP, "graph instantiation failed: %s", hipGetErrorString(ie)); }
     HIP_TRY(hipGraphLaunch(pl->gexec, s));
     return PILOT_OT_OK;
 }
diff --git a/pilot_amd/csrc/quad_kernels.hpp b/pilot_amd/csrc/quad_kernels.hpp
--- a/pilot_amd/csrc/quad_kernels.hpp
+++ b/pilot_amd/csrc/quad_kernels.hpp
@@ -154,6 +154,7 @@
 #pragma unroll
         for (int r = 0; r < NREG; ++r) { A[tl][r] = B[tl][r] = V[tl][r] = 0.f; ACC[tl][r] = 1.f; }
     int res_next = 0, res_end = 0, res_base = 0, qbatch = 0, ibatch = 0, jbatch = 0, draws = 0;
+    const PairMap pmap = pair_map_of(p);
     const bool all_over = p.unequal && *p.unequal != 0;
     if (threadIdx.x < 2 * TILE) (&ovc[0][0])[threadIdx.x] = 0;
     lds_barrier();
@@ -180,7 +181,7 @@
                 if (exhausted) res_end = n_items;
                 res_base = base;
                 const int bi = base + col;
-                qbatch = (p.list && bi < n_items) ? p.list[bi] : bi;
+                qbatch = bi < n_items ? pair_at(p, pmap, bi) : bi;
                 const int qv = bi < n_items ? qbatch : 0;
                 ibatch = p.row_begin + (qv / N) * p.row_step;
                 jbatch = qv % N;
diff --git a/pilot_amd/csrc/sinkhorn_kernels.hpp b/pilot_amd/csrc/sinkhorn_kernels.hpp
--- a/pilot_amd/csrc/sinkhorn_kernels.hpp
+++ b/pilot_amd/csrc/sinkhorn_kernels.hpp
@@ -567,6 +567,7 @@
     int n_pairs;
     const int *list;
     const int *list_len;
+    const int *class_end;
     int row_begin, row_step;
     int max_iter, period;
     double stop_thr, tau, floor_ulps;
@@ -601,6 +602,22 @@
 template <class C> __host__ __device__ constexpr int img_total(int RT) { return img_total_plain<C>(RT) + (C::HALF ? img_total_plain<CfgS32x16>(RT) : 0); }
 
 
+struct PairMap { int end[ORDER_CLASSES - 1]; };
+__device__ inline PairMap pair_map_of(const GridParams &p) {
+    PairMap m;
+#pragma unroll
+    for (int c = 0; c < ORDER_CLASSES - 1; ++c) m.end[c] = p.class_end ? __builtin_amdgcn_readfirstlane(p.class_end[c]) : 0;
+    return m;
+}
+__device__ inline int pair_at(const GridParams &p, const PairMap &m, int item) {
+    if (!p.list) return item;
+    if (!p.class_end) return p.list[item];
+    int at = item;
+#pragma unroll
+    for (int c = 0; c < ORDER_CLASSES - 1; ++c) at = item >= m.end[c] ? item - m.end[c] + (c + 1) * p.n_pairs : at;
+    return p.list[at];
+}
+
 template <typename T> __device__ inline T readlane_t(T x, int k);
 template <> __device__ inline float readlane_t<float>(float x, int k) {
     return __int_as_float(__builtin_amdgcn_readlane(__float_as_int(x), k));
@@ -664,13 +681,14 @@
     const T acc0 = inrec ? img[acc0_offset<C>(RT) + pos] * (C::HALF ? T(1) / (T(H_GIBBS_SCALE) * T(H_PANEL_SCALE)) : T(1)) : T(1);
     const T tau = T(p.tau);
     const int n_items = *n_items_ptr;
+    const PairMap pmap = pair_map_of(p);
     const T kk = T(K) * T(K);
     for (;;) {
         int item = 0;
         if (lane == 0) item = __hip_atomic_fetch_add(head_ptr, 1, __ATOMIC_RELAXED, __HIP_MEMORY_SCOPE_AGENT);
         item = __builtin_amdgcn_readfirstlane(item);
         if (item >= n_items) break;
-        const int q = p.list[item];
+        const int q = pair_at(p, pmap, item);
         const int i = p.row_begin + (q / N) * p.row_step, j = q % N;
         const T a = inrec ? Pt[(size_t)i * KP + pos] : T(0), b = inrec ? Pt[(size_t)j * KP + pos] : T(0);
         const T thr = Pt[(size_t)N * KP + j];
@@ -925,6 +943,7 @@
     const int n_items = p.list_len ? *p.list_len : p.n_pairs;
     const int lane = threadIdx.x % WAVE;
     if (block * WAVES_PER_WG * TILE >= n_items) return;
+    const PairMap pmap = pair_map_of(p);
 
     const bool two_bands = C::SPLIT && TRACK && p.bands == 2;
     const int n_img = two_bands ? stream_layout(shape_of<C>(), RT, SYM, TRACK, TV, 2, 0).table : L0.table;
@@ -1106,7 +1125,7 @@
                 if (exhausted) res_end = n_items;
                 res_base = base;
                 const int bi = base + col;
-                qbatch = (p.list && bi < n_items) ? p.list[bi] : bi;
+                qbatch = bi < n_items ? pair_at(p, pmap, bi) : bi;
                 const int qv = bi < n_items ? qbatch : 0;
                 ibatch = p.row_begin + (qv / N) * p.row_step;
                 jbatch = qv % N;
@@ -1641,9 +1660,12 @@
 
 constexpr int ORDER_JW = 128, ORDER_RI = 8;
 
-__device__ inline void bucket_body(int tile, const double *__restrict__ Psrc, int N, int K, int n_rows, int row_begin,
-                                   int row_step, unsigned char *__restrict__ bucket, int *__restrict__ hist, int collapse,
+__device__ inline void bucket_body(int tile, int n_tiles, const double *__restrict__ Psrc, int N, int K, int n_rows, int row_begin,
+                                   int row_step, unsigned char *__restrict__ bucket, int *__restrict__ ctrl, int *__restrict__ list, int mode,
                                    unsigned char *order_smem) {
+    const bool one_pass = (mode & 8) != 0;
+    const int collapse = (mode >> 2) & 1;
+    int *const hist = ctrl + CTRL_ORDER_HIST;
     const int K4 = (K + 3) & ~3;
     float *Bt = reinterpret_cast<float *>(order_smem);
     float *Ar = Bt + (size_t)K4 * (ORDER_JW + 1);
@@ -1680,6 +1702,7 @@
             for (int e = 0; e < 4; ++e) l1[r] += fabsf(av[e] - bv[e]);
         }
     }
+    int cls[R], slot[R];
 #pragma unroll
     for (int r = 0; r < R; ++r) {
         const int rr = rb + half * R + r;
@@ -1692,11 +1715,46 @@
         } else if (row_begin + rr * row_step != jb + jl) {
             b = ORDER_NB - 2;
         }
-        if (valid) bucket[(size_t)rr * N + jb + jl] = (unsigned char)b;
-        (void)lds_count_aggregated(lh, b, valid);
+        if (one_pass) {
+            cls[r] = order_class_of(b);
+            slot[r] = lds_count_aggregated(lh, cls[r], valid);
+        } else {
+            if (valid) bucket[(size_t)rr * N + jb + jl] = (unsigned char)b;
+            (void)lds_count_aggregated(lh, b, valid);
+        }
     }
     __syncthreads();
-    for (int i = threadIdx.x; i < ORDER_NB; i += blockDim.x) if (lh[i]) atomicAdd(&hist[i], lh[i]);
+    if (!one_pass) {
+        for (int i = threadIdx.x; i < ORDER_NB; i += blockDim.x) if (lh[i]) atomicAdd(&hist[i], lh[i]);
+        return;
+    }
+    const int n_pairs = n_rows * N;
+    if (threadIdx.x < ORDER_CLASSES) {
+        const int c = lh[threadIdx.x];
+        lh[ORDER_CLASSES + threadIdx.x] = c ? __hip_atomic_fetch_add(ctrl + CTRL_CLASS_COUNT + threadIdx.x, c, __ATOMIC_RELAXED, __HIP_MEMORY_SCOPE_AGENT) : 0;
+    }
+    __syncthreads();
+#pragma unroll
+    for (int r = 0; r < R; ++r) {
+        const bool valid = jl < nj && half * R + r < nr;
+        const int at = lh[ORDER_CLASSES + cls[r]] + slot[r];
+        if (valid && at < n_pairs) list[order_class_offset(cls[r], n_pairs) + at] = (rb + half * R + r) * N + jb + jl;
+    }
+    if (threadIdx.x == 0) {
+        const int done = __hip_atomic_fetch_add(ctrl + CTRL_ORDER_TICKET, 1, __ATOMIC_ACQ_REL, __HIP_MEMORY_SCOPE_AGENT);
+        if (done == n_tiles - 1) {
+            int end = 0;
+            for (int c = 0; c < ORDER_CLASSES; ++c) {
+                end += __hip_atomic_load(ctrl + CTRL_CLASS_COUNT + c, __ATOMIC_RELAXED, __HIP_MEMORY_SCOPE_AGENT);
+                ctrl[CTRL_CLASS_END + c] = end;
+                if (c == 0) {
+                    const int n_dup = (mode & 2) ? end : 0;
+                    for (int i = 0; i < CTRL_SPLIT_INTS; ++i) ctrl[CTRL_SPLIT + i] = n_dup;
+                    ctrl[CTRL_HEAD_FAST] = n_dup;
+                }
+            }
+        }
+    }
 }
 
 constexpr int PREP_SETUP_BLOCKS = 64;
@@ -1706,14 +1764,17 @@
                                                             typename C::T *__restrict__ Pdst, int N, int write_tail, double stop_thr,
                                                             double floor_ulps, int n_tiles,
                                                             int n_rows, int row_begin, int row_step,
-                                                            unsigned char *__restrict__ bucket, int *__restrict__ hist, int collapse) {
+                                                            unsigned char *__restrict__ bucket, int *__restrict__ ctrl, int *__restrict__ list,
+                                                            int *__restrict__ zero_ctrl, int mode) {
     extern __shared__ __attribute__((aligned(16))) unsigned char order_smem[];
     if ((int)blockIdx.x < n_tiles) {
-        bucket_body(blockIdx.x, Psrc, N, K, n_rows, row_begin, row_step, bucket, hist, collapse, order_smem);
+        bucket_body(blockIdx.x, n_tiles, Psrc, N, K, n_rows, row_begin, row_step, bucket, ctrl, list, mode, order_smem);
     } else {
+        if (zero_ctrl && (int)blockIdx.x == n_tiles)
+            for (int i = threadIdx.x; i < CTRL_BLOCK_INTS; i += blockDim.x) zero_ctrl[i] = 0;
         setup_body<C>(Msrc, K, RT, reg, img, Psrc, Pdst, (long)N * RT * C::TILE, write_tail, stop_thr, floor_ulps,
                       ((int)blockIdx.x - n_tiles) * (int)blockDim.x + (int)threadIdx.x, PREP_SETUP_BLOCKS * (int)blockDim.x,
-                      hist - (CTRL_ORDER_HIST - CTRL_UNEQUAL));
+                      ctrl + CTRL_UNEQUAL);
     }
 }
 
diff --git a/pilot_amd/csrc/sinkhorn_launch.hpp b/pilot_amd/csrc/sinkhorn_launch.hpp
--- a/pilot_amd/csrc/sinkhorn_launch.hpp
+++ b/pilot_amd/csrc/sinkhorn_launch.hpp
@@ -17,9 +17,16 @@
 hipError_t launch_stream_s32(int RT, bool sym, bool track, int live1, dim3 grid, size_t lds, hipStream_t s, const GridParams &p);
 hipError_t launch_stream_h32(int RT, bool sym, int live1, dim3 grid, size_t lds, hipStream_t s, const GridParams &p);
 hipError_t launch_stream_tv(int cfg, int tv, int RT, bool sym, bool track, dim3 grid, size_t lds, hipStream_t s, const GridParams &p);
+struct PrepOrder {
+    unsigned char *bucket;
+    int *ctrl;
+    int *list;
+    int *zero_ctrl;
+    int mode;
+    int n_blocks;
+};
 hipError_t launch_prep(int cfg, const double *M, int K, int RT, double reg, void *img, const double *P, void *Pslot, int N, int write_tail,
-                       double stop_thr, double floor_ulps, int n_rows, int row_begin, int row_step, unsigned char *bucket, int *hist, int *list, int *split,
-                       int *main_queue_head, int mode, int n_blocks, hipStream_t s);
+                       double stop_thr, double floor_ulps, int n_rows, int row_begin, int row_step, const PrepOrder &o, hipStream_t s);
 hipError_t launch_wide(dim3 grid, hipStream_t s, const GridParams &p, float *rec);
 hipError_t launch_wide_value(dim3 grid, hipStream_t s, const GridParams &p, const float *rec);
 size_t wide_rec_elems();
diff --git a/pilot_amd/csrc/sinkhorn_layout.hpp b/pilot_amd/csrc/sinkhorn_layout.hpp
--- a/pilot_amd/csrc/sinkhorn_layout.hpp
+++ b/pilot_amd/csrc/sinkhorn_layout.hpp
@@ -86,6 +86,7 @@
         if (ring >= min_ring || want == 1) return {fixed + slots * (size_t)(ring < 1 ? 1 : ring), ring, want};
     }
 }
+constexpr int CTRL_BLOCKS = 2;
 constexpr int ORDER_NB = 48;
 constexpr int QUEUE_SHARDS = 32, QUEUE_SHARD_STRIDE = 32;
 enum : int {
@@ -102,13 +103,24 @@
     CTRL_NAN_LEN = 10,
     CTRL_NAN_HEAD = 11,
     CTRL_UNEQUAL = 12,
+    CTRL_ORDER_TICKET = 13,
     CTRL_INTS = 16,
     CTRL_ORDER_HIST = CTRL_INTS,
+    CTRL_CLASS_COUNT = CTRL_ORDER_HIST,
+    CTRL_CLASS_END = CTRL_CLASS_COUNT + 8,
     CTRL_SHARDS_AT = (CTRL_ORDER_HIST + 2 * ORDER_NB + 31) / 32 * 32,
     CTRL_SHARDS_TRACK_AT = CTRL_SHARDS_AT + QUEUE_SHARDS * QUEUE_SHARD_STRIDE,
     CTRL_BLOCK_INTS = CTRL_SHARDS_TRACK_AT + QUEUE_SHARDS * QUEUE_SHARD_STRIDE,
     CTRL_NONE = -1,
 };
+constexpr int ORDER_CLASSES = 8;
+static_assert(CTRL_CLASS_END + ORDER_CLASSES <= CTRL_ORDER_HIST + 2 * ORDER_NB, "the class slots lie in the histogram's ints");
+constexpr int order_class_of(int b) { return b == ORDER_NB - 1 ? 0 : (b == ORDER_NB - 2 ? 1 : (b >= 6 ? 2 : (b >= 2 ? 8 - b : ORDER_CLASSES - 1))); }
+constexpr size_t ORDER_ONE_PASS_MAX_BYTES = (size_t)256 << 20;
+constexpr size_t order_class_bytes(int N) { return sizeof(int) * (size_t)ORDER_CLASSES * (size_t)N * (size_t)N; }
+constexpr bool order_one_pass(int N) { return order_class_bytes(N) <= ORDER_ONE_PASS_MAX_BYTES; }
+constexpr size_t order_ws_bytes(int N) { return order_one_pass(N) ? order_class_bytes(N) : sizeof(int) * (size_t)N * (size_t)N; }
+constexpr size_t order_class_offset(int c, int n_pairs) { return (size_t)c * (size_t)n_pairs; }
 enum : int {
     DBG_NATURAL_ORDER = 2,
     DBG_WGS_SHIFT = 4,
@@ -123,7 +135,10 @@
     int debug;
     int no_quad;
     int generic_wgs;
-    bool operator==(const SinkhornSwitches &o) const { return debug == o.debug && no_quad == o.no_quad && generic_wgs == o.generic_wgs; }
+    int two_pass_order;
+    bool operator==(const SinkhornSwitches &o) const {
+        return debug == o.debug && no_quad == o.no_quad && generic_wgs == o.generic_wgs && two_pass_order == o.two_pass_order;
+    }
 };
 
 constexpr int QUAD_MIN_K = 113, QUAD_MAX_K = 128;
@@ -144,8 +159,10 @@
     int rc = PILOT_OT_OK;
     char msg[160] = "";
     int mode = 0, write_tail = 0, ob = 0;
+    bool one_pass = false;
     PassPlan fast, track, f64;
 };
+constexpr bool one_pass_order(int N, const SinkhornSwitches &sw) { return order_one_pass(N) && !sw.two_pass_order; }
 inline GridPasses plan_grid(int cfg, int N, int K, int n_rows, bool sym, bool mixed, double max_cost_over_reg, int n_cu, const SinkhornSwitches &sw) {
     GridPasses g;
     const CfgShape fast = shape_of(cfg);
@@ -184,6 +201,7 @@
     }
     g.rc = PILOT_OT_OK;
     if (n_rows == 0) { f.run = t.run = d.run = false; return g; }
+    g.one_pass = one_pass_order(N, sw);
     g.ob = min_of((n_pairs + 1023) / 1024, n_cu);
     g.mode = (solo ? 2 : 0) | ((debug & DBG_NATURAL_ORDER) ? 4 : 0);
     g.write_tail = (tv ? 1 : 0) | 2 | (mixed ? 4 : 0);
diff --git a/pilot_amd/csrc/sk_inst.hip b/pilot_amd/csrc/sk_inst.hip
--- a/pilot_amd/csrc/sk_inst.hip
+++ b/pilot_amd/csrc/sk_inst.hip
@@ -39,10 +39,8 @@
 
 template <class C>
 hipError_t prep_any(const double *M, int K, int RT, double reg, void *img, const double *P, void *Pslot, int N, int write_tail,
-                    double stop_thr, double floor_ulps, int n_rows, int row_begin, int row_step, unsigned char *bucket, int *hist, int *list, int *split,
-                    int *main_queue_head, int mode, int n_blocks, hipStream_t s) {
+                    double stop_thr, double floor_ulps, int n_rows, int row_begin, int row_step, const PrepOrder &o, hipStream_t s) {
     using T = typename C::T;
-    const int collapse = (mode >> 2) & 1;
     const int tiles = n_rows > 0 ? ((N + ORDER_JW - 1) / ORDER_JW) * ((n_rows + ORDER_RI - 1) / ORDER_RI) : 0;
     const int K4 = (K + 3) & ~3;
     const size_t lds = sizeof(float) * ((size_t)K4 * (ORDER_JW + 1) + (size_t)ORDER_RI * K4) + sizeof(int) * ORDER_NB;
@@ -56,10 +54,11 @@
         attr_set[dev] = true;
     }
     hipLaunchKernelGGL(sinkhorn_prep_kernel<C>, dim3(tiles + PREP_SETUP_BLOCKS), dim3(256), lds, s, M, K, RT, reg, static_cast<T *>(img), P,
-                       static_cast<T *>(Pslot), N, write_tail, stop_thr, floor_ulps, tiles, n_rows, row_begin, row_step, bucket, hist, collapse);
-    if (n_rows > 0)
-        hipLaunchKernelGGL(order_scatter_kernel, dim3(n_blocks), dim3(256), 0, s, bucket, n_rows * N, hist, hist + ORDER_NB, list, split,
-                           main_queue_head, mode & 3);
+                       static_cast<T *>(Pslot), N, write_tail, stop_thr, floor_ulps, tiles, n_rows, row_begin, row_step, o.bucket, o.ctrl, o.list,
+                       o.zero_ctrl, o.mode);
+    if (n_rows > 0 && !(o.mode & 8))
+        hipLaunchKernelGGL(order_scatter_kernel, dim3(o.n_blocks), dim3(256), 0, s, o.bucket, n_rows * N, o.ctrl + CTRL_ORDER_HIST,
+                           o.ctrl + CTRL_ORDER_HIST + ORDER_NB, o.list, o.ctrl + CTRL_SPLIT, o.ctrl + CTRL_HEAD_FAST, o.mode & 3);
     return hipGetLastError();
 }
 }
@@ -69,28 +68,20 @@
     return stream_any<CfgF32x16>(RT, sym, track, grid, lds, s, p);
 }
 hipError_t launch_prep_f64(const double *M, int K, int RT, double reg, void *img, const double *P, void *Pslot, int N, int write_tail,
-                           double stop_thr, double floor_ulps, int n_rows, int row_begin, int row_step, unsigned char *bucket, int *hist, int *list, int *split,
-                           int *main_queue_head, int mode, int n_blocks, hipStream_t s);
+                           double stop_thr, double floor_ulps, int n_rows, int row_begin, int row_step, const PrepOrder &o, hipStream_t s);
 hipError_t launch_prep_s32(const double *M, int K, int RT, double reg, void *img, const double *P, void *Pslot, int N, int write_tail,
-                           double stop_thr, double floor_ulps, int n_rows, int row_begin, int row_step, unsigned char *bucket, int *hist, int *list, int *split,
-                           int *main_queue_head, int mode, int n_blocks, hipStream_t s);
+                           double stop_thr, double floor_ulps, int n_rows, int row_begin, int row_step, const PrepOrder &o, hipStream_t s);
 hipError_t launch_prep_h32(const double *M, int K, int RT, double reg, void *img, const double *P, void *Pslot, int N, int write_tail,
-                           double stop_thr, double floor_ulps, int n_rows, int row_begin, int row_step, unsigned char *bucket, int *hist, int *list, int *split,
-                           int *main_queue_head, int mode, int n_blocks, hipStream_t s);
+                           double stop_thr, double floor_ulps, int n_rows, int row_begin, int row_step, const PrepOrder &o, hipStream_t s);
 hipError_t launch_prep(int cfg, const double *M, int K, int RT, double reg, void *img, const double *P, void *Pslot, int N, int write_tail,
-                       double stop_thr, double floor_ulps, int n_rows, int row_begin, int row_step, unsigned char *bucket, int *hist, int *list, int *split,
-                       int *main_queue_head, int mode, int n_blocks, hipStream_t s) {
+                       double stop_thr, double floor_ulps, int n_rows, int row_begin, int row_step, const PrepOrder &o, hipStream_t s) {
     if (cfg == CFG_F64)
-        return launch_prep_f64(M, K, RT, reg, img, P, Pslot, N, write_tail, stop_thr, floor_ulps, n_rows, row_begin, row_step, bucket, hist, list, split,
-                               main_queue_head, mode, n_blocks, s);
+        return launch_prep_f64(M, K, RT, reg, img, P, Pslot, N, write_tail, stop_thr, floor_ulps, n_rows, row_begin, row_step, o, s);
     if (cfg == CFG_H32)
-        return launch_prep_h32(M, K, RT, reg, img, P, Pslot, N, write_tail, stop_thr, floor_ulps, n_rows, row_begin, row_step, bucket, hist, list, split,
-                               main_queue_head, mode, n_blocks, s);
+        return launch_prep_h32(M, K, RT, reg, img, P, Pslot, N, write_tail, stop_thr, floor_ulps, n_rows, row_begin, row_step, o, s);
     if (cfg == CFG_S32)
-        return launch_prep_s32(M, K, RT, reg, img, P, Pslot, N, write_tail, stop_thr, floor_ulps, n_rows, row_begin, row_step, bucket, hist, list, split,
-                               main_queue_head, mode, n_blocks, s);
-    return prep_any<CfgF32x16>(M, K, RT, reg, img, P, Pslot, N, write_tail, stop_thr, floor_ulps, n_rows, row_begin, row_step, bucket, hist, list, split,
-                               main_queue_head, mode, n_blocks, s);
+        return launch_prep_s32(M, K, RT, reg, img, P, Pslot, N, write_tail, stop_thr, floor_ulps, n_rows, row_begin, row_step, o, s);
+    return prep_any<CfgF32x16>(M, K, RT, reg, img, P, Pslot, N, write_tail, stop_thr, floor_ulps, n_rows, row_begin, row_step, o, s);
 }
 size_t track_img_elems(int cfg, int RT) { return cfg == CFG_H32 ? (size_t)track_img_offset<CfgH32x16>(RT) : 0; }
 size_t img_elems(int cfg, int RT) {
@@ -114,10 +105,8 @@
     return hipGetLastError();
 }
 hipError_t launch_prep_f64(const double *M, int K, int RT, double reg, void *img, const double *P, void *Pslot, int N, int write_tail,
-                           double stop_thr, double floor_ulps, int n_rows, int row_begin, int row_step, unsigned char *bucket, int *hist, int *list, int *split,
-                           int *main_queue_head, int mode, int n_blocks, hipStream_t s) {
-    return prep_any<CfgF64x16>(M, K, RT, reg, img, P, Pslot, N, write_tail, stop_thr, floor_ulps, n_rows, row_begin, row_step, bucket, hist, list, split,
-                               main_queue_head, mode, n_blocks, s);
+                           double stop_thr, double floor_ulps, int n_rows, int row_begin, int row_step, const PrepOrder &o, hipStream_t s) {
+    return prep_any<CfgF64x16>(M, K, RT, reg, img, P, Pslot, N, write_tail, stop_thr, floor_ulps, n_rows, row_begin, row_step, o, s);
 }
 #elif SK_PART == 7
 hipError_t launch_stream_s32_l1(int RT, bool sym, bool track, dim3 grid, size_t lds, hipStream_t s, const GridParams &p) {
@@ -134,10 +123,8 @@
     return stream_any<CfgH32x16>(RT, sym, false, grid, lds, s, p);
 }
 hipError_t launch_prep_h32(const double *M, int K, int RT, double reg, void *img, const double *P, void *Pslot, int N, int write_tail,
-                           double stop_thr, double floor_ulps, int n_rows, int row_begin, int row_step, unsigned char *bucket, int *hist, int *list, int *split,
-                           int *main_queue_head, int mode, int n_blocks, hipStream_t s) {
-    return prep_any<CfgH32x16>(M, K, RT, reg, img, P, Pslot, N, write_tail, stop_thr, floor_ulps, n_rows, row_begin, row_step, bucket, hist, list, split,
-                               main_queue_head, mode, n_blocks, s);
+                           double stop_thr, double floor_ulps, int n_rows, int row_begin, int row_step, const PrepOrder &o, hipStream_t s) {
+    return prep_any<CfgH32x16>(M, K, RT, reg, img, P, Pslot, N, write_tail, stop_thr, floor_ulps, n_rows, row_begin, row_step, o, s);
 }
 #elif SK_PART == 6
 hipError_t launch_stream_s32_l1(int RT, bool sym, bool track, dim3 grid, size_t lds, hipStream_t s, const GridParams &p);
@@ -146,10 +133,8 @@
     return stream_any<CfgS32x16>(RT, sym, track, grid, lds, s, p);
 }
 hipError_t launch_prep_s32(const double *M, int K, int RT, double reg, void *img, const double *P, void *Pslot, int N, int write_tail,
-                           double stop_thr, double floor_ulps, int n_rows, int row_begin, int row_step, unsigned char *bucket, int *hist, int *list, int *split,
-                           int *main_queue_head, int mode, int n_blocks, hipStream_t s) {
-    return prep_any<CfgS32x16>(M, K, RT, reg, img, P, Pslot, N, write_tail, stop_thr, floor_ulps, n_rows, row_begin, row_step, bucket, hist, list, split,
-                               main_queue_head, mode, n_blocks, s);
+                           double stop_thr, double floor_ulps, int n_rows, int row_begin, int row_step, const PrepOrder &o, hipStream_t s) {
+    return prep_any<CfgS32x16>(M, K, RT, reg, img, P, Pslot, N, write_tail, stop_thr, floor_ulps, n_rows, row_begin, row_step, o, s);
 }
 #else
 #if SK_PART == 2
diff --git a/pilot_amd/csrc/wide_kernels.hpp b/pilot_amd/csrc/wide_kernels.hpp
--- a/pilot_amd/csrc/wide_kernels.hpp
+++ b/pilot_amd/csrc/wide_kernels.hpp
@@ -75,6 +75,7 @@
         for (int r = 0; r < NREG; ++r) { A[tl][r] = B[tl][r] = V[tl][r] = U[tl][r] = 0.f; ACC[tl][r] = 1.f; }
     u32x4_t pu_hi = {0u, 0u, 0u, 0u}, pu_lo = pu_hi, pv_hi = pu_hi, pv_lo = pu_hi;
     int res_next = 0, res_end = 0, res_base = 0, qbatch = 0, ibatch = 0, jbatch = 0, draws = 0;
+    const PairMap pmap = pair_map_of(p);
     const bool all_over = p.unequal && *p.unequal != 0;
     if (threadIdx.x < 2 * TILE) (&ovc[0][0])[threadIdx.x] = 0;
     __syncthreads();
@@ -100,7 +101,7 @@
                 if (exhausted) res_end = n_items;
                 res_base = base;
                 const int bi = base + col;
-                qbatch = (p.list && bi < n_items) ? p.list[bi] : bi;
+                qbatch = bi < n_items ? pair_at(p, pmap, bi) : bi;
                 const int qv = bi < n_items ? qbatch : 0;
                 ibatch = p.row_begin + (qv / N) * p.row_step;
                 jbatch = qv % N;
```

Result: slower. 529.0 million (-6.9%).
